# adalkiran/llama-nuts-and-bolts

Hardware: AMD Instinct MI355X
Metric: decode tokens/s Llama-3.1-8B bf16 @1/2/4/8 MI355X; % HBM roofline (higher is better)
Workload: dtype bf16; 1 GPU; Llama-3.1-8B bf16, 1xMI355X, single-prompt greedy decode, seq_len=128 -> +125 tokens (configs[1]'s prompt, --steps 125); prompt_len=128, sequences_in_flight=1, parallelism=single GPU, mode=exact-order (token-id identical to the CPU reference path), reported_repeat=median, weight_bytes_resident=16060522496

## Files before the change

### include/lnb.h

```cpp
#ifndef LNB_H
#define LNB_H
#include <stdint.h>
#ifdef __cplusplus
extern "C" {
#endif

typedef struct lnb_model lnb_model;
typedef struct lnb_ctx lnb_ctx;

typedef struct lnb_model_args {
    int32_t dim;
    int32_t n_layers;
    int32_t n_heads;
    int32_t n_kv_heads;
    int32_t vocab_size;
    int32_t multiple_of;
    double  ffn_dim_multiplier;
    float   norm_eps;
    int32_t use_scaled_rope;
    double  rope_theta;
    int32_t max_seq_len;
} lnb_model_args;

#define LNB_ABI_VERSION 6
// ... 52 lines not shown
enum { LNB_SCHED_LATENCY = 0, LNB_SCHED_THROUGHPUT = 1 };
int lnb_ctx_set_schedule(lnb_ctx* c, int sched);
int lnb_ctx_get_schedule(const lnb_ctx* c);
int lnb_ctx_set_attention(lnb_ctx* c, int long_threshold, int force_zseq);
int lnb_ctx_zseq_count(lnb_ctx* c, int* out);
int lnb_ctx_norm_fallbacks(lnb_ctx* c, int* out);
int lnb_ctx_prefill_attention_form(const lnb_ctx* c, int* out);
typedef void (*lnb_layer_cb)(int layer_1based, int n_layers, double secs, void* user);
int lnb_ctx_set_layer_callback(lnb_ctx* c, lnb_layer_cb cb, void* user);

int lnb_forward(lnb_ctx* c, const int32_t* tokens, int seq, int start_pos, float* logits_out, int32_t* argmax_last_out);

int lnb_forward_append(lnb_ctx* c, const int32_t* tokens, int seq, int start_pos, float* logits_out, int32_t* argmax_last_out);
int lnb_forward_score_append(lnb_ctx* c, const int32_t* tokens, int seq, int start_pos, const int32_t* targets,
                             float* target_logit, float* target_prob, double* log_z, int32_t* argmax_last_out);
int lnb_ctx_set_rows_attention(lnb_ctx* c, int long_threshold, int flags);
int lnb_ctx_append_attention_form(const lnb_ctx* c, int* out);

int lnb_forward_append_many(lnb_ctx* const* ctxs, int n, const int32_t* tokens, const int32_t* n_rows, const int32_t* start_pos,
                            float* logits_out, int32_t* argmax_out);
int lnb_model_append_many_info(const lnb_model* m, int* passes, int* max_columns, int* long_passes);

int lnb_decode_greedy(lnb_ctx* c, int32_t token, int start_pos, int n_steps, int32_t* out_tokens, float* ms_out);
int lnb_ctx_set_stop_ids(lnb_ctx* c, const int32_t* ids, int n);
int lnb_decode_greedy_until(lnb_ctx* c, int32_t token, int start_pos, int max_steps, int32_t* out_tokens, int* n_generated, int* finished, float* ms_out);

#define LNB_MAX_DRAFT 15
typedef struct lnb_spec_stats { int64_t passes, verify_passes, drafted, accepted; } lnb_spec_stats;
int lnb_ctx_set_draft(lnb_ctx* c, int max_draft, int ngram_min, int ngram_max, const int32_t* corpus, int n_corpus);
int lnb_decode_speculative_until(lnb_ctx* c, const int32_t* history, int n_history, int32_t token, int start_pos,
                                 int max_steps, int32_t* out_tokens, int* n_generated, int* finished,
                                 lnb_spec_stats* stats, float* ms_out);
int lnb_op_ngram_draft(int device, const int32_t* text, int n_text, const int32_t* corpus, int n_corpus,
                       int ngram_min, int ngram_max, int max_draft, int32_t* out, int* n_out);

typedef struct lnb_spec_many_info { int64_t passes, verify_passes, columns, max_columns, long_passes; } lnb_spec_many_info;
int lnb_decode_speculative_many(lnb_ctx* const* ctxs, int n, const int32_t* const* history, const int32_t* n_history,
                                const int32_t* tokens, const int32_t* start_pos, int max_steps, int col_budget,
                                int32_t* out_tokens, int32_t* n_generated, int32_t* finished,
                                lnb_spec_stats* stats, lnb_spec_many_info* info, float* ms_out);

#define LNB_MAX_TOP_K 16
int lnb_ctx_set_token_probs(lnb_ctx* c, int top_k);
int lnb_ctx_read_token_probs(lnb_ctx* c, int first, int n, int32_t* ids, float* logits, float* probs, double* log_z);
int lnb_ctx_token_prob_walks(lnb_ctx* c, int* out);
int lnb_forward_score(lnb_ctx* c, const int32_t* tokens, int seq, int start_pos, const int32_t* targets,
                      float* target_logit, float* target_prob, double* log_z, int32_t* argmax_last_out);
int lnb_op_token_probs(int device, const uint16_t* logits_bf16, int rows, int V, int top_k, const int32_t* targets,
                       int force_serial, int32_t* ids, float* logits, float* probs, float* target_prob, double* log_z, int* serial_walks);

typedef struct lnb_batch lnb_batch;
int lnb_model_enable_batch(lnb_model* m);
int64_t lnb_model_batch_bytes(lnb_model* m);
int lnb_batch_create(lnb_ctx* const* ctxs, int n, lnb_batch** out);
int lnb_batch_destroy(lnb_batch* b);
int lnb_batch_decode(lnb_batch* b, const int32_t* tokens, const int32_t* start_pos, int n_steps, int32_t* out_tokens, float* ms_out);
int lnb_batch_decode_until(lnb_batch* b, const int32_t* tokens, const int32_t* start_pos, int max_steps, int32_t* out_tokens, int32_t* n_generated, int32_t* finished, float* ms_out);
int lnb_batch_profile_kernel(lnb_batch* b, int which, int pos, int iters, float* avg_ms_out);
int lnb_batch_set_attention(lnb_batch* b, int long_threshold, int force_zseq);
int lnb_ctx_set_batched_attention(lnb_ctx* c, int long_threshold, int force_zseq);
int lnb_batch_attention_form(const lnb_batch* b, int* out);
int lnb_ctx_verify_attention_form(const lnb_ctx* c, int* out);

void* lnb_ctx_hidden_ptr(lnb_ctx* c, int which);
int lnb_forward_stage(lnb_ctx* c, const int32_t* tokens, int seq, int start_pos, float* logits_out, int32_t* argmax_last_out);
int lnb_forward_stage_begin(lnb_ctx* c, const int32_t* tokens, int seq, int start_pos, int want_argmax);
int lnb_forward_stage_end(lnb_ctx* c, int32_t* argmax_last_out);
int lnb_ctx_synchronize(lnb_ctx* c);
void* lnb_ctx_stream(lnb_ctx* c);

typedef struct lnb_pipe lnb_pipe;
int lnb_pipeline_unique_id(void* id128);
int lnb_pipeline_init(lnb_model* stage, int rank, int world, const void* id128, lnb_pipe** out);
int lnb_pipeline_init_loopback(lnb_model* stage, int rank, int world, const char* group, lnb_pipe** out);
int lnb_pipeline_init_host(lnb_model* stage, int rank, int world, lnb_pipe** out);
int lnb_pipeline_destroy(lnb_pipe* p);
int lnb_pipeline_tick(lnb_pipe* p, lnb_ctx* run, int run_rows, int run_pos, const int32_t* run_tokens,
                      lnb_ctx* send, int send_rows, lnb_ctx* recv, int recv_rows, int* token_slot_out);
int lnb_batch_set_state(lnb_batch* b, const int32_t* tokens, const int32_t* start_pos);
int lnb_batch_check_error(lnb_batch* b);
void* lnb_batch_boundary_ptr(lnb_batch* b, int which);
int lnb_pipeline_tick_batch(lnb_pipe* p, lnb_batch* run, lnb_batch* send, lnb_batch* recv, int* token_slot_out);
int lnb_pipeline_sync(lnb_pipe* p);
int lnb_pipeline_comm_count(lnb_pipe* p, int* out);
int lnb_pipeline_read_tokens(lnb_pipe* p, int first_slot, int n, int32_t* out);
int lnb_pipeline_selftest(int device, int n_bytes);

int lnb_profile_kernel(lnb_ctx* c, int which, int pos, int iters, float* avg_ms_out);
int lnb_profile_ffn_pair(lnb_ctx* c, int pos, int iters, int w2_delay_us, int w2_lds_pad, float* avg_ms_out);
int lnb_profile_kernel_stamps(lnb_ctx* c, int which, int pos, double* out, int* wall_clock_khz);

int lnb_op_linear(int device, const uint16_t* x, const uint16_t* w, uint16_t* y, int rows, int n_out, int k_in, int rw);
int lnb_op_rmsnorm_linear(int device, const uint16_t* x, const uint16_t* norm_w, float eps, const uint16_t* w,
                          uint16_t* y, int rows, int n_out, int k_in, int rw);

int lnb_op_linear_mode(int device, const uint16_t* x, const uint16_t* norm_w, float eps, const uint16_t* w, uint16_t* y,
                       int rows, int n_out, int k_in, int rw, int mode);
int lnb_op_argmax(int device, const uint16_t* logits_bf16, int n, int32_t* out);
int lnb_op_exp_table(int device, float divisor, double* out65536);

typedef struct lnb_checkpoint lnb_checkpoint;
enum { LNB_DTYPE_BF16 = 0, LNB_DTYPE_F16 = 1, LNB_DTYPE_F32 = 2 };
int lnb_checkpoint_open(const char* path, lnb_checkpoint** out);
void lnb_checkpoint_close(lnb_checkpoint* c);
int lnb_checkpoint_num_tensors(const lnb_checkpoint* c);
int lnb_checkpoint_find(const lnb_checkpoint* c, const char* name);
int lnb_checkpoint_tensor(const lnb_checkpoint* c, int index, const char** name, int* dtype, int64_t* shape4, int* rank,
                          const void** data, int64_t* nbytes);
int lnb_model_load_checkpoint(lnb_model* m, const lnb_checkpoint* c);
int lnb_model_args_from_json(const char* params_json_path, lnb_model_args* out);

typedef struct lnb_tokenizer lnb_tokenizer;
int lnb_tokenizer_load(const char* tokenizer_model_path, lnb_tokenizer** out);
void lnb_tokenizer_free(lnb_tokenizer* t);
int lnb_tokenizer_vocab_size(const lnb_tokenizer* t);
int lnb_tokenizer_special(const lnb_tokenizer* t, int32_t* bos, int32_t* eos, int32_t* eot, int32_t* eom);
int lnb_tokenizer_token_id(const lnb_tokenizer* t, const char* bytes, int len);
int lnb_tokenizer_piece(const lnb_tokenizer* t, int32_t id, const char** bytes, int* len);
int lnb_tokenizer_encode(const lnb_tokenizer* t, const char* text, int len, int32_t* out, int cap);
int lnb_tokenizer_encode_chat(const lnb_tokenizer* t, const char* const* headers, const char* const* contents, int n_parts,
                              int32_t* out, int cap);
typedef struct lnb_detok lnb_detok;
int lnb_tokenizer_stream_create(const lnb_tokenizer* t, lnb_detok** out);
void lnb_tokenizer_stream_free(lnb_detok* d);
int lnb_tokenizer_decode_stream(lnb_detok* d, int32_t token_id, char* out, int cap, int* added_to_waiting);
int lnb_tokenizer_stream_pending(const lnb_detok* d, const char** bytes, int* len);

#ifdef __cplusplus
}
#endif
#endif
```

### llama-nuts-and-bolts_amd/csrc/lnb_api.cpp

```cpp
#include <hip/hip_runtime.h>
#include <algorithm>
#include <array>
#include <cmath>
#include <cstdarg>
#include <cstdio>
#include <cstdlib>
#include <cstring>
#include <chrono>
#include <dirent.h>
#include <unistd.h>
#include <deque>
#include <map>
#include <mutex>
#include <string>
#include <vector>
#include "../../include/lnb.h"
#include "lnb_device.h"
#include "lnb_knobs.h"
#include "lnb_kvcopy.h"
#include "lnb_rowpack.h"
#include "lnb_batchplan.h"
#include "lnb_rccl.h"
static_assert(LNB_MAX_SEQ_LEN == LNB_SEQ_MAX, "lnb.h and lnb_device.h disagree on the longest context");
static_assert(ROWPACK_MAX_W == LNB_BATCH_MAX, "lnb_rowpack.h and lnb_device.h disagree on the columns of a pass");
static_assert(BATCHPLAN_COLS == LNB_STREAM_COLS, "lnb_batchplan.h and lnb_device.h disagree on the sequences of a column group");
static_assert(LNB_MAX_FORK == KVC_MAX_DST, "lnb.h and lnb_kvcopy.h disagree on the destinations of a fork");
static_assert(LNB_MAX_TOP_K == LNB_TOKPROB_MAX_K, "lnb.h and lnb_device.h disagree on the largest top-k");
static_assert(LNB_MAX_DRAFT == LNB_SPEC_MAX_DRAFT && LNB_MAX_DRAFT + 1 <= LNB_STREAM_COLS, "a verify pass is one column group of at most 16 columns");

extern "C" {
hipError_t lnbk_gemv(const GemvParams* p, int rw, int nch, int epi, int norm, hipStream_t st);
hipError_t lnbk_attn(const AttnParams* p, hipStream_t st);
hipError_t lnbk_attn_rows(const AttnParams* p, int pos0, hipStream_t st);
int lnbk_attn_short_max_T(int hd);
size_t lnbk_attn_long_lds(int seq_len);
size_t lnbk_attn_long_layout_lds(int seq_len);
size_t lnbk_attn_one_lds(int seq_len, int hd);
hipError_t lnbk_exp_table(double* tab, float divisor, hipStream_t st);
hipError_t lnbk_gemm(const GemmParams* p, int epi, hipStream_t st);
hipError_t lnbk_rmsnorm_rows(const uint16_t* x, const uint16_t* w, uint16_t* out, int S, int K, float eps, hipStream_t st);
hipError_t lnbk_embed(const uint16_t* emb, const int32_t* tokens, uint16_t* x, int S, int dim, int vocab, int* err, hipStream_t st);
hipError_t lnbk_argmax(const uint16_t* logits, int V, int32_t* next_token, StepState* state, int32_t* out_tokens, int out_cap, int advance, hipStream_t st);
hipError_t lnbk_set_state(StepState* state, int pos, int n_out, int honour_stop, hipStream_t st);
hipError_t lnbk_set_stop(StepState* state, const int32_t* ids, int n, hipStream_t st);
hipError_t lnbk_advance_state(StepState* state, int rows, hipStream_t st);
hipError_t lnbk_tile(const uint16_t* src, uint16_t* dst, int rows, int K, int row_off, int chain, int RW, int NCH, int gather, hipStream_t st);
hipError_t lnbk_synth_fill(uint16_t* dst, int rows, int K, int row_off, int chain, int RW, int NCH, uint64_t seed, uint32_t tensor_id, int kind, float sigma, hipStream_t st);
hipError_t lnbk_init(void);
hipError_t lnbk_fast_gemv(const GemvParams* p, int rw, int nch, int epi, int norm, hipStream_t st);
hipError_t lnbk_fast_gemm(const GemmParams* p, int epi, hipStream_t st);
hipError_t lnbk_fast_attn(const AttnParams* p, hipStream_t st);
hipError_t lnbk_fast_init(void);
hipError_t lnbk_m16_from_tiled(const uint16_t* src, uint16_t* dst, int rows, int K, int RW, int NCH, hipStream_t st);
hipError_t lnbk_stream(const StreamParams* p, int epi, int acc2, int num_cus, hipStream_t st);
hipError_t lnbk_batch_rmsnorm(const uint16_t* x, const uint16_t* norm_w, float eps, uint16_t* xt, int K, int nseq, hipStream_t st);
hipError_t lnbk_batch_embed(const uint16_t* emb, const BatchTab* tab, uint16_t* x, int nseq, int dim, int vocab, int* err, hipStream_t st);
hipError_t lnbk_batch_argmax(const uint16_t* logits, int V, const BatchTab* tab, int nseq, int32_t* ring, hipStream_t st);
hipError_t lnbk_batch_set_state(const BatchTab* tab, const int32_t* tokens, const int32_t* pos, int32_t* ring, int honour_stop, hipStream_t st);
hipError_t lnbk_batch_scatter_ring(const BatchTab* tab, const int32_t* ring, hipStream_t st);
hipError_t lnbk_batch_advance(const BatchTab* tab, hipStream_t st);
hipError_t lnbk_batch_prepare(void);
hipError_t lnbk_gemm_stream(const GemmParams* p, int epi, int num_cus, hipStream_t st);
hipError_t lnbk_spin(int us, hipStream_t st);
hipError_t lnbk_token_probs(const TokProbParams* p, hipStream_t st);
hipError_t lnbk_spec_argmax(const uint16_t* logits, int V, int w, int32_t* g, hipStream_t st);
hipError_t lnbk_spec_commit(const int32_t* g, int w, const BatchTab* tab, hipStream_t st);
hipError_t lnbk_ngram_draft(const DraftParams* p, hipStream_t st);
hipError_t lnbk_kv_fork(const KvForkTab* tab, int nt, int split, hipStream_t st);
hipError_t lnbk_append_many_setup(const AmPass* p, hipStream_t st);
hipError_t lnbk_append_many_finish(const uint16_t* logits, int V, const AmRow* rows, int width, int32_t* out, hipStream_t st);
hipError_t lnbk_spec_many_draft(const SmPass* p, hipStream_t st);
hipError_t lnbk_spec_many_pack(const SmPass* p, hipStream_t st);
hipError_t lnbk_spec_many_commit(const SmPass* p, hipStream_t st);
}

static int g_hwq_set_by_library = 0;
static int g_hip_live_at_load = 0;
static bool kfd_is_open() {
    DIR* d = opendir("/proc/self/fd");
    if (!d) return false;
    bool found = false;
    char path[64], target[256];
    while (struct dirent* e = readdir(d)) {
        if (e->d_name[0] == '.') continue;
        snprintf(path, sizeof path, "/proc/self/fd/%s", e->d_name);
        const ssize_t n = readlink(path, target, sizeof target - 1);
        if (n <= 0) continue;
        target[n] = 0;
        if (!strcmp(target, "/dev/kfd")) { found = true; break; }
    }
    closedir(d);
    return found;
}
__attribute__((constructor)) static void lnb_record_hip_state_at_load() {
    g_hip_live_at_load = kfd_is_open() ? 1 : 0;
}

static thread_local char g_err[1024] = "";
static int fail(const char* fmt, ...) {
    va_list ap; va_start(ap, fmt); vsnprintf(g_err, sizeof g_err, fmt, ap); va_end(ap);
    return -1;
}
extern "C" const char* lnb_last_error(void) { return g_err; }
extern "C" __attribute__((visibility("hidden"))) void lnb_set_error(const char* msg) { snprintf(g_err, sizeof g_err, "%s", msg); }
#define HIPCHK(expr) do { hipError_t e_ = (expr); if (e_ != hipSuccess) return fail("%s failed: %s (%s:%d)", #expr, hipGetErrorString(e_), __FILE__, __LINE__); } while (0)

static inline float bf_wide_h(uint16_t b) { uint32_t u = (uint32_t)b << 16; float f; memcpy(&f, &u, 4); return f; }
static inline uint16_t bf_trunc_h(float f) { uint32_t u; memcpy(&u, &f, 4); return (uint16_t)(u >> 16); }

struct TensorRef {
    int rows = 0, cols = 0;
    bool tiled = false;
    uint16_t* linear = nullptr;
    TiledDesc* td = nullptr;
    int row_off = 0, chain = 0;
    uint32_t synth_id = 0; int synth_kind = 0;
    int rank = 2;
};
struct LayerW {
    uint16_t* attn_norm = nullptr; uint16_t* ffn_norm = nullptr;
    TiledDesc wqkv{}, wo{}, w13{}, w2{};
    uint16_t *m_wqkv = nullptr, *m_wo = nullptr, *m_w13 = nullptr, *m_w2 = nullptr;
};
struct lnb_model {
    lnb_model_args a{};
    int device = 0, layer_begin = 0, layer_end = 0;
    int part_begin = 0, part_end = 0;
    int head_dim = 0, n_rep = 0, ffn_hidden = 0, q_dim = 0, kv_dim = 0;
    uint16_t* tok_embd = nullptr; uint16_t* norm = nullptr; TiledDesc output{};
    std::vector<LayerW> layers;
    std::map<std::string, TensorRef> tensors;
    float* cis = nullptr; int cis_rows = 0; float* silu = nullptr; double* exp_tab = nullptr;
    double* prob_etab = nullptr;
    std::vector<float> cis_host;
    hipStream_t stream = nullptr;
    bool finalized = false;
    int64_t weight_bytes = 0;
    bool batch_enabled = false; uint16_t* m_output = nullptr; int64_t batch_bytes = 0;
    std::mutex am_mu; struct AppendMany* am = nullptr;
    bool first() const { return part_begin == 0; }
    bool last() const { return part_end == 3 * a.n_layers; }
    bool has_part(int l, int q) const { return 3 * l + q >= part_begin && 3 * l + q < part_end; }
    bool has_attn(int l) const { return has_part(l, 0); }
    bool has_w13(int l) const { return has_part(l, 1); }
    bool has_w2(int l) const { return has_part(l, 2); }
    bool whole(int l) const { return has_attn(l) && has_w13(l) && has_w2(l); }
};
struct lnb_ctx {
    lnb_model* m = nullptr; int seq_len = 0;
    int max_rows = 0;
    hipStream_t stream = nullptr;
    std::vector<uint16_t*> ck, cv;
    StepState* st = nullptr; int32_t* dtok = nullptr; int32_t* dnext = nullptr; int* derr = nullptr;
    int32_t* dout = nullptr; int dout_cap = 0;
    uint16_t *x = nullptr, *h = nullptr, *q = nullptr, *att = nullptr, *ffn = nullptr, *logits = nullptr;
    uint16_t* xn = nullptr;
    int logits_rows = 0;
    hipGraphExec_t graph = nullptr;
    hipEvent_t ev0 = nullptr, ev1 = nullptr;
    lnb_layer_cb cb = nullptr; void* cb_user = nullptr;
    int32_t* h_io = nullptr;
    bool pending = false, pending_tokens = false, pending_argmax = false;
    int mode = LNB_MODE_EXACT;
    int sched = LNB_SCHED_LATENCY;
    int n_stop = 0;
    int batch_users = 0;
    double* e_buf = nullptr; double* z_part = nullptr; int* zseq_count = nullptr;
    int last_prefill_form = 0;
    uint64_t* score_idx = nullptr; size_t score_idx_bytes = 0; int sidx_jt = 0;
    unsigned* attn_cnt = nullptr;
    int attn_long_T = 0; int force_zseq = 0;
    int attn_short_cap = 0;
    bool attn_long = false;
    hipGraphExec_t graph_long = nullptr;
    hipGraphExec_t stage_graph[2] = {nullptr, nullptr};
    hipEvent_t ev_done = nullptr, ev_in = nullptr, ev_sent = nullptr;
    bool in_pending = false, sent_pending = false;
    int dev_pos = -1;
    bool attn_causal = false;
    int call_T = 0;
    hipEvent_t ev_h2d = nullptr; bool h2d_pending = false;
    bool recv_unmatched = false;
    int top_k = 0;
    TokProbOut* tp_out = nullptr;
    int32_t* tp_ids = nullptr; float* tp_logit = nullptr; float* tp_prob = nullptr; double* tp_logz = nullptr;
    double* tp_zpart = nullptr; uint64_t* tp_kpart = nullptr; unsigned* tp_cnt = nullptr;
    int tp_last_k = 0, tp_last_n = 0;
    void* sc_buf = nullptr; size_t sc_bytes = 0;
    int sp_max_draft = 0, sp_ngram_min = 1, sp_ngram_max = 1;
    int32_t* sp_corpus = nullptr; int sp_n_corpus = 0;
    int32_t* sp_text = nullptr; int sp_text_cap = 0;
// ... 131 lines not shown

extern "C" int lnb_model_ffn_hidden_dim(const lnb_model_args* a) {
    int h = 4 * a->dim;
    h = (int)(2 * h / 3);
    if (a->ffn_dim_multiplier > -1) h = (int)(a->ffn_dim_multiplier * (double)h);
    h = a->multiple_of * ((h + a->multiple_of - 1) / a->multiple_of);
    return h;
}

static void reg_linear(lnb_model* m, const std::string& name, uint16_t* p, int cols, uint32_t sid, int kind, int rows = 1, int rank = 1) {
    TensorRef r; r.rows = rows; r.cols = cols; r.tiled = false; r.linear = p; r.synth_id = sid; r.synth_kind = kind; r.rank = rank;
    m->tensors[name] = r;
}
static void reg_tiled(lnb_model* m, const std::string& name, TiledDesc* td, int rows, int cols, int row_off, int chain, uint32_t sid) {
    TensorRef r; r.rows = rows; r.cols = cols; r.tiled = true; r.td = td; r.row_off = row_off; r.chain = chain; r.synth_id = sid; r.rank = 2;
    m->tensors[name] = r;
}

extern "C" int lnb_model_create(const lnb_model_args* args, int device, int layer_begin, int layer_end, lnb_model** out) {
    return lnb_model_create_parts(args, device, 3 * layer_begin, 3 * layer_end, out);
}
static int model_alloc(lnb_model* m);
extern "C" int lnb_model_create_parts(const lnb_model_args* args, int device, int part_begin, int part_end, lnb_model** out) {
    if (!args || !out) return fail("null argument");
    *out = nullptr;
    const int layer_begin = part_begin / 3, layer_end = (part_end + 2) / 3;
    lnb_model_args a = *args;
    if (a.n_kv_heads < 0) a.n_kv_heads = a.n_heads;
    if (a.rope_theta <= 0) a.rope_theta = 500000.0;
    if (a.n_layers <= 0) return fail("n_layers must be positive (got %d)", a.n_layers);
    if (a.vocab_size <= 0) return fail("vocab_size must be positive (got %d; params.json without the key gives -1: take it from tok_embeddings)", a.vocab_size);
    if (a.multiple_of <= 0) return fail("multiple_of must be positive (got %d)", a.multiple_of);
    if (a.dim <= 0 || a.n_heads <= 0 || a.n_kv_heads <= 0 || a.dim % a.n_heads || a.n_heads % a.n_kv_heads) return fail("invalid head configuration");
    if (part_begin < 0 || part_end > 3 * a.n_layers || part_begin >= part_end) return fail("invalid layer range [%d,%d)", part_begin / 3, (part_end + 2) / 3);
    int hd = a.dim / a.n_heads;
    if (a.dim % 8 || hd % 8) return fail("dim and head_dim must be multiples of 8");
    int ndev = 0; HIPCHK(hipGetDeviceCount(&ndev));
    if (ndev == 0) return fail("no HIP device: liblnb_hip.so has no CPU fallback");
    if (device < 0 || device >= ndev) return fail("device %d out of range (%d devices)", device, ndev);
    HIPCHK(hipSetDevice(device));
    HIPCHK(lnbk_init());
    HIPCHK(lnbk_fast_init());
    HIPCHK(lnbk_batch_prepare());
    { hipDeviceProp_t prop; HIPCHK(hipGetDeviceProperties(&prop, device)); if (prop.multiProcessorCount > 0) g_num_cus = prop.multiProcessorCount; }
    lnb_model* m = new lnb_model();
    m->a = a; m->device = device; m->layer_begin = layer_begin; m->layer_end = layer_end; m->part_begin = part_begin; m->part_end = part_end;
    m->head_dim = hd; m->n_rep = a.n_heads / a.n_kv_heads; m->ffn_hidden = lnb_model_ffn_hidden_dim(&a);
    m->q_dim = a.n_heads * hd; m->kv_dim = a.n_kv_heads * hd;
    if (m->ffn_hidden <= 0 || m->ffn_hidden % 8) { delete m; return fail("ffn hidden dim must be a positive multiple of 8"); }
    if (model_alloc(m)) { lnb_model_destroy(m); return -1; }
    *out = m;
    return 0;
}
static int model_alloc(lnb_model* m) {
    const lnb_model_args& a = m->a;
    const int layer_begin = m->layer_begin, layer_end = m->layer_end;
    HIPCHK(hipStreamCreate(&m->stream));
    int64_t& wb = m->weight_bytes;
    const int dim = a.dim, F = m->ffn_hidden;
    if (m->first()) {
        if (alloc_linear(&m->tok_embd, (size_t)a.vocab_size * dim, wb)) return -1;
        reg_linear(m, "tok_embeddings.weight", m->tok_embd, dim, 0, 0, a.vocab_size, 2);
    }
    m->layers.resize(layer_end - layer_begin);
    const int qkv_rows = m->q_dim + 2 * m->kv_dim, rwo = auto_rw(dim, Knob::RW_WO, m->q_dim, true), rw2 = auto_rw(dim, Knob::RW_W2, F, true);
    const int rwq = auto_rw(qkv_rows, Knob::RW_QKV, dim, false, qkv_rows == 24 * g_num_cus && dim % 256 == 0 ? 24 : 0);
    const int rw13 = auto_rw(F, Knob::RW_W13, 0, false, F == 56 * g_num_cus ? 56 : 0);
    for (int l = layer_begin; l < layer_end; l++) {
        LayerW& L = m->layers[l - layer_begin];
        char nm[128]; uint32_t base = 16u * (uint32_t)(l + 1);
        if (m->has_attn(l)) {
            if (alloc_linear(&L.attn_norm, dim, wb)) return -1;
            if (alloc_tiled(L.wqkv, m->q_dim + 2 * m->kv_dim, dim, rwq, 1, wb)) return -1;
            if (alloc_tiled(L.wo, dim, m->q_dim, rwo, 1, wb)) return -1;
            snprintf(nm, sizeof nm, "layers.%d.attention_norm.weight", l); reg_linear(m, nm, L.attn_norm, dim, base + 0, 1);
            snprintf(nm, sizeof nm, "layers.%d.attention.wq.weight", l); reg_tiled(m, nm, &L.wqkv, m->q_dim, dim, 0, 0, base + 1);
            snprintf(nm, sizeof nm, "layers.%d.attention.wk.weight", l); reg_tiled(m, nm, &L.wqkv, m->kv_dim, dim, m->q_dim, 0, base + 2);
            snprintf(nm, sizeof nm, "layers.%d.attention.wv.weight", l); reg_tiled(m, nm, &L.wqkv, m->kv_dim, dim, m->q_dim + m->kv_dim, 0, base + 3);
            snprintf(nm, sizeof nm, "layers.%d.attention.wo.weight", l); reg_tiled(m, nm, &L.wo, dim, m->q_dim, 0, 0, base + 4);
        }
        if (m->has_w13(l)) {
            if (alloc_linear(&L.ffn_norm, dim, wb)) return -1;
            if (alloc_tiled(L.w13, F, dim, rw13, 2, wb)) return -1;
            snprintf(nm, sizeof nm, "layers.%d.ffn_norm.weight", l); reg_linear(m, nm, L.ffn_norm, dim, base + 5, 1);
            snprintf(nm, sizeof nm, "layers.%d.feed_forward.w1.weight", l); reg_tiled(m, nm, &L.w13, F, dim, 0, 0, base + 6);
            snprintf(nm, sizeof nm, "layers.%d.feed_forward.w3.weight", l); reg_tiled(m, nm, &L.w13, F, dim, 0, 1, base + 8);
        }
        if (m->has_w2(l)) {
            if (alloc_tiled(L.w2, dim, F, rw2, 1, wb)) return -1;
            snprintf(nm, sizeof nm, "layers.%d.feed_forward.w2.weight", l); reg_tiled(m, nm, &L.w2, dim, F, 0, 0, base + 7);
        }
    }
    if (m->last()) {
        if (alloc_linear(&m->norm, dim, wb)) return -1;
        reg_linear(m, "norm.weight", m->norm, dim, 1, 1);
        if (alloc_tiled(m->output, a.vocab_size, dim, auto_rw(a.vocab_size, Knob::RW_OUT), 1, wb)) return -1;
        reg_tiled(m, "output.weight", &m->output, a.vocab_size, dim, 0, 0, 2);
    }
    return 0;
}

static void append_many_free(lnb_model* m);
extern "C" int lnb_model_destroy(lnb_model* m) {
    if (!m) return 0;
    hipSetDevice(m->device);
    append_many_free(m);
    if (m->tok_embd) hipFree(m->tok_embd);
    if (m->norm) hipFree(m->norm);
    if (m->output.w) hipFree(m->output.w);
    for (auto& L : m->layers) {
        hipFree(L.attn_norm); hipFree(L.ffn_norm); hipFree(L.wqkv.w); hipFree(L.wo.w); hipFree(L.w13.w); hipFree(L.w2.w);
        hipFree(L.m_wqkv); hipFree(L.m_wo); hipFree(L.m_w13); hipFree(L.m_w2);
    }
    hipFree(m->m_output);
    if (m->cis) hipFree(m->cis);
    if (m->silu) hipFree(m->silu);
    if (m->exp_tab) hipFree(m->exp_tab);
    if (m->prob_etab) hipFree(m->prob_etab);
    if (m->stream) hipStreamDestroy(m->stream);
    delete m;
    return 0;
}

extern "C" int64_t lnb_model_weight_bytes(lnb_model* m) { return m ? m->weight_bytes : 0; }

extern "C" int lnb_model_set_tensor(lnb_model* m, const char* name, const uint16_t* host, const int64_t* shape, int rank) {
    if (!m || !name || !host || !shape) return fail("null argument");
    HIPCHK(hipSetDevice(m->device));
    auto it = m->tensors.find(name);
    if (it == m->tensors.end()) return fail("tensor \"%s\" does not belong to this model stage", name);
    if (m->batch_enabled) return fail("tensor \"%s\": the model's batched-decode copy has been built; bind tensors before lnb_model_enable_batch", name);
    TensorRef& r = it->second;
    if (rank != r.rank || (rank == 1 && shape[0] != r.cols) || (rank == 2 && (shape[0] != r.rows || shape[1] != r.cols)))
        return fail("tensor \"%s\": shape mismatch, expected [%d%s%d]", name, r.rank == 1 ? r.cols : r.rows, r.rank == 1 ? "" : " ", r.rank == 1 ? 0 : r.cols);
    size_t n = (size_t)r.rows * r.cols;
    if (!r.tiled) { HIPCHK(hipMemcpy(r.linear, host, n * 2, hipMemcpyHostToDevice)); return 0; }
    uint16_t* stage = nullptr;
    HIPCHK(hipMalloc((void**)&stage, n * 2));
    HIPCHK(hipMemcpy(stage, host, n * 2, hipMemcpyHostToDevice));
    hipError_t e = lnbk_tile(stage, r.td->w, r.rows, r.cols, r.row_off, r.chain, r.td->rw, r.td->nch, 0, m->stream);
    if (e == hipSuccess) e = hipStreamSynchronize(m->stream);
    hipFree(stage);
    HIPCHK(e);
    return 0;
}

extern "C" int lnb_model_num_tensors(const lnb_model* m) { return m ? (int)m->tensors.size() : 0; }
extern "C" int lnb_model_tensor_info(const lnb_model* m, int k, const char** name, int64_t* shape, int* rank) {
    if (!m || k < 0 || k >= (int)m->tensors.size()) return fail("tensor index %d out of range", k);
    auto it = m->tensors.begin();
    std::advance(it, k);
    if (name) *name = it->first.c_str();
    if (rank) *rank = it->second.rank;
    if (shape) { if (it->second.rank == 1) shape[0] = it->second.cols; else { shape[0] = it->second.rows; shape[1] = it->second.cols; } }
    return 0;
}

extern "C" int lnb_model_get_tensor(lnb_model* m, const char* name, uint16_t* host, int64_t nelem) {
    if (!m || !name || !host) return fail("null argument");
    HIPCHK(hipSetDevice(m->device));
    auto it = m->tensors.find(name);
    if (it == m->tensors.end()) return fail("tensor \"%s\" does not belong to this model stage", name);
    TensorRef& r = it->second;
    size_t n = (size_t)r.rows * r.cols;
    if ((int64_t)n != nelem) return fail("tensor \"%s\": expected %zu elements", name, n);
    if (!r.tiled) { HIPCHK(hipMemcpy(host, r.linear, n * 2, hipMemcpyDeviceToHost)); return 0; }
    uint16_t* stage = nullptr;
    HIPCHK(hipMalloc((void**)&stage, n * 2));
    hipError_t e = lnbk_tile(r.td->w, stage, r.rows, r.cols, r.row_off, r.chain, r.td->rw, r.td->nch, 1, m->stream);
    if (e == hipSuccess) e = hipStreamSynchronize(m->stream);
    if (e == hipSuccess) e = hipMemcpy(host, stage, n * 2, hipMemcpyDeviceToHost);
    hipFree(stage);
    HIPCHK(e);
    return 0;
}

extern "C" int lnb_model_fill_synthetic(lnb_model* m, uint64_t seed) {
    if (!m) return fail("null argument");
    if (m->batch_enabled) return fail("the model's batched-decode copy has been built; fill the weights before lnb_model_enable_batch");
    HIPCHK(hipSetDevice(m->device));
    for (auto& kv : m->tensors) {
        TensorRef& r = kv.second;
        if (r.tiled) HIPCHK(lnbk_synth_fill(r.td->w, r.rows, r.cols, r.row_off, r.chain, r.td->rw, r.td->nch, seed, r.synth_id, 0, 0.02f, m->stream));
        else HIPCHK(lnbk_synth_fill(r.linear, r.rows, r.cols, 0, 0, 0, 1, seed, r.synth_id, r.synth_kind, 0.02f, m->stream));
    }
    HIPCHK(hipStreamSynchronize(m->stream));
    return 0;
}

static void build_rope_table(int head_dim, int rows, double theta, bool scaled, std::vector<float>& cis) {
    const int n = head_dim / 2;
    std::vector<uint16_t> freqs(n);
    const float dimf = (float)head_dim;
    for (int i = 0; i < n; i++) {
        float val = bf_wide_h(bf_trunc_h((float)(2 * i)));
        freqs[i] = bf_trunc_h((float)(1.0 / std::pow(theta, (double)(val / dimf))));
    }
    if (scaled) {
        const float scale_factor = 8.0f, low_freq_factor = 1.0f, high_freq_factor = 4.0f, old_context_len = 8192.0f;
        const float low_freq_wavelen = old_context_len / low_freq_factor, high_freq_wavelen = old_context_len / high_freq_factor;
        for (int i = 0; i < n; i++) {
            volatile float freq = bf_wide_h(freqs[i]);
            volatile float wavelen = (float)(2 * M_PI) / freq;
            float nf;
            if (wavelen < high_freq_wavelen) nf = freq;
            else if (wavelen > low_freq_wavelen) nf = freq / scale_factor;
            else {
                volatile float smooth = (old_context_len / wavelen - low_freq_factor) / (high_freq_factor - low_freq_factor);
                volatile float t1 = (1 - smooth) * freq; t1 = t1 / scale_factor;
                volatile float t2 = smooth * freq;
                nf = t1 + t2;
            }
            freqs[i] = bf_trunc_h(nf);
        }
    }
    cis.resize((size_t)rows * n * 2);
    for (int p = 0; p < rows; p++) {
        const float t = bf_wide_h(bf_trunc_h((float)p));
        for (int i = 0; i < n; i++) {
            volatile float prod = t * bf_wide_h(freqs[i]);
            const double ang = (double)bf_wide_h(bf_trunc_h(prod));
            cis[((size_t)p * n + i) * 2 + 0] = (float)std::cos(ang);
            cis[((size_t)p * n + i) * 2 + 1] = (float)std::sin(ang);
        }
    }
}

static void prob_exp_table(std::vector<double>& et) {
    et.resize(1 << 16);
    for (int i = 0; i < (1 << 16); i++) et[i] = std::exp((double)bf_wide_h((uint16_t)i));
}
extern "C" int lnb_model_finalize(lnb_model* m, int rope_rows) {
    if (!m) return fail("null argument");
    HIPCHK(hipSetDevice(m->device));
    m->cis_rows = rope_rows > 0 ? rope_rows : m->a.max_seq_len * 2;
    build_rope_table(m->head_dim, m->cis_rows, m->a.rope_theta, m->a.use_scaled_rope != 0, m->cis_host);
    if (m->cis) hipFree(m->cis);
    HIPCHK(hipMalloc((void**)&m->cis, m->cis_host.size() * 4));
    HIPCHK(hipMemcpy(m->cis, m->cis_host.data(), m->cis_host.size() * 4, hipMemcpyHostToDevice));
    std::vector<float> silu(1 << 16);
    for (int i = 0; i < (1 << 16); i++) { double x = (double)bf_wide_h((uint16_t)i); silu[i] = (float)(x / (1.0 + std::exp(-x))); }
    if (!m->silu) HIPCHK(hipMalloc((void**)&m->silu, silu.size() * 4));
    HIPCHK(hipMemcpy(m->silu, silu.data(), silu.size() * 4, hipMemcpyHostToDevice));
    std::vector<double> et;
    prob_exp_table(et);
    if (!m->prob_etab) HIPCHK(hipMalloc((void**)&m->prob_etab, et.size() * 8));
    HIPCHK(hipMemcpy(m->prob_etab, et.data(), et.size() * 8, hipMemcpyHostToDevice));
    if (!m->exp_tab) HIPCHK(hipMalloc((void**)&m->exp_tab, (size_t)(1 << 16) * 8));
    HIPCHK(lnbk_exp_table(m->exp_tab, bf_wide_h(bf_trunc_h((float)std::sqrt((double)m->head_dim))), m->stream));
    HIPCHK(hipStreamSynchronize(m->stream));
    m->finalized = true;
    return 0;
}

extern "C" int lnb_model_rope_table(lnb_model* m, float* out, int64_t nfloats, int* rows_out) {
    if (!m || !m->finalized) return fail("model not finalized");
    if (rows_out) *rows_out = m->cis_rows;
    if (out) {
        if ((size_t)nfloats != m->cis_host.size()) return fail("rope table has %zu floats", m->cis_host.size());
        memcpy(out, m->cis_host.data(), m->cis_host.size() * 4);
    }
    return 0;
}

static int ctx_alloc(lnb_ctx* c);
static int ctx_create_common(lnb_model* m, int seq_len, int max_rows, lnb_ctx** out) {
    if (m->head_dim != 128 && m->head_dim != 64 && m->head_dim != 32) return fail("head_dim %d not one of 32/64/128", m->head_dim);
    lnb_ctx* c = new lnb_ctx();
    c->m = m; c->seq_len = seq_len; c->max_rows = max_rows > 0 && max_rows < seq_len ? max_rows : seq_len;
    if (ctx_alloc(c)) { lnb_ctx_destroy(c); return -1; }
    *out = c;
    return 0;
}
extern "C" int lnb_ctx_create(lnb_model* m, int seq_len, lnb_ctx** out) {
    if (!m || !out) return fail("null argument");
    *out = nullptr;
    if (!m->finalized) return fail("model not finalized");
    HIPCHK(hipSetDevice(m->device));
    const int sl = seq_len > 0 ? seq_len : m->a.max_seq_len;
    if (m->head_dim != 128 && m->head_dim != 64 && m->head_dim != 32) return fail("head_dim %d not one of 32/64/128", m->head_dim);
    if (lnbk_attn_long_lds(sl) > 160 * 1024)
        return fail("seq_len %d too long for the LDS staging of the attention kernels (about 23000 positions)", sl);
    return ctx_create_common(m, sl, 0, out);
}
extern "C" int lnb_ctx_create_long(lnb_model* m, int seq_len, int max_rows, lnb_ctx** out) {
    if (!m || !out) return fail("null argument");
    *out = nullptr;
    if (!m->finalized) return fail("model not finalized");
    HIPCHK(hipSetDevice(m->device));
    const int sl = seq_len > 0 ? seq_len : m->a.max_seq_len;
    if (sl > LNB_MAX_SEQ_LEN) return fail("seq_len %d too long: a long context holds at most %d positions", sl, LNB_MAX_SEQ_LEN);
    if (sl > m->cis_rows)
        return fail("seq_len %d is beyond the model's %d-row RoPE table: pass rope_rows >= %d to lnb_model_finalize", sl, m->cis_rows, sl);
    return ctx_create_common(m, sl, max_rows, out);
}
extern "C" int lnb_ctx_max_rows(const lnb_ctx* c, int* out) {
    if (!c || !out) return fail("null argument");
    *out = c->max_rows;
    return 0;
}
static int ctx_alloc(lnb_ctx* c) {
    lnb_model* m = c->m;
    HIPCHK(hipStreamCreateWithFlags(&c->stream, hipStreamNonBlocking));
// ... 324 lines not shown
    uint16_t* ck = c->ck[l - m->layer_begin]; uint16_t* cv = c->cv[l - m->layer_begin];
    uint16_t* const hbuf = m->whole(l) ? c->h : c->x;
    if (use_mfma(S) && which != K_ATTN) {
        switch (which) {
        case K_QKV: {
            HIPCHK(lnbk_rmsnorm_rows(c->x, L.attn_norm, c->xn, S, a.dim, a.norm_eps, st));
            GemmParams g = gemm_of(L.wqkv, c->xn, a.dim, L.wqkv.n_rows, S, c->st);
            g.cis = m->cis; g.q_out = c->q; g.cache_k = ck; g.cache_v = cv; g.seq_len = c->seq_len; g.q_dim = m->q_dim; g.kv_dim = m->kv_dim; g.head_dim = m->head_dim;
            HIPCHK(gemm_dispatch(c->mode, &g, EPI_QKV_ROPE, st)); return 0; }
        case K_WO: { GemmParams g = gemm_of(L.wo, c->att, m->q_dim, a.dim, S, c->st); g.out = hbuf; g.res = c->x; HIPCHK(gemm_dispatch(c->mode, &g, EPI_RESID, st)); return 0; }
        case K_W13: {
            HIPCHK(lnbk_rmsnorm_rows(hbuf, L.ffn_norm, c->xn, S, a.dim, a.norm_eps, st));
            GemmParams g = gemm_of(L.w13, c->xn, a.dim, m->ffn_hidden, S, c->st); g.out = c->ffn; g.silu = m->silu;
            HIPCHK(gemm_dispatch(c->mode, &g, EPI_SILU_MUL, st)); return 0; }
        case K_W2: { GemmParams g = gemm_of(L.w2, c->ffn, m->ffn_hidden, a.dim, S, c->st); g.out = c->x; g.res = hbuf; HIPCHK(gemm_dispatch(c->mode, &g, EPI_RESID, st)); return 0; }
        }
    }
    switch (which) {
    case K_QKV: {
        GemvParams g{}; g.w = L.wqkv.w; g.x = c->x; g.norm_w = L.attn_norm; g.norm_fb = c->zseq_count + 1; g.eps = a.norm_eps; g.K = a.dim; g.n_rows = L.wqkv.n_rows; g.S = S; g.st = c->st;
        g.cis = m->cis; g.q_out = c->q; g.cache_k = ck; g.cache_v = cv; g.seq_len = c->seq_len; g.q_dim = m->q_dim; g.kv_dim = m->kv_dim; g.head_dim = m->head_dim;
        g.sched = c->sched;
        set_grid(g, L.wqkv); HIPCHK(gemv_dispatch(c, &g, L.wqkv.rw, 1, EPI_QKV_ROPE, 1, st)); return 0; }
    case K_ATTN: {
        AttnParams ap{}; ap.q = c->q; ap.cache_k = ck; ap.cache_v = cv; ap.out = c->att; ap.st = c->st; ap.dbg = g_dbg;
        ap.S = S; ap.H = a.n_heads; ap.KVH = a.n_kv_heads; ap.hd = m->head_dim; ap.seq_len = c->seq_len;
        ap.lds_T = c->seq_len < c->attn_short_cap ? c->seq_len : c->attn_short_cap;
        ap.host_T = c->call_T;
        ap.divisor = bf_wide_h(bf_trunc_h((float)std::sqrt((double)m->head_dim)));
        ap.mfma = use_mfma(S) ? 1 : 0; ap.exp_tab = m->exp_tab;
        ap.causal = (c->attn_causal && S > 1) ? 1 : 0;
        ap.longctx = 0; ap.force_zseq = c->force_zseq & 1; ap.e_buf = c->e_buf; ap.z_part = c->z_part; ap.zseq_count = c->zseq_count; ap.cnt = c->attn_cnt;
        if (ap.mfma && c->sidx_jt > 0 && c->call_T > 0 && c->sidx_jt * 16 >= c->call_T) { ap.score_idx = c->score_idx; ap.sidx_jt = c->sidx_jt; }
        if (S == 1 && c->attn_long) {
            const bool one = (knob(Knob::ATTN_ONE) || (c->force_zseq & 12)) && !(c->force_zseq & 2) && c->sched == LNB_SCHED_LATENCY && m->head_dim % 16 == 0 &&
                             a.n_heads * (m->head_dim / 16) <= g_num_cus && lnbk_attn_one_lds(c->seq_len, m->head_dim) <= (size_t)160 * 1024;
            ap.longctx = one ? ((c->force_zseq & 4) ? 3 : 2) : 1;
        }
        if (c->attn_rows && ap.causal) {
            ap.e_buf = c->sp_e_buf; ap.z_part = c->sp_z_part; ap.force_zseq = c->rows_flags & 1;
            HIPCHK(lnbk_attn_rows(&ap, c->call_T - S, st)); return 0;
        }
        if (c->mode == LNB_MODE_FAST && ap.mfma) {
            hipError_t e = lnbk_fast_attn(&ap, st);
            if (e != hipErrorNotSupported) { HIPCHK(e); return 0; }
        }
        HIPCHK(lnbk_attn(&ap, st)); return 0; }
    case K_WO: {
        GemvParams o{}; o.w = L.wo.w; o.x = c->att; o.K = m->q_dim; o.n_rows = a.dim; o.S = S; o.st = c->st; o.out = hbuf; o.res = c->x; o.sched = c->sched;
        set_grid(o, L.wo); HIPCHK(gemv_dispatch(c, &o, L.wo.rw, 1, EPI_RESID, 0, st)); return 0; }
    case K_W13: {
        GemvParams f{}; f.w = L.w13.w; f.x = hbuf; f.norm_w = L.ffn_norm; f.norm_fb = c->zseq_count + 1; f.eps = a.norm_eps; f.K = a.dim; f.n_rows = m->ffn_hidden; f.S = S; f.st = c->st;
        f.out = c->ffn; f.silu = m->silu; f.sched = c->sched;
        set_grid(f, L.w13); HIPCHK(gemv_dispatch(c, &f, L.w13.rw, 2, EPI_SILU_MUL, 1, st)); return 0; }
    case K_W2: {
        GemvParams d{}; d.w = L.w2.w; d.x = c->ffn; d.K = m->ffn_hidden; d.n_rows = a.dim; d.S = S; d.st = c->st; d.out = c->x; d.res = hbuf; d.lds_pad = lds_pad; d.sched = c->sched; d.prio = knob(Knob::W2_PRIO);
        set_grid(d, L.w2); HIPCHK(gemv_dispatch(c, &d, L.w2.rw, 1, EPI_RESID, 0, st)); return 0; }
    }
    return fail("bad kernel id");
}
static int enqueue_layers(lnb_ctx* c, int S, bool with_cb) {
    lnb_model* m = c->m;
    for (int l = m->layer_begin; l < m->layer_end; l++) {
        auto t0 = std::chrono::steady_clock::now();
        for (int k = K_QKV; k <= K_W2; k++) {
            if (!(k <= K_WO ? m->has_attn(l) : k == K_W13 ? m->has_w13(l) : m->has_w2(l))) continue;
            if (enqueue_layer_kernel(c, l, S, k)) return -1;
        }
        if (with_cb && c->cb) {
            HIPCHK(hipStreamSynchronize(c->stream));
            double secs = std::chrono::duration<double>(std::chrono::steady_clock::now() - t0).count();
            c->cb(l + 1, m->a.n_layers, secs, c->cb_user);
        }
    }
    return 0;
}
static int enqueue_head(lnb_ctx* c, int first, int rows) {
    lnb_model* m = c->m;
    if (use_mfma(rows)) {
        HIPCHK(lnbk_rmsnorm_rows(c->x + (size_t)first * m->a.dim, m->norm, c->xn, rows, m->a.dim, m->a.norm_eps, c->stream));
        GemmParams gm = gemm_of(m->output, c->xn, m->a.dim, m->a.vocab_size, rows, c->st); gm.out = c->logits;
        HIPCHK(gemm_dispatch(c->mode, &gm, EPI_STORE, c->stream));
        return 0;
    }
    GemvParams g{}; g.w = m->output.w; g.x = c->x + (size_t)first * m->a.dim; g.norm_w = m->norm; g.norm_fb = c->zseq_count + 1; g.eps = m->a.norm_eps; g.K = m->a.dim;
    g.n_rows = m->a.vocab_size; g.S = rows; g.st = c->st; g.out = c->logits;
    set_grid(g, m->output);
    HIPCHK(gemv_dispatch(c, &g, m->output.rw, 1, EPI_STORE, 1, c->stream));
    return 0;
}

static bool want_long_attention(const lnb_ctx* c, int seq, int start_pos) {
    return seq == 1 && (start_pos + 1 > c->attn_long_T || start_pos + 1 > c->attn_short_cap);
}
static int check_call(lnb_ctx* c, int seq, int start_pos, bool causal = false) {
    if (seq == 0) return fail("empty token array");
    if (seq < 0 || start_pos < 0) return fail("negative sequence length or start position");
    const int T = start_pos + seq;
    if (T > c->m->cis_rows) return fail("incompatible locStart, locEnd values and tensor (position %d beyond the %d-row RoPE table)", T, c->m->cis_rows);
    if (T > c->seq_len) return fail("incompatible locStart, locEnd values and tensor (position %d beyond the KV cache of %d)", T, c->seq_len);
    if (seq > c->max_rows) return fail("a call of %d rows on a context whose activation buffers hold %d rows (lnb_ctx_create_long's max_rows)", seq, c->max_rows);
    if (seq > 1 && !causal && T % seq != 0) return fail("two tensor shapes cannot be broadcasted: [%d %d %d] and [%d %d]", c->m->a.n_heads, seq, T, seq, seq);
    const bool mfma_attn = use_mfma(seq) && (c->m->head_dim == 64 || c->m->head_dim == 128);
    c->call_T = T;
    c->sidx_jt = 0;
    bool stage_has_attn = false;
    for (int l = c->m->layer_begin; l < c->m->layer_end && !stage_has_attn; l++) stage_has_attn = c->m->has_attn(l);
// ... 1950 lines not shown
    HIPCHK(hipSetDevice(p->m->device));
    HIPCHK(hipDeviceSynchronize());
    for (int i = 0; i < n; i++) out[i] = p->h_tok[(first_slot + i) % p->tok_cap];
    return 0;
}

static int op_linear_impl(int device, const uint16_t* x, const uint16_t* norm_w, float eps, const uint16_t* w, uint16_t* y,
                          int rows, int n_out, int k_in, int rw, int mode = LNB_MODE_EXACT) {
    if (!x || !w || !y) return fail("null argument");
    if (rows <= 0 || n_out <= 0 || k_in <= 0) return fail("empty operand");
    if (k_in % 8) return fail("in_features must be a multiple of 8");
    int ndev = 0; HIPCHK(hipGetDeviceCount(&ndev));
    if (ndev == 0) return fail("no HIP device: liblnb_hip.so has no CPU fallback");
    HIPCHK(hipSetDevice(device));
    HIPCHK(lnbk_init());
    HIPCHK(lnbk_fast_init());
    if (mode != LNB_MODE_EXACT && mode != LNB_MODE_FAST) return fail("unknown mode %d", mode);
    if (rw == 0) rw = auto_rw(n_out, Knob::RW_OP, k_in, norm_w == nullptr);
    if (rw != 16 && rw != 32 && rw != 64 && !(rw == 4 && !norm_w && k_in % 128 == 0 && k_in <= 16384) && !(rw == 24 && k_in % 256 == 0))
        return fail("rw must be 16, 32 or 64 (or 4: row-broadcast layout, no fused norm, in_features a multiple of 128; or 24: quad layout, in_features a multiple of 256)");
    if ((size_t)k_in * 4 > 120 * 1024) return fail("in_features %d does not fit the LDS staging", k_in);
    TiledDesc t{}; int64_t bytes = 0;
    if (alloc_tiled(t, n_out, k_in, rw, 1, bytes)) return -1;
    uint16_t *dx = nullptr, *dw = nullptr, *dy = nullptr, *dn = nullptr; StepState* st = nullptr;
    HIPCHK(hipMalloc((void**)&dx, (size_t)rows * k_in * 2)); HIPCHK(hipMalloc((void**)&dw, (size_t)n_out * k_in * 2));
    HIPCHK(hipMalloc((void**)&dy, (size_t)rows * n_out * 2)); HIPCHK(hipMalloc((void**)&st, sizeof(StepState)));
    HIPCHK(hipMemset(st, 0, sizeof(StepState)));
    HIPCHK(hipMemcpy(dx, x, (size_t)rows * k_in * 2, hipMemcpyHostToDevice));
    HIPCHK(hipMemcpy(dw, w, (size_t)n_out * k_in * 2, hipMemcpyHostToDevice));
    if (norm_w) { HIPCHK(hipMalloc((void**)&dn, (size_t)k_in * 2)); HIPCHK(hipMemcpy(dn, norm_w, (size_t)k_in * 2, hipMemcpyHostToDevice)); }
    HIPCHK(lnbk_tile(dw, t.w, n_out, k_in, 0, 0, rw, 1, 0, nullptr));
    if (use_mfma(rows) && knob(Knob::OP_STREAM) && k_in % 128 == 0) {
        HIPCHK(lnbk_batch_prepare());
        const size_t mb = m16_elems(n_out, k_in, 1) * 2;
        HIPCHK(hipMalloc((void**)&t.w16, mb)); HIPCHK(hipMemset(t.w16, 0, mb));
        HIPCHK(lnbk_m16_from_tiled(t.w, t.w16, n_out, k_in, rw, 1, nullptr));
    }
    if (use_mfma(rows)) {
        uint16_t* dxn = nullptr;
        if (norm_w) { HIPCHK(hipMalloc((void**)&dxn, (size_t)rows * k_in * 2)); HIPCHK(lnbk_rmsnorm_rows(dx, dn, dxn, rows, k_in, eps, nullptr)); }
        GemmParams gm = gemm_of(t, norm_w ? dxn : dx, k_in, n_out, rows, st); gm.out = dy;
        HIPCHK(gemm_dispatch(mode, &gm, EPI_STORE, nullptr));
        HIPCHK(hipDeviceSynchronize());
        if (dxn) hipFree(dxn);
    } else {
    GemvParams g{}; g.w = t.w; g.x = dx; g.norm_w = dn; g.eps = eps; g.K = k_in; g.n_rows = n_out; g.S = rows; g.st = st; g.out = dy;
    set_grid(g, t);
    if (mode == LNB_MODE_FAST) HIPCHK(lnbk_fast_gemv(&g, rw, 1, EPI_STORE, norm_w ? 1 : 0, nullptr));
    else HIPCHK(lnbk_gemv(&g, rw, 1, EPI_STORE, norm_w ? 1 : 0, nullptr));
    }
    HIPCHK(hipDeviceSynchronize());
    HIPCHK(hipMemcpy(y, dy, (size_t)rows * n_out * 2, hipMemcpyDeviceToHost));
    hipFree(dx); hipFree(dw); hipFree(dy); hipFree(st); hipFree(t.w); if (dn) hipFree(dn); if (t.w16) hipFree(t.w16);
    return 0;
}
extern "C" int lnb_op_argmax(int device, const uint16_t* logits_bf16, int n, int32_t* out) {
    if (!logits_bf16 || !out) return fail("null argument");
    if (n <= 0) return fail("empty operand");
    int ndev = 0; HIPCHK(hipGetDeviceCount(&ndev));
    if (ndev == 0) return fail("no HIP device: liblnb_hip.so has no CPU fallback");
    HIPCHK(hipSetDevice(device));
    uint16_t* d = nullptr; int32_t* dn = nullptr; StepState* st = nullptr;
    HIPCHK(hipMalloc((void**)&d, (size_t)n * 2 + 16)); HIPCHK(hipMalloc((void**)&dn, 16)); HIPCHK(hipMalloc((void**)&st, sizeof(StepState)));
    HIPCHK(hipMemset(st, 0, sizeof(StepState)));
    HIPCHK(hipMemcpy(d, logits_bf16, (size_t)n * 2, hipMemcpyHostToDevice));
    hipError_t e = lnbk_argmax(d, n, dn, st, nullptr, 0, 0, nullptr);
    if (e == hipSuccess) e = hipDeviceSynchronize();
    if (e == hipSuccess) e = hipMemcpy(out, dn, 4, hipMemcpyDeviceToHost);
    hipFree(d); hipFree(dn); hipFree(st);
    HIPCHK(e);
    return 0;
}
extern "C" int lnb_op_token_probs(int device, const uint16_t* logits_bf16, int rows, int V, int top_k, const int32_t* targets,
                                  int force_serial, int32_t* ids, float* logits, float* probs, float* target_prob, double* log_z, int* serial_walks) {
    if (!logits_bf16 || !log_z || (top_k > 0 && (!ids || !logits || !probs)) || (targets && !target_prob)) return fail("null argument");
    if (rows <= 0 || V <= 0) return fail("empty operand");
    if (top_k < 0 || top_k > LNB_MAX_TOP_K) return fail("top_k must be 0..%d (got %d)", LNB_MAX_TOP_K, top_k);
    if (targets) for (int i = 0; i < rows; i++) if (targets[i] >= V) return fail("target id %d at index %d is outside the row of %d", targets[i], i, V);
    int ndev = 0; HIPCHK(hipGetDeviceCount(&ndev));
    if (ndev == 0) return fail("no HIP device: liblnb_hip.so has no CPU fallback");
    HIPCHK(hipSetDevice(device));
    const size_t R = rows, K = top_k, G = lnb_tokprob_slices(rows);
    std::vector<double> et; prob_exp_table(et);
    const size_t o_et = align256(sizeof(TokProbOut)), o_x = o_et + align256(65536 * 8), o_z = o_x + align256(R * V * 2 + 16), o_k = o_z + align256(R * LNB_TOKPROB_MAX_G * 8),
                 o_cnt = o_k + align256(R * G * K * 8), o_ids = o_cnt + align256(R * 4), o_lg = o_ids + align256(R * K * 4), o_pr = o_lg + align256(R * K * 4),
                 o_lz = o_pr + align256(R * K * 4), o_tg = o_lz + align256(R * 8), o_tl = o_tg + align256(R * 4), o_tp = o_tl + align256(R * 4),
                 o_w = o_tp + align256(R * 4), need = o_w + 256;
    char* b = nullptr;
    HIPCHK(hipMalloc((void**)&b, need));
    TokProbOut o{}; o.ids = (int32_t*)(b + o_ids); o.logit = (float*)(b + o_lg); o.prob = (float*)(b + o_pr); o.log_z = (double*)(b + o_lz); o.walks = (int*)(b + o_w); o.cap = rows;
    TokProbParams p{};
    p.logits = (const uint16_t*)(b + o_x); p.V = V; p.rows = rows; p.k = top_k; p.G = (int)G; p.etab = (const double*)(b + o_et);
    p.zpart = (double*)(b + o_z); p.kpart = (uint64_t*)(b + o_k); p.cnt = (unsigned*)(b + o_cnt); p.out = (const TokProbOut*)b; p.per_row_out = 0;
    if (targets) { p.targets = (const int32_t*)(b + o_tg); p.tlogit = (float*)(b + o_tl); p.tprob = (float*)(b + o_tp); }
    p.force_serial = force_serial ? 1 : 0;
    int walks = 0;
    hipError_t e = hipMemcpy(b, &o, sizeof o, hipMemcpyHostToDevice);
    if (e == hipSuccess) e = hipMemcpy(b + o_et, et.data(), 65536 * 8, hipMemcpyHostToDevice);
    if (e == hipSuccess) e = hipMemcpy(b + o_x, logits_bf16, R * V * 2, hipMemcpyHostToDevice);
    if (e == hipSuccess && targets) e = hipMemcpy(b + o_tg, targets, R * 4, hipMemcpyHostToDevice);
    if (e == hipSuccess) e = hipMemset(b + o_cnt, 0, R * 4);
    if (e == hipSuccess) e = hipMemset(b + o_w, 0, 4);
    if (e == hipSuccess) e = lnbk_token_probs(&p, nullptr);
    if (e == hipSuccess) e = hipDeviceSynchronize();
    if (e == hipSuccess && K) e = hipMemcpy(ids, b + o_ids, R * K * 4, hipMemcpyDeviceToHost);
    if (e == hipSuccess && K) e = hipMemcpy(logits, b + o_lg, R * K * 4, hipMemcpyDeviceToHost);
// ... 37 lines not shown
```

### llama-nuts-and-bolts_amd/csrc/lnb_device.h

```cpp
#pragma once
#include <stdint.h>
#include <stddef.h>

#if defined(__HIPCC__)
#define LNB_HD __host__ __device__ __forceinline__
#else
#define LNB_HD inline
#endif

struct TiledDesc {
    uint16_t* w;
    int n_rows;
    int k;
    int rw;
    int nch;
    int n_blocks;
    uint16_t* w16;
};
LNB_HD size_t tiled_index(int n, int k, int c, int K, int RW, int NCH) {
    if (RW == 4) return ((((size_t)(n >> 2) * (size_t)(K >> 7) + (size_t)(k >> 7)) * 64 + (size_t)((n & 3) * 16 + (k & 15))) << 3) + (size_t)((k & 127) >> 4);
    size_t b = (size_t)(n / RW), r = (size_t)(n % RW), kc = (size_t)(k >> 3), e = (size_t)(k & 7);
    return ((((b * (size_t)(K >> 3) + kc) * (size_t)NCH + (size_t)c) * (size_t)RW + r) << 3) + e;
}
LNB_HD size_t tiled_elems(int n_rows, int K, int RW, int NCH) {
// ... 3 lines not shown

LNB_HD uint64_t lnb_splitmix64(uint64_t z) {
    z += 0x9E3779B97F4A7C15ULL;
    z = (z ^ (z >> 30)) * 0xBF58476D1CE4E5B9ULL;
    z = (z ^ (z >> 27)) * 0x94D049BB133111EBULL;
    return z ^ (z >> 31);
}
LNB_HD int32_t lnb_synth_isum(uint64_t base, uint64_t idx) {
    uint64_t a = lnb_splitmix64(base ^ idx);
    uint64_t b = lnb_splitmix64(a);
    int32_t s = 0;
    for (int i = 0; i < 4; i++) { s += (int32_t)((a >> (16 * i)) & 0xFFFF); s += (int32_t)((b >> (16 * i)) & 0xFFFF); }
    return s - 262140;
}

constexpr int LNB_MAX_STOP_IDS = 8;
struct StepState {
    int32_t pos;
    int32_t n_out;
    int32_t finished;
    int32_t n_stop;
    int32_t stop[LNB_MAX_STOP_IDS];
    int32_t honour_stop;
};

enum { EPI_STORE = 0, EPI_QKV_ROPE = 1, EPI_RESID = 2, EPI_SILU_MUL = 3 };

struct GemvParams {
    const uint16_t* w;
    const uint16_t* x;
    const uint16_t* norm_w;
    float eps;
    int K;
    int n_rows;
    int S;
    int n_blocks;
    int n_wg;
    const StepState* st;
    uint16_t* out;
    const uint16_t* res;
    const float* silu;
    const float* cis;
    uint16_t* q_out;
    uint16_t* cache_k;
    uint16_t* cache_v;
    int seq_len;
    int q_dim, kv_dim, head_dim;
    long long* dbg;
    int dbg_full;
    int* norm_fb;
    int lds_pad;
    int prio;
    int sched;
};

struct GemmParams {
    const uint16_t* w;
    int rw, nch;
    const uint16_t* x;
    int K, n_rows, S;
    const StepState* st;
    uint16_t* out; const uint16_t* res; const float* silu;
    const float* cis; uint16_t* q_out; uint16_t* cache_k; uint16_t* cache_v; int seq_len, q_dim, kv_dim, head_dim;
    const uint16_t* w16;
    const struct BatchTab* btab; const struct BatchKV* bkv;
    uint16_t* out_xt;
    int rows_fastest;
};

struct AttnParams {
    const uint16_t* q;
    const uint16_t* cache_k;
    const uint16_t* cache_v;
    uint16_t* out;
    const StepState* st;
    int S, H, KVH, hd, seq_len;
    int lds_T;
    int host_T;
    float divisor;
    long long* dbg;
    int mfma;
    const double* exp_tab;
    int longctx;
    int force_zseq;
    double* e_buf;
    double* z_part;
    int pw_floats;
    int* zseq_count;
    unsigned* cnt;
    const struct BatchTab* btab; const struct BatchKV* bkv; uint16_t* out_xt;
    uint64_t* score_idx;
    int sidx_jt;
    int touch;
    int causal;
    int head_major;
};
constexpr int LNB_ATTN_ROWS_MAX = 16;
struct AttnRowsParams {
    AttnParams a;
    int W;
    int row0;
    int pos0;
    int pos_off;
};

constexpr int LNB_BATCH_MAX = 128;
// ... 114 lines not shown
```

### llama-nuts-and-bolts_amd/csrc/lnb_kernels.hip

```cpp
#include <hip/hip_runtime.h>
#include <cstdlib>
#include <type_traits>
#include "lnb_device.h"
#include "lnb_seqsum.h"

#define DEVINL __device__ __forceinline__

DEVINL float bf_lo(uint32_t u) { return __uint_as_float(u << 16); }
DEVINL float bf_hi(uint32_t u) { return __uint_as_float(u & 0xffff0000u); }
DEVINL float bf_wide(uint16_t b) { return __uint_as_float(((uint32_t)b) << 16); }
DEVINL uint16_t bf_trunc(float f) { return (uint16_t)(__float_as_uint(f) >> 16); }

DEVINL uint4 ld_nt_u4(const void* p) {
    typedef unsigned int u4v __attribute__((ext_vector_type(4)));
    u4v v = __builtin_nontemporal_load((const u4v*)p);
    return make_uint4(v.x, v.y, v.z, v.w);
}

DEVINL float mac8(float acc, const float4& xa, const float4& xb, const uint4& w) {
    acc = fmaf(xa.x, bf_lo(w.x), acc); acc = fmaf(xa.y, bf_hi(w.x), acc);
    acc = fmaf(xa.z, bf_lo(w.y), acc); acc = fmaf(xa.w, bf_hi(w.y), acc);
    acc = fmaf(xb.x, bf_lo(w.z), acc); acc = fmaf(xb.y, bf_hi(w.z), acc);
    acc = fmaf(xb.z, bf_lo(w.w), acc); acc = fmaf(xb.w, bf_hi(w.w), acc);
    return acc;
}

DEVINL float add4(float acc, const float4& p) { acc += p.x; acc += p.y; acc += p.z; acc += p.w; return acc; }
DEVINL void touch16(const float4& a, const float4& b, const float4& c, const float4& d) {
    asm volatile("" ::"v"(a.x), "v"(a.y), "v"(a.z), "v"(a.w), "v"(b.x), "v"(b.y), "v"(b.z), "v"(b.w),
                 "v"(c.x), "v"(c.y), "v"(c.z), "v"(c.w), "v"(d.x), "v"(d.y), "v"(d.z), "v"(d.w));
}
typedef float f32x2 __attribute__((ext_vector_type(2)));
DEVINL float4 mul4(const float4& x, float w0, float w1, float w2, float w3) {
    f32x2 a = {x.x, x.y}, b = {x.z, x.w}, u = {w0, w1}, v = {w2, w3};
    a = a * u; b = b * v;
    return make_float4(a.x, a.y, b.x, b.y);
}


template <bool NORM> struct XCh { static constexpr int value = NORM ? 6 : 12; };
template <bool NORM, int NS, int X_CH>
DEVINL void x_issue(const GemvParams& p, const uint16_t* xrow, int sidx, int lane, uint4 (&xv)[X_CH], uint4 (&nv)[X_CH]) {
#pragma unroll
    for (int i = 0; i < X_CH; i++) {
        const int k = ((i * NS + sidx) * 64 + lane) * 8;
        const int kc = k < p.K ? k : p.K - 8;
        uint4 a = *(const uint4*)(xrow + kc);
        uint4 b = make_uint4(0, 0, 0, 0);
        if (NORM) b = *(const uint4*)(p.norm_w + kc);
        const bool in = k < p.K;
        xv[i] = make_uint4(in ? a.x : 0u, in ? a.y : 0u, in ? a.z : 0u, in ? a.w : 0u);
        nv[i] = b;
    }
}
template <bool NORM, int NS, int X_CH>
DEVINL void x_store(const GemvParams& p, float* xs, int kpad, int sidx, int lane, const uint4 (&xv)[X_CH]) {
#pragma unroll
// ... 332 lines not shown
            c.z = bf_wide(bf_trunc(bf_wide(bf_trunc(bf_lo(v.w) * r)) * bf_lo(wv.w)));
            c.w = bf_wide(bf_trunc(bf_wide(bf_trunc(bf_hi(v.w) * r)) * bf_hi(wv.w)));
            *(float4*)(xs + k) = a; *(float4*)(xs + k + 4) = c;
        }
    }
}

template <int NCH, int EPI, int PX = 1>
DEVINL void gemv_epilogue(const GemvParams& p, const float (&acc)[NCH], int m, int n, bool valid) {
    if (EPI == EPI_STORE) {
        if (valid) p.out[(size_t)m * p.n_rows + n] = bf_trunc(acc[0]);
    } else if (EPI == EPI_RESID) {
        if (valid) {
            size_t o = (size_t)m * p.n_rows + n;
            p.out[o] = bf_trunc(bf_wide(p.res[o]) + bf_wide(bf_trunc(acc[0])));
        }
    } else if (EPI == EPI_SILU_MUL) {
        if (valid) {
            uint16_t g = bf_trunc(acc[0]), u = bf_trunc(acc[NCH - 1]);
            uint16_t gs = bf_trunc(p.silu[g]);
            p.out[(size_t)m * p.n_rows + n] = bf_trunc(bf_wide(gs) * bf_wide(u));
        }
    } else if (EPI == EPI_QKV_ROPE) {
        const int pos = p.st->pos + m;
        const uint16_t mine = bf_trunc(acc[0]);
        const uint16_t other = (uint16_t)__shfl_xor((int)mine, PX);
        if (valid) {
            if (n < p.q_dim + p.kv_dim) {
                const int d = n % p.head_dim, i = d >> 1;
                const float2 cs = *(const float2*)(p.cis + ((size_t)pos * (p.head_dim >> 1) + i) * 2);
                const double cr = (double)cs.x, ci = (double)cs.y;
                uint16_t r16;
                if ((n & 1) == 0) { double a = (double)bf_wide(mine), bb = (double)bf_wide(other); r16 = bf_trunc((float)(a * cr - bb * ci)); }
                else              { double a = (double)bf_wide(other), bb = (double)bf_wide(mine); r16 = bf_trunc((float)(a * ci + bb * cr)); }
                if (n < p.q_dim) p.q_out[(size_t)m * p.q_dim + n] = r16;
                else {
                    const int kc = n - p.q_dim, kh = kc / p.head_dim;
                    p.cache_k[(((size_t)kh * (p.head_dim >> 3) + (d >> 3)) * p.seq_len + pos) * 8 + (d & 7)] = r16;
                }
            } else {
                p.cache_v[(size_t)pos * p.kv_dim + (n - p.q_dim - p.kv_dim)] = mine;
            }
        }
    }
}

#define TIMED_BARRIER() do { if (p.dbg_full) { long long tb_ = clock64(); __builtin_amdgcn_s_barrier(); t_wait += clock64() - tb_; } else __builtin_amdgcn_s_barrier(); } while (0)
#define LNB_STAMP(i) do { if (p.dbg && lane == 0) p.dbg[(size_t)4096 * 8 * 4 + ((size_t)blockIdx.x * 8 + wave) * 8 + (i)] = clock64() - t_begin; } while (0)
#define LNB_WALL_EXIT() do { if (p.dbg && lane == 0) p.dbg[(size_t)4096 * 8 * 4 + ((size_t)blockIdx.x * 8 + wave) * 8 + 7] = (long long)wall_clock64() - t_wall0; } while (0)
#define DBG_EXIT() do { if (p.dbg && lane == 0) { long long* d_ = p.dbg + ((size_t)blockIdx.x * 8 + wave) * 4; d_[0] = clock64() - t_begin; d_[1] = t_wait; d_[2] = t_x; d_[3] = t_aux; } LNB_WALL_EXIT(); } while (0)

typedef unsigned int u32x4 __attribute__((ext_vector_type(4)));
DEVINL void ld_nt_asm(u32x4& dst, unsigned voff, const char* sbase) { asm volatile("global_load_dwordx4 %0, %1, %2 nt ; RING_LOAD" : "=&v"(dst) : "v"(voff), "s"(sbase) : "memory"); }
template <int N, int NP> DEVINL void wait_ring(u32x4 (&b)[NP]) {
    static_assert(NP == 1 || NP == 2 || NP == 4 || NP == 8, "loads per stage per helper");
    if constexpr (NP == 1) asm volatile("s_waitcnt vmcnt(%1) ; RING_RETIRE %0" : "+v"(b[0]) : "n"(N) : "memory");
    if constexpr (NP == 2) asm volatile("s_waitcnt vmcnt(%2) ; RING_RETIRE %0 %1" : "+v"(b[0]), "+v"(b[1]) : "n"(N) : "memory");
    if constexpr (NP == 4) asm volatile("s_waitcnt vmcnt(%4) ; RING_RETIRE %0 %1 %2 %3" : "+v"(b[0]), "+v"(b[1]), "+v"(b[2]), "+v"(b[3]) : "n"(N) : "memory");
    if constexpr (NP == 8) asm volatile("s_waitcnt vmcnt(%8) ; RING_RETIRE %0 %1 %2 %3 %4 %5 %6 %7" : "+v"(b[0]), "+v"(b[1]), "+v"(b[2]), "+v"(b[3]), "+v"(b[4]), "+v"(b[5]), "+v"(b[6]), "+v"(b[7]) : "n"(N) : "memory");
}

template <int RW, int NCH, int SA, int NH, int R, int EPI, bool NORM, int XC = XCh<NORM>::value>
__global__ __launch_bounds__((1 + NH) * 64) void gemv_chain_kernel(GemvParams p) {
    extern __shared__ __attribute__((aligned(16))) char smem[];
    long long t_begin = p.dbg ? clock64() : 0, t_wait = 0, t_x = 0, t_aux = 0;
    const long long t_wall0 = p.dbg ? (long long)wall_clock64() : 0;
    constexpr int KC = SA / (NCH * RW * 16);
    constexpr int GS = KC / 2;
    constexpr int SB = 2 * SA;
    constexpr int UNITS = SA / 16;
    constexpr int NP = UNITS / (64 * NH);
    static_assert(KC >= 2 && (KC & 1) == 0, "bad stage geometry");
    static_assert(UNITS % (64 * NH) == 0 && R * NP <= 60, "vmcnt is a 6-bit counter");
    static_assert(NH >= 2, "x staging is sized for >= 3 stager waves");
    char* ringB = smem;
    float* xs = (float*)(smem + 2 * SB);

    const int lane = threadIdx.x & 63;
    const int wave = __builtin_amdgcn_readfirstlane((int)(threadIdx.x >> 6));
    const int K = p.K, S = p.S;
    const int m = (S == 1) ? 0 : (int)(blockIdx.x % (unsigned)S);
    const int wg = (S == 1) ? (int)blockIdx.x : (int)(blockIdx.x / (unsigned)S);
    const size_t stream_bytes = (size_t)K * NCH * RW * 2;
    const int nstages = (int)((stream_bytes + SA - 1) / SA);
    const int nb_mine = (p.n_blocks - wg + p.n_wg - 1) / p.n_wg;
    const int T = nb_mine * nstages;
    constexpr int NS = 1 + NH;
    const int kpad = nstages * KC * 8 + 320;
    const uint16_t* xrow = p.x + (size_t)m * K;

    constexpr int CW = (NH > 3) ? 3 : 0;
    if (wave != CW) {
        const int hw = wave < CW ? wave : wave - 1;
        u32x4 buf[R][NP];
        {
            uint4 xv[XC], nv[XC];
            x_issue<NORM, NS>(p, xrow, 1 + hw, lane, xv, nv);
            __builtin_amdgcn_s_waitcnt(0x0F70);
        const size_t last16 = stream_bytes - 16;
        static_assert(NCH == 1 || (NCH == 2 && NP % 2 == 0), "two chains: an even number of loads per lane (pairs)");
        unsigned loff[NP];
#pragma unroll
        for (int i = 0; i < NP; i++) {
            const int pq = ((i >> 1) * NH + hw) * 64 + lane;
            loff[i] = NCH == 2 ? (unsigned)((((pq / RW) * 2 + (i & 1)) * RW + (pq % RW)) * 16) : (unsigned)(((i * NH + hw) * 64 + lane) * 16);
        }
        int ib = wg, is = 0, issued = 0;
        auto issue_next = [&](u32x4 (&dst)[NP]) {
            const size_t soff = (size_t)is * SA;
            const char* sb = (const char*)p.w + (size_t)ib * stream_bytes + soff;
            const unsigned lim = (soff + SA <= stream_bytes) ? 0xFFFFFFFFu : (unsigned)(last16 - soff);
#pragma unroll
            for (int i = 0; i < NP; i++) ld_nt_asm(dst[i], loff[i] < lim ? loff[i] : lim, sb);
            if (issued + 1 < T) { issued++; if (++is == nstages) { is = 0; ib += p.n_wg; } }
        };
            constexpr bool late = NORM;
            constexpr int EARLY_ = NCH == 2 ? LNB_EARLY_W13 : LNB_EARLY_HEAD;
            constexpr int EARLY = late ? (EARLY_ < R ? EARLY_ : R) : R;
#pragma unroll
            for (int j = 0; j < EARLY; j++) issue_next(buf[j]);
            x_store<NORM, NS>(p, xs, kpad, 1 + hw, lane, xv);
            __builtin_amdgcn_fence(__ATOMIC_RELEASE, "workgroup");
            TIMED_BARRIER();
            if (NORM) {
                __builtin_amdgcn_fence(__ATOMIC_ACQUIRE, "workgroup");
                rms_fold<rms_nf(NH)>(p, xs, ringB, hw - (NH - rms_nf(NH)), lane, t_aux);
                {
#pragma unroll
                    for (int j = EARLY; j < R; j++) issue_next(buf[j]);
                }
                TIMED_BARRIER();
                __builtin_amdgcn_fence(__ATOMIC_ACQUIRE, "workgroup");
                if constexpr (NORM) x_normalize<NS>(p, xs, kpad, xs[kpad], 1 + hw, lane, xv, nv);
                __builtin_amdgcn_fence(__ATOMIC_RELEASE, "workgroup");
                TIMED_BARRIER();
            }
            __builtin_amdgcn_fence(__ATOMIC_ACQUIRE, "workgroup");
        int st = 0;
        for (int it0 = 0; it0 <= T; it0 += R) {
#pragma unroll
            for (int j = 0; j < R; j++) {
                const int t = it0 + j;
                if (t <= T) {
                    if (t < T) {
                        const long long tb_ = p.dbg_full ? clock64() : 0;
                        wait_ring<(R - 1) * NP, NP>(buf[j]);
                        if (p.dbg_full) t_x += clock64() - tb_;
                        char* dst = ringB + (t & 1) * SB;
                        const float* xst = xs + (size_t)st * (KC * 8);
                        if constexpr (NCH == 2) {
#pragma unroll
                            for (int pi = 0; pi < NP / 2; pi++) {
                                const int pq = (pi * NH + hw) * 64 + lane, kc = pq / RW, r = pq % RW;
                                const float4 xa = *(const float4*)(xst + kc * 8), xb = *(const float4*)(xst + kc * 8 + 4);
                                const u32x4 vg = buf[j][2 * pi], vu = buf[j][(2 * pi + 1) % NP];
                                const float4 ga = mul4(xa, bf_lo(vg.x), bf_hi(vg.x), bf_lo(vg.y), bf_hi(vg.y)), gb = mul4(xb, bf_lo(vg.z), bf_hi(vg.z), bf_lo(vg.w), bf_hi(vg.w));
                                const float4 ua = mul4(xa, bf_lo(vu.x), bf_hi(vu.x), bf_lo(vu.y), bf_hi(vu.y)), ub = mul4(xb, bf_lo(vu.z), bf_hi(vu.z), bf_lo(vu.w), bf_hi(vu.w));
                                char* d = dst + r * 16;
                                *(float4*)(d + ((4 * kc + 0) * RW) * 16) = make_float4(ga.x, ua.x, ga.y, ua.y);
                                *(float4*)(d + ((4 * kc + 1) * RW) * 16) = make_float4(ga.z, ua.z, ga.w, ua.w);
                                *(float4*)(d + ((4 * kc + 2) * RW) * 16) = make_float4(gb.x, ub.x, gb.y, ub.y);
                                *(float4*)(d + ((4 * kc + 3) * RW) * 16) = make_float4(gb.z, ub.z, gb.w, ub.w);
                            }
                        } else {
                        float4 xa[NP], xb[NP];
#pragma unroll
                        for (int i = 0; i < NP; i++) {
                            const int q = (i * NH + hw) * 64 + lane;
                            const int kc = q / (NCH * RW);
                            xa[i] = *(const float4*)(xst + kc * 8); xb[i] = *(const float4*)(xst + kc * 8 + 4);
                        }
#pragma unroll
                        for (int i = 0; i < NP; i++) {
                            const int q = (i * NH + hw) * 64 + lane;
                            const int kc = q / (NCH * RW), u = q % (NCH * RW);
                            const u32x4 v = buf[j][i];
                            *(float4*)(dst + ((2 * kc) * (NCH * RW) + u) * 16) = mul4(xa[i], bf_lo(v.x), bf_hi(v.x), bf_lo(v.y), bf_hi(v.y));
                            *(float4*)(dst + ((2 * kc + 1) * (NCH * RW) + u) * 16) = mul4(xb[i], bf_lo(v.z), bf_hi(v.z), bf_lo(v.w), bf_hi(v.w));
                        }
                        }
                        if (++st == nstages) st = 0;
                        __builtin_amdgcn_sched_barrier(0);
                        issue_next(buf[j]);
                    }
                    __builtin_amdgcn_fence(__ATOMIC_RELEASE, "workgroup");
                    TIMED_BARRIER();
                }
            }
        }
        }
        asm volatile("s_waitcnt vmcnt(0) ; RING_RETIRE_ALL" ::: "memory");
        DBG_EXIT();
        return;
    }
    {
        uint4 xv[XC], nv[XC];
        x_issue<NORM, NS>(p, xrow, 0, lane, xv, nv);
        x_store<NORM, NS>(p, xs, kpad, 0, lane, xv);
        __builtin_amdgcn_fence(__ATOMIC_RELEASE, "workgroup");
        TIMED_BARRIER();
        __builtin_amdgcn_fence(__ATOMIC_ACQUIRE, "workgroup");
        if (NORM) {
            const float r = rms_scale_wide<rms_nf(NH)>(p, xs, ringB, lane, t_aux);
            if (lane == 0) xs[kpad] = r;
            __builtin_amdgcn_fence(__ATOMIC_RELEASE, "workgroup");
            TIMED_BARRIER();
            if constexpr (NORM) x_normalize<NS>(p, xs, kpad, r, 0, lane, xv, nv);
            __builtin_amdgcn_fence(__ATOMIC_RELEASE, "workgroup");
            TIMED_BARRIER();
            __builtin_amdgcn_fence(__ATOMIC_ACQUIRE, "workgroup");
        }
    }
    if (p.dbg) t_x = clock64() - t_begin;
    LNB_STAMP(6);
    float acc[NCH];
#pragma unroll
    for (int c = 0; c < NCH; c++) acc[c] = 0.0f;
    const int row = (RW & (RW - 1)) == 0 ? (lane & (RW - 1)) : (lane % RW);
    int st = 0, blk = wg;
    for (int it = 0; it <= T; it++) {
        const int t = it - 1;
        if (t >= 0) {
            const char* src = ringB + (t & 1) * SB + row * 16;
            float4 pb[2][NCH][4];
#pragma unroll
            for (int c = 0; c < NCH; c++)
#pragma unroll
                for (int j = 0; j < 4; j++) pb[0][c][j] = *(const float4*)(src + ((j * NCH + c) * RW) * 16);
#pragma unroll
            for (int g = 0; g < GS; g++) {
                const int cur = g & 1, nxt = cur ^ 1;
                if (g + 1 < GS) {
#pragma unroll
                    for (int c = 0; c < NCH; c++)
#pragma unroll
                        for (int j = 0; j < 4; j++) pb[nxt][c][j] = *(const float4*)(src + (((4 * (g + 1) + j) * NCH + c) * RW) * 16);
                }
                __builtin_amdgcn_sched_barrier(0);
#pragma unroll
                for (int c = 0; c < NCH; c++) touch16(pb[cur][c][0], pb[cur][c][1], pb[cur][c][2], pb[cur][c][3]);
                __builtin_amdgcn_sched_barrier(0);
                if constexpr (NCH == 2) {
                    f32x2 a2 = {acc[0], acc[1]};
#pragma unroll
                    for (int j = 0; j < 4; j++)
#pragma unroll
                        for (int h = 0; h < 2; h++) {
                            const float4 q4 = pb[cur][h][j];
                            a2 = a2 + f32x2{q4.x, q4.y};
                            a2 = a2 + f32x2{q4.z, q4.w};
                        }
                    acc[0] = a2.x; acc[1] = a2.y;
                } else {
#pragma unroll
                for (int j = 0; j < 4; j++)
#pragma unroll
                    for (int c = 0; c < NCH; c++) acc[c] = add4(acc[c], pb[cur][c][j]);
                }
                __builtin_amdgcn_sched_barrier(0);
            }
            if (++st == nstages) {
                gemv_epilogue<NCH, EPI>(p, acc, m, blk * RW + lane, (lane < RW) && (blk * RW + lane < p.n_rows));
#pragma unroll
                for (int c = 0; c < NCH; c++) acc[c] = 0.0f;
                st = 0; blk += p.n_wg;
            }
        }
        TIMED_BARRIER();
        __builtin_amdgcn_fence(__ATOMIC_ACQUIRE, "workgroup");
    }
    DBG_EXIT();
}

#define LNB_QP(j) " quad_perm:[" #j "," #j "," #j "," #j "] row_mask:0xf bank_mask:0xf\n\t"
#define LNB_QADD4(j) "v_add_f32_dpp %0, %1, %0" LNB_QP(j) "v_add_f32_dpp %0, %2, %0" LNB_QP(j) "v_add_f32_dpp %0, %3, %0" LNB_QP(j) "v_add_f32_dpp %0, %4, %0" LNB_QP(j)
DEVINL void chain16q(float& acc, const float4& q) {
    asm volatile("s_nop 1\n\t" LNB_QADD4(0) LNB_QADD4(1) LNB_QADD4(2) LNB_QADD4(3) : "+v"(acc) : "v"(q.x), "v"(q.y), "v"(q.z), "v"(q.w));
}
constexpr int GQ_SLOTS = 3;
__host__ __device__ constexpr int gq_ncw(int RW) { return (RW + 15) / 16; }
template <int RW, int KS, int NH, int R, int EPI, bool NORM, int XC = XCh<NORM>::value>
__global__ __launch_bounds__((gq_ncw(RW) + NH) * 64) void gemv_quad_kernel(GemvParams p) {
    extern __shared__ __attribute__((aligned(16))) char smem[];
    long long t_begin = p.dbg ? clock64() : 0, t_wait = 0, t_x = 0, t_aux = 0;
    const long long t_wall0 = p.dbg ? (long long)wall_clock64() : 0;
    constexpr int NCW = gq_ncw(RW), NW = NCW + NH;
    constexpr int KC = KS / 8;
    constexpr int GS = KS / 16;
    constexpr int SA = RW * KS * 2;
    constexpr int SB = 2 * SA;
    constexpr int UNITS = RW * KC;
    constexpr int NP = UNITS / (64 * NH);
    static_assert(RW % 8 == 0 && KS % 16 == 0, "rows in eights (conflict-free product writes), whole 16-step groups");
    static_assert(UNITS % (64 * NH) == 0 && R * NP <= 60, "vmcnt is a 6-bit counter");
    static_assert(NH >= 2 && GS >= 4 && GS % 4 == 0, "stage geometry");
    char* ringB = smem;
    float* xs = (float*)(smem + GQ_SLOTS * SB);

    const int lane = threadIdx.x & 63;
    const int wave = __builtin_amdgcn_readfirstlane((int)(threadIdx.x >> 6));
    const int K = p.K, S = p.S;
    const int m = (S == 1) ? 0 : (int)(blockIdx.x % (unsigned)S);
    const int wg = (S == 1) ? (int)blockIdx.x : (int)(blockIdx.x / (unsigned)S);
    const size_t stream_bytes = (size_t)K * RW * 2;
    const int nstages = (int)((stream_bytes + SA - 1) / SA);
    const int nb_mine = (p.n_blocks - wg + p.n_wg - 1) / p.n_wg;
    const int T = nb_mine * nstages;
    constexpr int NS = NW;
    const int kpad = nstages * KS + 320;
    const uint16_t* xrow = p.x + (size_t)m * K;

    if (wave >= NCW) {
        const int hw = wave - NCW;
        u32x4 buf[R][NP];
        uint4 xv[XC], nv[XC];
        x_issue<NORM, NS>(p, xrow, wave, lane, xv, nv);
        __builtin_amdgcn_s_waitcnt(0x0F70);
        const size_t last16 = stream_bytes - 16;
        unsigned loff[NP];
#pragma unroll
        for (int i = 0; i < NP; i++) loff[i] = (unsigned)(((i * NH + hw) * 64 + lane) * 16);
        int ib = wg, is = 0, issued = 0;
        auto issue_next = [&](u32x4 (&dst)[NP]) {
            const size_t soff = (size_t)is * SA;
            const char* sb = (const char*)p.w + (size_t)ib * stream_bytes + soff;
// ... 2926 lines not shown
    const float qnan = __uint_as_float(0x7FC00000u);
    if (lane < k) {
        const size_t at = (size_t)slot * k + lane;
        o.ids[at] = id;
        o.logit[at] = id >= 0 ? bf_wide(b) : qnan;
        o.prob[at] = id >= 0 ? pr : qnan;
    }
    if (lane == 0 && o.log_z) o.log_z[slot] = log(z);
    if (lane == 32 && p.targets) { p.tlogit[row] = id >= 0 ? bf_wide(b) : qnan; p.tprob[row] = id >= 0 ? pr : qnan; }
}

__global__ void set_state_kernel(StepState* st, int pos, int n_out, int honour_stop) { st->pos = pos; st->n_out = n_out; st->finished = 0; st->honour_stop = honour_stop; }
struct StopIds { int32_t n; int32_t id[LNB_MAX_STOP_IDS]; };
__global__ void set_stop_kernel(StepState* st, StopIds s) { st->n_stop = s.n; for (int k = 0; k < LNB_MAX_STOP_IDS; k++) st->stop[k] = k < s.n ? s.id[k] : -1; st->finished = 0; }
__global__ void advance_state_kernel(StepState* st, int rows) { st->pos = st->pos + rows; }

__global__ void tile_scatter_kernel(const uint16_t* src, uint16_t* dst, int rows, int K, int row_off, int chain, int RW, int NCH) {
    size_t idx = (size_t)blockIdx.x * blockDim.x + threadIdx.x;
    size_t total = (size_t)rows * (K >> 3);
    if (idx >= total) return;
    int r = (int)(idx / (K >> 3)), kc = (int)(idx % (K >> 3));
    uint4 v = *(const uint4*)(src + (size_t)r * K + (size_t)kc * 8);
    if (RW == 4) {
        const uint16_t* e = (const uint16_t*)&v;
        for (int i = 0; i < 8; i++) dst[tiled_index(row_off + r, kc * 8 + i, chain, K, RW, NCH)] = e[i];
        return;
    }
    *(uint4*)(dst + tiled_index(row_off + r, kc * 8, chain, K, RW, NCH)) = v;
}
__global__ void tile_gather_kernel(const uint16_t* src, uint16_t* dst, int rows, int K, int row_off, int chain, int RW, int NCH) {
    size_t idx = (size_t)blockIdx.x * blockDim.x + threadIdx.x;
    size_t total = (size_t)rows * (K >> 3);
    if (idx >= total) return;
    int r = (int)(idx / (K >> 3)), kc = (int)(idx % (K >> 3));
    if (RW == 4) {
        for (int i = 0; i < 8; i++) dst[(size_t)r * K + (size_t)kc * 8 + i] = src[tiled_index(row_off + r, kc * 8 + i, chain, K, RW, NCH)];
        return;
    }
    uint4 v = *(const uint4*)(src + tiled_index(row_off + r, kc * 8, chain, K, RW, NCH));
    *(uint4*)(dst + (size_t)r * K + (size_t)kc * 8) = v;
}
__global__ void synth_fill_kernel(uint16_t* dst, int rows, int K, int row_off, int chain, int RW, int NCH,
                                  uint64_t base, int kind, float sigma) {
    size_t idx = (size_t)blockIdx.x * blockDim.x + threadIdx.x;
    size_t total = (size_t)rows * K;
    if (idx >= total) return;
    int r = (int)(idx / K), k = (int)(idx % K);
    float g = (float)lnb_synth_isum(base, idx) * (1.0f / 53510.0f);
    float v = kind == 1 ? fmaf(0.1f, g, 1.0f) : sigma * g;
    size_t o = RW ? tiled_index(row_off + r, k, chain, K, RW, NCH) : idx;
    dst[o] = bf_trunc(v);
}

#include "lnb_batch_kernels.h"
#include "lnb_knobs.h"

template <class... K> static hipError_t raise_lds_to(int bytes, K... kernels) {
    hipError_t e = hipSuccess;
    ((e = e != hipSuccess ? e : hipFuncSetAttribute((const void*)kernels, hipFuncAttributeMaxDynamicSharedMemorySize, bytes)), ...);
    return e;
}
template <class... K> static hipError_t raise_lds(K... kernels) { return raise_lds_to(160 * 1024, kernels...); }
template <int MIN_HD = 32, class F> static hipError_t with_hd(const AttnParams* p, F&& f) {
    hipError_t e = hipErrorInvalidValue;
    if (!p || p->hd == 128) e = f(std::integral_constant<int, 128>{});
    if (p ? p->hd == 64 : e == hipSuccess) e = f(std::integral_constant<int, 64>{});
    if constexpr (MIN_HD <= 32) if (p ? p->hd == 32 : e == hipSuccess) e = f(std::integral_constant<int, 32>{});
    return e;
}

static size_t xs_bytes(int K, int steps_per_stage) { return ((size_t)((K + steps_per_stage - 1) / steps_per_stage) * steps_per_stage + 320) * 4 + 16; }

template <int RW, int NCH, int SA, int NH, int R, int EPI, bool NORM, int XC>
static hipError_t launch_chain_x(const GemvParams* p, hipStream_t st) {
    auto kfn = gemv_chain_kernel<RW, NCH, SA, NH, R, EPI, NORM, XC>;
    if (!p) return raise_lds(kfn);
    size_t lds = 4 * (size_t)SA + xs_bytes(p->K, SA / (NCH * RW * 2));
    if (lds > 160 * 1024) return hipErrorInvalidValue;
    if (xs_bytes(p->K, SA / (NCH * RW * 2)) / 4 > (size_t)XC * (1 + NH) * 512) return hipErrorInvalidValue;
    if (NORM && (rms_scratch_bytes(rms_nf(NH)) > 4 * (size_t)SA || seq_leaf_size(p->K, rms_nf(NH) * 64) > 256)) return hipErrorInvalidValue;
    hipLaunchKernelGGL(kfn, dim3((unsigned)(p->S * p->n_wg)), dim3((1 + NH) * 64), lds, st, *p);
    return hipGetLastError();
}
template <int RW, int NCH, int SA, int NH, int R, int EPI, bool NORM>
static hipError_t launch_chain_t(const GemvParams* p, hipStream_t st) {
    if constexpr (NORM) {
        if (!p) {
            hipError_t e = launch_chain_x<RW, NCH, SA, NH, R, EPI, NORM, 2>(p, st);
            if (e == hipSuccess) e = launch_chain_x<RW, NCH, SA, NH, R, EPI, NORM, 3>(p, st);
            return e != hipSuccess ? e : launch_chain_x<RW, NCH, SA, NH, R, EPI, NORM, XCh<NORM>::value>(p, st);
        }
        const size_t need = xs_bytes(p->K, SA / (NCH * RW * 2)) / 4, per = (size_t)(1 + NH) * 512;
        if (need <= 2 * per) return launch_chain_x<RW, NCH, SA, NH, R, EPI, NORM, 2>(p, st);
        if (need <= 3 * per) return launch_chain_x<RW, NCH, SA, NH, R, EPI, NORM, 3>(p, st);
    }
    return launch_chain_x<RW, NCH, SA, NH, R, EPI, NORM, XCh<NORM>::value>(p, st);
}

template <int RW, int KS, int NH, int R, int EPI, bool NORM, int XC>
static hipError_t launch_quad_x(const GemvParams* p, hipStream_t st) {
    auto kfn = gemv_quad_kernel<RW, KS, NH, R, EPI, NORM, XC>;
    if (!p) return raise_lds(kfn);
    constexpr int NW = gq_ncw(RW) + NH;
    constexpr size_t SB = (size_t)RW * KS * 4;
    if (p->K % KS) return hipErrorInvalidValue;
    const size_t lds = GQ_SLOTS * SB + xs_bytes(p->K, KS);
    if (lds > 160 * 1024) return hipErrorInvalidValue;
    if (xs_bytes(p->K, KS) / 4 > (size_t)XC * NW * 512) return hipErrorInvalidValue;
    if (NORM && (rms_scratch_bytes(rms_nf(NH)) > GQ_SLOTS * SB || seq_leaf_size(p->K, rms_nf(NH) * 64) > 256)) return hipErrorInvalidValue;
    hipLaunchKernelGGL(kfn, dim3((unsigned)(p->S * p->n_wg)), dim3(NW * 64), lds, st, *p);
    return hipGetLastError();
}
template <int RW, int KS, int NH, int R, int EPI, bool NORM>
static hipError_t launch_quad_t(const GemvParams* p, hipStream_t st) {
    if constexpr (NORM) {
        if (!p) {
            hipError_t e = launch_quad_x<RW, KS, NH, R, EPI, NORM, 2>(p, st);
            return e != hipSuccess ? e : launch_quad_x<RW, KS, NH, R, EPI, NORM, XCh<NORM>::value>(p, st);
        }
        if (xs_bytes(p->K, KS) / 4 <= (size_t)2 * (gq_ncw(RW) + NH) * 512) return launch_quad_x<RW, KS, NH, R, EPI, NORM, 2>(p, st);
    }
    return launch_quad_x<RW, KS, NH, R, EPI, NORM, XCh<NORM>::value>(p, st);
}

template <int EPI, bool NORM, int NCH>
static hipError_t launch_gemv_rw(const GemvParams* p, int rw, hipStream_t st) {
    auto either = [&](bool first, auto a, auto b) { const hipError_t e = (p && !first) ? hipSuccess : a(p, st); return (p ? first : e != hipSuccess) ? e : b(p, st); };
    if constexpr (NCH == 1) if (rw == 24) return either(p && p->sched, launch_quad_t<24, 128, 6, 10, EPI, NORM>, launch_quad_t<24, 256, 6, LNB_QUAD_R, EPI, NORM>);
    if (!NORM && NCH == 1 && (rw == 16 || rw == 32) && (!p || xs_bytes(p->K, 8192 / (rw * 2)) / 4 > (size_t)XCh<false>::value * 3 * 512)) {
        const hipError_t e = rw == 16 ? launch_chain_t<16, 1, 8192, 4, 7, EPI, false>(p, st) : launch_chain_t<32, 1, 8192, 4, 7, EPI, false>(p, st);
        if (p || e != hipSuccess) return e;
    }
    if constexpr (NCH == 1 && !NORM && (EPI == EPI_RESID || EPI == EPI_STORE)) {
        const int quad16 = p ? knob(Knob::W2_QUAD) : 0;
        if (rw == 16 && (!p || (quad16 && p->K % 128 == 0))) {
            const hipError_t e = either(quad16 == 2, launch_quad_t<16, 256, 4, 7, EPI, false>, launch_quad_t<16, 128, 4, 14, EPI, false>);
            if (p || e != hipSuccess) return e;
        }
    }
    if (rw == 16) return launch_chain_t<16, NCH, 8192, 2, 7, EPI, NORM>(p, st);
    if (rw == 32) return (NORM && NCH == 1) ? launch_chain_t<32, 1, 12288, 6, 5, EPI, NORM>(p, st) : launch_chain_t<32, NCH, 8192, 2, 7, EPI, NORM>(p, st);
    if (rw == 64) return launch_chain_t<64, NCH, 12288, 6, 8, EPI, NORM>(p, st);
    if constexpr (NCH == 2) if (rw == 56) return either(p && p->sched && knob(Knob::TP_W13), launch_chain_t<56, 2, 14336, 7, 6, EPI, NORM>, launch_chain_t<56, 2, 14336, 7, 8, EPI, NORM>);
    if constexpr (NCH == 2) if (rw == 28) return launch_chain_t<28, 2, 14336, 7, 8, EPI, NORM>(p, st);
    return hipErrorInvalidValue;
}

template <int EPI> static hipError_t launch_rowcast(const GemvParams* p, hipStream_t st) {
    auto kfn = rowcast_kernel<EPI>;
    auto kl = rowcast_lds_kernel<EPI>;
    if (!p) return raise_lds(kl, kfn);
    if ((p->K & 127) || p->K > 16384) return hipErrorInvalidValue;
    if (knob(Knob::ROWCAST_LDS) && !p->sched && p->K % (128 * RL_SC) == 0 && p->K >= 2 * 128 * RL_SC && rl_lds_bytes(p->K) + (size_t)(p->lds_pad > 0 ? p->lds_pad : 0) <= 160 * 1024) {
        hipLaunchKernelGGL(kl, dim3((unsigned)(p->S * p->n_wg)), dim3(512), rl_lds_bytes(p->K) + (size_t)(p->lds_pad > 0 ? p->lds_pad : 0), st, *p);
        return hipGetLastError();
    }
    hipLaunchKernelGGL(kfn, dim3((unsigned)(p->S * p->n_wg)), dim3(256), (size_t)p->K * 4 + (size_t)(p->lds_pad > 0 ? p->lds_pad : 0), st, *p);
    return hipGetLastError();
}

extern "C" hipError_t lnbk_gemv(const GemvParams* p, int rw, int nch, int epi, int norm, hipStream_t st) {
    if (rw == 4) {
        if (nch != 1 || norm) return hipErrorInvalidValue;
        if (epi == EPI_STORE) return launch_rowcast<EPI_STORE>(p, st);
        if (epi == EPI_RESID) return launch_rowcast<EPI_RESID>(p, st);
        return hipErrorInvalidValue;
    }
    if (nch == 2) {
        if (epi == EPI_SILU_MUL && norm) return launch_gemv_rw<EPI_SILU_MUL, true, 2>(p, rw, st);
        return hipErrorInvalidValue;
    }
    switch (epi) {
        case EPI_STORE: return norm ? launch_gemv_rw<EPI_STORE, true, 1>(p, rw, st) : launch_gemv_rw<EPI_STORE, false, 1>(p, rw, st);
        case EPI_QKV_ROPE: return norm ? launch_gemv_rw<EPI_QKV_ROPE, true, 1>(p, rw, st) : hipErrorInvalidValue;
        case EPI_RESID: return norm ? hipErrorInvalidValue : launch_gemv_rw<EPI_RESID, false, 1>(p, rw, st);
        default: return hipErrorInvalidValue;
    }
}

template <int EPI, int NCH> static hipError_t launch_gemm(const GemmParams* p, hipStream_t st) {
    const struct { void (*k)(GemmParams); size_t lds; } t128{gemm_mfma_kernel<EPI, NCH, 4, 128>, gemm_lds_bytes(NCH, 4)},
        t64{gemm_mfma_kernel<EPI, NCH, 4, 64>, gemm_lds_bytes(NCH, 4, 64)}, t1{gemm_mfma_kernel<EPI, NCH, 1, 128>, gemm_lds_bytes(NCH, 1)};
    hipError_t e = hipSuccess;
    if (!p) { for (const auto& t : {t128, t64, t1}) if (e == hipSuccess) e = raise_lds_to((int)t.lds, t.k); return e; }
    const unsigned mb = (unsigned)((p->S + 127) / 128), nb4 = (unsigned)((p->n_rows + GM_NB - 1) / GM_NB);
    const int force = knob(Knob::GEMM_TILE);
    const int tile = force ? force : (nb4 * mb <= 160 ? 1 : (NCH == 2 && nb4 * mb > 1024) ? 128 : nb4 * mb <= GM_MB64_UPTO ? 64 : 128);
    if (tile == 1)
        hipLaunchKernelGGL(t1.k, dim3((unsigned)((p->n_rows + 15) / 16), mb), dim3(256), t1.lds, st, *p);
    else if (tile == 64)
        hipLaunchKernelGGL(t64.k, dim3(nb4, (unsigned)((p->S + 63) / 64)), dim3(256), t64.lds, st, *p);
    else
        hipLaunchKernelGGL(t128.k, dim3(nb4, mb), dim3(256), t128.lds, st, *p);
    return hipGetLastError();
}

extern "C" hipError_t lnbk_gemm(const GemmParams* p, int epi, hipStream_t st) {
    switch (epi) {
// ... 102 lines not shown
    });
}
static hipError_t launch_attn_short(const AttnParams* p, hipStream_t st) {
    const auto gqa = attn_gqa_kernel<128, 4>;
    const auto dense = attn_exact_kernel<128, true>;
    const size_t lds = p ? attn_lds_bytes(p->lds_T, p->hd) : 0;
    if (!p) { const hipError_t e = raise_lds(gqa, dense); if (e != hipSuccess) return e; }
    else {
        if (lds > 160 * 1024 || p->lds_T <= 0 || p->lds_T > p->seq_len || p->host_T > p->lds_T) return hipErrorInvalidValue;
        if (p->btab && p->hd == 128 && p->H == 4 * p->KVH) {
            const int mode = knob(Knob::ATTN_GQA);
            const size_t gl = gqa_lds_bytes(p->lds_T, 128, 4);
            if (mode != 0 && p->exp_tab && gl <= 160 * 1024 && (mode == 1 || (long)p->KVH * p->S >= 256)) {
                AttnParams q = *p;
                if (knob(Knob::ATTN_GQA_FORCE_ZSEQ)) q.force_zseq = 1;
                if (knob(Knob::ATTN_GQA_DBG)) q.dbg = g_gqa_dbg;
                hipLaunchKernelGGL(gqa, dim3(p->KVH, p->S), dim3(512), gl, st, q);
                return hipGetLastError();
            }
        }
        if (p->btab && p->hd == 128 && (long)p->H * p->S > 256 && knob(Knob::ATTN_BATCH_DENSE)) {
            AttnParams q = *p;
            q.head_major = knob(Knob::ATTN_BATCH_HEADMAJOR) != 0;
            hipLaunchKernelGGL(dense, dim3(p->H, p->S), dim3(ATT_NT), lds, st, q);
            return hipGetLastError();
        }
    }
    return with_hd(p, [&](auto HD) {
        const auto plain = attn_exact_kernel<HD>, append = attn_exact_kernel<HD, false, true>;
        if (!p) return raise_lds(plain, append);
        const auto k = p->causal && !p->btab && p->S > 1 ? append : plain;
        hipLaunchKernelGGL(k, dim3(p->H, p->S), dim3(ATT_NT), lds, st, *p);
        return hipGetLastError();
    });
}
extern "C" hipError_t lnbk_attn(const AttnParams* p, hipStream_t st) {
    if (p->btab && p->longctx) return launch_attn_long<true>(p, st);
    if (p->longctx >= 2 && p->S == 1) return launch_attn_one(p, st);
    if (p->longctx && p->S == 1) return launch_attn_long<false>(p, st);
    if (p->mfma && p->S >= 16 && (p->hd == 128 || p->hd == 64)) return launch_attn_prefill(p, st);
    return launch_attn_short(p, st);
}
extern "C" hipError_t lnbk_init(void) {
    static bool done = false;
    if (done) return hipSuccess;
    hipError_t e = raise_lds(rmsnorm_rows_kernel);
    for (int ep = EPI_STORE; ep <= EPI_SILU_MUL && e == hipSuccess; ep++) e = lnbk_gemm(nullptr, ep, nullptr);
    auto gemv = [&](int rw, int nch, int epi, int norm) { if (e == hipSuccess) e = lnbk_gemv(nullptr, rw, nch, epi, norm, nullptr); };
    gemv(4, 1, EPI_STORE, 0); gemv(4, 1, EPI_RESID, 0); gemv(56, 2, EPI_SILU_MUL, 1); gemv(28, 2, EPI_SILU_MUL, 1);
    for (int rw : {16, 24, 32, 64}) {
        gemv(rw, 1, EPI_STORE, 1); gemv(rw, 1, EPI_STORE, 0); gemv(rw, 1, EPI_QKV_ROPE, 1); gemv(rw, 1, EPI_RESID, 0);
        if (rw != 24) gemv(rw, 2, EPI_SILU_MUL, 1);
    }
    for (auto prepare : {launch_attn_long<true>, launch_attn_long<false>, launch_attn_one, launch_attn_short}) if (e == hipSuccess) e = prepare(nullptr, nullptr);
    if (e == hipSuccess) e = launch_attn_rows(nullptr, -1, nullptr);
    if (e != hipSuccess) return e;
    if (knob(Knob::ATTN_GQA_DBG) && !g_gqa_dbg) { if (hipMalloc(&g_gqa_dbg, 8 * 16 * 8) != hipSuccess) return hipErrorOutOfMemory; (void)hipMemset(g_gqa_dbg, 0, 8 * 16 * 8); }
    done = true;
    return hipSuccess;
}

extern "C" hipError_t lnbk_embed(const uint16_t* emb, const int32_t* tokens, uint16_t* x, int S, int dim, int vocab, int* err, hipStream_t st) {
    hipLaunchKernelGGL(embed_kernel, dim3(S), dim3(256), 0, st, emb, tokens, x, dim, vocab, err);
    return hipGetLastError();
}
extern "C" hipError_t lnbk_argmax(const uint16_t* logits, int V, int32_t* next_token, StepState* state, int32_t* out_tokens,
                                  int out_cap, int advance, hipStream_t st) {
    hipLaunchKernelGGL(argmax_kernel, dim3(1), dim3(1024), 0, st, logits, V, next_token, state, out_tokens, out_cap, advance);
    return hipGetLastError();
}
extern "C" hipError_t lnbk_set_state(StepState* state, int pos, int n_out, int honour_stop, hipStream_t st) {
    hipLaunchKernelGGL(set_state_kernel, dim3(1), dim3(1), 0, st, state, pos, n_out, honour_stop);
    return hipGetLastError();
}
extern "C" hipError_t lnbk_set_stop(StepState* state, const int32_t* ids, int n, hipStream_t st) {
    StopIds s{}; s.n = n; for (int k = 0; k < n && k < LNB_MAX_STOP_IDS; k++) s.id[k] = ids[k];
    hipLaunchKernelGGL(set_stop_kernel, dim3(1), dim3(1), 0, st, state, s);
    return hipGetLastError();
}
extern "C" hipError_t lnbk_advance_state(StepState* state, int rows, hipStream_t st) {
    hipLaunchKernelGGL(advance_state_kernel, dim3(1), dim3(1), 0, st, state, rows);
    return hipGetLastError();
}
extern "C" hipError_t lnbk_tile(const uint16_t* src, uint16_t* dst, int rows, int K, int row_off, int chain, int RW, int NCH, int gather, hipStream_t st) {
    size_t total = (size_t)rows * (K >> 3);
    unsigned blocks = (unsigned)((total + 255) / 256);
    if (gather) hipLaunchKernelGGL(tile_gather_kernel, dim3(blocks), dim3(256), 0, st, src, dst, rows, K, row_off, chain, RW, NCH);
    else hipLaunchKernelGGL(tile_scatter_kernel, dim3(blocks), dim3(256), 0, st, src, dst, rows, K, row_off, chain, RW, NCH);
    return hipGetLastError();
}
extern "C" hipError_t lnbk_synth_fill(uint16_t* dst, int rows, int K, int row_off, int chain, int RW, int NCH,
                                      uint64_t seed, uint32_t tensor_id, int kind, float sigma, hipStream_t st) {
    uint64_t base = lnb_splitmix64(seed + 0x9E3779B97F4A7C15ULL * (uint64_t)(tensor_id + 1u));
    size_t total = (size_t)rows * K;
    unsigned blocks = (unsigned)((total + 255) / 256);
    hipLaunchKernelGGL(synth_fill_kernel, dim3(blocks), dim3(256), 0, st, dst, rows, K, row_off, chain, RW, NCH, base, kind, sigma);
    return hipGetLastError();
}

extern "C" hipError_t lnbk_m16_from_tiled(const uint16_t* src, uint16_t* dst, int rows, int K, int RW, int NCH, hipStream_t st) {
    const size_t total = (size_t)rows * NCH * K;
    hipLaunchKernelGGL(m16_from_tiled_kernel, dim3((unsigned)((total + 255) / 256)), dim3(256), 0, st, src, dst, rows, K, RW, NCH);
    return hipGetLastError();
}
static auto pair_kernel(int epi) -> void (*)(StreamParams) {
    return epi == EPI_STORE ? mfma_pair_kernel<EPI_STORE> : epi == EPI_RESID ? mfma_pair_kernel<EPI_RESID> : epi == EPI_QKV_ROPE ? mfma_pair_kernel<EPI_QKV_ROPE> : nullptr;
// ... 198 lines not shown
```

### llama-nuts-and-bolts_amd/csrc/lnb_knobs.h

```cpp
#pragma once
#include <atomic>
#include <cstdlib>
#define LNB_KNOBS(X) \
     \
    X(RW_QKV, 0, LIVE, "rows per block of the resident wq|wk|wv layout (16 / 24 / 32 / 64; 0: by shape)") \
    X(RW_WO, 0, LIVE, "rows per block of the resident wo layout (4: row-broadcast; 0: by shape)") \
    X(RW_W13, 0, LIVE, "rows per block of the resident gate|up layout (28: the half-height band order, measurement; 0: by shape)") \
    X(RW_W2, 0, LIVE, "rows per block of the resident w2 layout (16 with W2_QUAD: measurement; 0: by shape)") \
    X(RW_OUT, 0, LIVE, "rows per block of the resident LM-head layout (0: by shape)") \
    X(RW_OP, 0, LIVE, "rows per block of a stand-alone lnb_op_linear operand (0: by shape)") \
     \
    X(PREFILL_MFMA, 1, ONCE, "0: calls of 16+ rows stay on the one-row kernels (what the parity tests compare the matrix-core forms with)") \
    X(PREFILL_STREAM, 1, ONCE, "0: prefill products on the LDS-tiled gemm_mfma_kernel, never the streaming feed") \
    X(PREFILL_NATIVE, 1, ONCE, "0: the streaming feed only from the matrix-core copy, not from the resident layouts") \
    X(GEMM_TILE, 0, ONCE, "force the gemm_mfma_kernel tile: 1 (16-row) / 64 / 128; 0: by tile count") \
    X(GS_NTW, 0, LIVE, "force gemm_stream_kernel's batch tiles per wave: 1 / 2 / 4") \
    X(GS_NTW_CHAIN, 0, ONCE, "the same, for the chain layouts only") \
    X(GS_TT, -1, LIVE, "two weight tiles per wave in gemm_stream_kernel: 0 never, 1 whenever the form exists, -1 by workgroup count") \
    X(GS_ORDER, -1, ONCE, "gemm_stream_kernel dispatch order: 1 row groups fastest, 0 tile groups fastest, -1 by row-group count") \
    X(GEMM_BLGP, 0, LIVE, "1 / 2: chain-layout prefill products through gemm_blgp_kernel (bit-exact, measured slower)") \
    X(NORM_ROWS_WIDE, 1, ONCE, "0: prefill RMSNorm on the one-wave rmsnorm_rows_kernel") \
    X(ATTN_MFMA2, 0, LIVE, "N > 0: prefill attention of N+ rows on the two-tile attn_mfma2_kernel (measured slower); 0: never") \
    X(ATTN_SIDX_MB, 4096, LIVE, "largest score-index scratch (MiB) the scores-kept prefill attention may allocate") \
    X(ATTN_SIDX_KEEP_MB, 256, LIVE, "a score-index scratch above this (MiB) is given back at the next one-token call") \
    X(OP_STREAM, 0, LIVE, "1: lnb_op_linear of 16+ rows through gemm_stream_kernel (tests)") \
     \
    X(ATTN_LONG_T, 512, LIVE, "context length from which a new context decodes with the long-context attention kernels") \
    X(ATTN_ONE, 0, ONCE, "1: long-context decode attention in one launch (attn_one_kernel; measured slower); a context beyond lnb_ctx_create's capacity keeps the two launches") \
    X(ATTN_LAZY, 1, LIVE, "0: the long-context PV pass without the lazy certificate (attn_long_pv_kernel); a context beyond lnb_ctx_create's capacity keeps the lazy one") \
    X(ATTN_TOUCH, 1, LIVE, "0: the long-context scores pass does not touch V ahead of the PV pass (A/B)") \
    X(ATTN_ROWS_RPW, 4, ONCE, "query rows per PV workgroup of the multi-row long-context attention (attn_rows_pv_kernel): 1, 2 or 4 -- any other value makes the calls that would run it fail with a message naming this knob") \
     \
    X(BATCH_GROUPS, 1, ONCE, "0: 17..32 sequences decode as rows, not as two column groups") \
    X(STREAM_PAIR, 1, LIVE, "0: thin batched products on the one-wave mfma_stream_kernel, not mfma_pair_kernel") \
    X(ATTN_GQA, -1, LIVE, "batched decode attention per (KV head, sequence): 0 never, 1 always, -1 from 256 workgroups on") \
    X(ATTN_GQA_FORCE_ZSEQ, 0, LIVE, "1: every head of attn_gqa_kernel walks the serial denominator (tests)") \
    X(ATTN_BATCH_DENSE, 1, LIVE, "0: batched decode attention never takes the dense-dispatch attn_exact_kernel form") \
    X(ATTN_BATCH_HEADMAJOR, 0, LIVE, "1: that form dispatches head-major (A/B)") \
    X(APPEND_MANY_COLS, 128, LIVE, "columns per pass of lnb_forward_append_many (1..128; any other value makes the call fail with a message naming this knob): tests reach every width form and the pass boundary with few rows, the bench sweeps it") \
     \
    X(FORK_COPY, 0, LIVE, "1: lnb_ctx_fork on the copy engine (hipMemcpy2DAsync per layer and destination, no kernel launch): the comparison kv_fork_kernel has to beat (2.5x slower at 4096 positions into 127 contexts, 7.6 - 52x at 128 positions, 1.4x at its best: no crossover), and a cross-check on its bits") \
    X(FORK_NT, 0, LIVE, "1: kv_fork_kernel with non-temporal loads and stores (measurement: from 3 % faster to 20 % slower than the plain form)") \
    X(FORK_SPLIT, 0, LIVE, "N > 1: kv_fork_kernel deals the destinations over N workgroup groups, each reading the source (measurement: slower from 1024 positions on)") \
     \
    X(FAST_GEMM_MIN_ROWS, 192, ONCE, "rows from which the tolerance mode uses its bf16 GEMM instead of the exact one") \
    X(FAST_GEMM_2WG, -1, ONCE, "bf16 GEMM batch tile: 1 = 128 rows and two workgroups per CU, 0 = 256 rows, -1 by row count") \
    X(FAST_RG, 0, ONCE, "force the rows per unit of the split-K GEMV: 8 / 16 / 32 / 64") \
    X(FAST_GRID_CAP, 2048, ONCE, "largest grid.x of the split-K GEMV") \
     \
    X(PIPELINE_GRAPH, 1, LIVE, "0: pipeline stages launch eagerly instead of replaying captured graphs") \
    X(PIPELINE_LOG_CAP, 1 << 16, LIVE, "entries of a pipeline stage's event log ring (the wrap-around test shrinks it)") \
     \
    X(NO_GRAPH, 0, LIVE, "1: greedy and batched decode launch every step eagerly") \
    X(GEMV_TIMING, 0, LIVE, "1: lnb_profile_kernel dumps the per-wave stamps of the profiled launch") \
    X(PROFILE_SAME_LAYER, 0, LIVE, "1: lnb_profile_kernel stays on one layer (weights served from the Infinity Cache)") \
    X(MEASURE_SKIP_TOKEN_KERNELS, 0, LIVE, "1: the decode step without its embedding and argmax launches (timing only: tokens are garbage)") \
    X(ROWCAST_LDS, 1, ONCE, "0: the row-broadcast GEMV always on the self-feeding rowcast_kernel") \
    X(TP_W13, 1, ONCE, "0: the throughput schedule keeps the eight-stage gate|up kernel (A/B)") \
    X(W2_QUAD, 0, LIVE, "1 / 2: a 16-row w2 layout on gemv_quad_kernel with 128- / 256-step stages (measurement only)") \
    X(W2_PRIO, 0, LIVE, "wave priority handed to the w2 launch of a block (measurement)") \
    X(W2_LDS_PAD, 28 * 1024, LIVE, "LDS padding of the w2 launch in the profiled w1|w3 + w2 pair (measurement)") \
    X(ATTN_GQA_DBG, 0, LIVE, "1: attn_gqa_kernel stamps the phases of one workgroup (lnbk_attn_gqa_dbg_dump prints them)")
enum KnobLife { ONCE, LIVE };
// ... 16 lines not shown
```

### llama-nuts-and-bolts_amd/lnb.py

```python
import ctypes as C
import os
import subprocess

import numpy as np

_HERE = os.path.dirname(os.path.abspath(__file__))
_SO = os.environ.get("LNB_SO") or os.path.join(_HERE, "liblnb_hip.so")
_CSRC = os.path.join(_HERE, "csrc")


MODE_EXACT, MODE_FAST = 0, 1


class LnbError(RuntimeError):
    pass


def build(force=False):
    srcs = [os.path.join(_CSRC, f) for f in os.listdir(_CSRC) if f.endswith((".hip", ".cpp", ".h", ".hpp")) or f == "Makefile"]
    srcs.append(os.path.join(_HERE, "..", "include", "lnb.h"))
    if os.environ.get("LNB_SO"):
        return _SO
    if force or not os.path.exists(_SO) or any(os.path.getmtime(s) > os.path.getmtime(_SO) for s in srcs):
        subprocess.check_call(["make", "-C", _CSRC, "-s"])
    return _SO


class ModelArgs(C.Structure):
    _fields_ = [("dim", C.c_int32), ("n_layers", C.c_int32), ("n_heads", C.c_int32), ("n_kv_heads", C.c_int32),
                ("vocab_size", C.c_int32), ("multiple_of", C.c_int32), ("ffn_dim_multiplier", C.c_double),
                ("norm_eps", C.c_float), ("use_scaled_rope", C.c_int32), ("rope_theta", C.c_double),
                ("max_seq_len", C.c_int32)]


LLAMA_8B = dict(dim=4096, n_layers=32, n_heads=32, n_kv_heads=8, vocab_size=128256, multiple_of=1024,
                ffn_dim_multiplier=1.3, norm_eps=1e-5, use_scaled_rope=1, rope_theta=500000.0, max_seq_len=2048)

_lib = None
EXPORTS = [
    "lnb_last_error", "lnb_device_count", "lnb_device_info", "lnb_device_can_access_peer", "lnb_device_pci_bus_id", "lnb_model_create", "lnb_model_create_parts", "lnb_model_destroy", "lnb_model_ffn_hidden_dim",
    "lnb_model_set_tensor", "lnb_model_get_tensor", "lnb_model_fill_synthetic", "lnb_model_finalize",
    "lnb_model_rope_table", "lnb_model_weight_bytes", "lnb_ctx_create", "lnb_ctx_destroy", "lnb_ctx_reset",
    "lnb_ctx_read_kv", "lnb_ctx_set_layer_callback", "lnb_forward", "lnb_decode_greedy", "lnb_ctx_hidden_ptr",
    "lnb_forward_stage", "lnb_forward_stage_begin", "lnb_forward_stage_end", "lnb_ctx_synchronize", "lnb_ctx_stream", "lnb_op_linear", "lnb_op_rmsnorm_linear", "lnb_op_argmax", "lnb_op_exp_table", "lnb_op_linear_mode", "lnb_ctx_set_mode", "lnb_ctx_get_mode", "lnb_ctx_set_schedule", "lnb_ctx_get_schedule", "lnb_ctx_set_attention", "lnb_ctx_zseq_count", "lnb_ctx_norm_fallbacks", "lnb_ctx_prefill_attention_form",
    "lnb_profile_kernel", "lnb_profile_kernel_stamps", "lnb_model_num_tensors", "lnb_model_tensor_info",
    "lnb_checkpoint_open", "lnb_checkpoint_close", "lnb_checkpoint_num_tensors", "lnb_checkpoint_find", "lnb_checkpoint_tensor",
    "lnb_model_load_checkpoint", "lnb_model_args_from_json",
    "lnb_tokenizer_load", "lnb_tokenizer_free", "lnb_tokenizer_vocab_size", "lnb_tokenizer_special", "lnb_tokenizer_token_id",
    "lnb_tokenizer_piece", "lnb_tokenizer_encode", "lnb_tokenizer_encode_chat",
    "lnb_tokenizer_stream_create", "lnb_tokenizer_stream_free", "lnb_tokenizer_decode_stream", "lnb_tokenizer_stream_pending",
    "lnb_pipeline_unique_id", "lnb_pipeline_init", "lnb_pipeline_init_loopback", "lnb_pipeline_destroy", "lnb_pipeline_tick", "lnb_pipeline_sync", "lnb_pipeline_read_tokens", "lnb_pipeline_selftest", "lnb_pipeline_comm_count",
    "lnb_model_enable_batch", "lnb_model_batch_bytes", "lnb_batch_create", "lnb_batch_destroy", "lnb_batch_decode", "lnb_batch_decode_until", "lnb_ctx_set_stop_ids", "lnb_decode_greedy_until", "lnb_batch_profile_kernel", "lnb_batch_set_state", "lnb_batch_check_error", "lnb_pipeline_tick_batch",
    "lnb_pipeline_init_host", "lnb_batch_boundary_ptr",
    "lnb_abi_version", "lnb_runtime_info", "lnb_profile_ffn_pair",
    "lnb_ctx_set_token_probs", "lnb_ctx_read_token_probs", "lnb_ctx_token_prob_walks", "lnb_forward_score", "lnb_op_token_probs",
    "lnb_forward_append", "lnb_forward_score_append",
    "lnb_ctx_set_draft", "lnb_decode_speculative_until", "lnb_op_ngram_draft",
    "lnb_batch_set_attention", "lnb_ctx_set_batched_attention", "lnb_batch_attention_form", "lnb_ctx_verify_attention_form",
    "lnb_ctx_create_long", "lnb_ctx_max_rows",
    "lnb_ctx_set_rows_attention", "lnb_ctx_append_attention_form",
    "lnb_ctx_fork", "lnb_ctx_prefix_bytes", "lnb_ctx_save_prefix", "lnb_ctx_load_prefix",
    "lnb_forward_append_many", "lnb_model_append_many_info",
    "lnb_decode_speculative_many",
]
MAX_TOP_K = 16
MAX_DRAFT = 15
MAX_SEQ_LEN = 131072
MAX_FORK = 128
ABI_VERSION = 6


class SpecStats(C.Structure):
    _fields_ = [("passes", C.c_int64), ("verify_passes", C.c_int64), ("drafted", C.c_int64), ("accepted", C.c_int64)]

    def as_dict(self):
        return {n: int(getattr(self, n)) for n, _ in self._fields_}


class SpecManyInfo(C.Structure):
    _fields_ = [("passes", C.c_int64), ("verify_passes", C.c_int64), ("columns", C.c_int64), ("max_columns", C.c_int64), ("long_passes", C.c_int64)]

    def as_dict(self):
        return {n: int(getattr(self, n)) for n, _ in self._fields_}


class RuntimeInfo(C.Structure):
    _fields_ = [("abi_version", C.c_int32), ("device", C.c_int32), ("n_cus", C.c_int32),
                ("shader_clock_khz", C.c_int32), ("memory_clock_khz", C.c_int32), ("wall_clock_khz", C.c_int32),
                ("hw_queues_env", C.c_int32), ("hw_queues_set_by_library", C.c_int32), ("hip_initialised_before_load", C.c_int32),
                ("hw_queues_expected", C.c_int32), ("hw_queues_measured", C.c_int32), ("probe_ms", C.c_float),
                ("device_name", C.c_char * 64), ("arch", C.c_char * 32)]



def lib():
    global _lib
    if _lib is not None:
        return _lib
    if not os.path.exists(_SO):
        raise LnbError("liblnb_hip.so is not built (run __graft_entry__.build()); there is no fallback path")
    L = C.CDLL(_SO)
    vp, i32p, f32p = C.c_void_p, C.POINTER(C.c_int32), C.POINTER(C.c_float)
    if not hasattr(L, "lnb_abi_version") or L.lnb_abi_version() != ABI_VERSION:
        raise LnbError("liblnb_hip.so reports ABI version %s, this binding is written against %d: rebuild the library (make -C csrc)"
                       % (L.lnb_abi_version() if hasattr(L, "lnb_abi_version") else "none", ABI_VERSION))
    L.lnb_runtime_info.argtypes = [C.c_int, C.c_int, C.POINTER(RuntimeInfo)]
    L.lnb_profile_ffn_pair.argtypes = [vp, C.c_int, C.c_int, C.c_int, C.c_int, f32p]
# ... 6 lines not shown
    L.lnb_model_create_parts.argtypes = [C.POINTER(ModelArgs), C.c_int, C.c_int, C.c_int, C.POINTER(vp)]
    L.lnb_model_destroy.argtypes = [vp]
    L.lnb_model_ffn_hidden_dim.argtypes = [C.POINTER(ModelArgs)]
    L.lnb_model_set_tensor.argtypes = [vp, C.c_char_p, vp, C.POINTER(C.c_int64), C.c_int]
    L.lnb_model_get_tensor.argtypes = [vp, C.c_char_p, vp, C.c_int64]
    L.lnb_model_fill_synthetic.argtypes = [vp, C.c_uint64]
    L.lnb_model_finalize.argtypes = [vp, C.c_int]
    L.lnb_model_rope_table.argtypes = [vp, vp, C.c_int64, C.POINTER(C.c_int)]
    L.lnb_model_weight_bytes.argtypes = [vp]
    L.lnb_model_weight_bytes.restype = C.c_int64
    L.lnb_ctx_create.argtypes = [vp, C.c_int, C.POINTER(vp)]
    L.lnb_ctx_create_long.argtypes = [vp, C.c_int, C.c_int, C.POINTER(vp)]
    L.lnb_ctx_max_rows.argtypes = [vp, C.POINTER(C.c_int)]
    L.lnb_ctx_destroy.argtypes = [vp]
    L.lnb_ctx_reset.argtypes = [vp]
    L.lnb_ctx_read_kv.argtypes = [vp, C.c_int, C.c_int, vp]
    L.lnb_ctx_set_layer_callback.argtypes = [vp, vp, vp]
    L.lnb_forward.argtypes = [vp, vp, C.c_int, C.c_int, vp, i32p]
    L.lnb_decode_greedy.argtypes = [vp, C.c_int32, C.c_int, C.c_int, vp, f32p]
    L.lnb_ctx_hidden_ptr.argtypes = [vp, C.c_int]
    L.lnb_ctx_hidden_ptr.restype = vp
    L.lnb_forward_stage.argtypes = [vp, vp, C.c_int, C.c_int, vp, i32p]
    L.lnb_forward_stage_begin.argtypes = [vp, vp, C.c_int, C.c_int, C.c_int]
    L.lnb_forward_stage_end.argtypes = [vp, i32p]
    L.lnb_ctx_synchronize.argtypes = [vp]
    L.lnb_ctx_stream.argtypes = [vp]
    L.lnb_ctx_stream.restype = vp
    L.lnb_profile_kernel.argtypes = [vp, C.c_int, C.c_int, C.c_int, f32p]
    L.lnb_profile_kernel_stamps.argtypes = [vp, C.c_int, C.c_int, vp, C.POINTER(C.c_int)]
    L.lnb_op_linear.argtypes = [C.c_int, vp, vp, vp, C.c_int, C.c_int, C.c_int, C.c_int]
    L.lnb_op_rmsnorm_linear.argtypes = [C.c_int, vp, vp, C.c_float, vp, vp, C.c_int, C.c_int, C.c_int, C.c_int]
    L.lnb_ctx_set_mode.argtypes = [vp, C.c_int]
    L.lnb_ctx_get_mode.argtypes = [vp]
    L.lnb_ctx_set_schedule.argtypes = [vp, C.c_int]
    L.lnb_ctx_get_schedule.argtypes = [vp]
    L.lnb_ctx_set_attention.argtypes = [vp, C.c_int, C.c_int]
    L.lnb_ctx_zseq_count.argtypes = [vp, C.POINTER(C.c_int)]
    L.lnb_ctx_norm_fallbacks.argtypes = [vp, C.POINTER(C.c_int)]
    L.lnb_ctx_prefill_attention_form.argtypes = [vp, C.POINTER(C.c_int)]
    L.lnb_pipeline_unique_id.argtypes = [vp]
    L.lnb_pipeline_init.argtypes = [vp, C.c_int, C.c_int, vp, C.POINTER(vp)]
    L.lnb_pipeline_init_loopback.argtypes = [vp, C.c_int, C.c_int, C.c_char_p, C.POINTER(vp)]
    L.lnb_pipeline_init_host.argtypes = [vp, C.c_int, C.c_int, C.POINTER(vp)]
    L.lnb_batch_boundary_ptr.argtypes = [vp, C.c_int]
    L.lnb_batch_boundary_ptr.restype = C.c_void_p
    L.lnb_pipeline_selftest.argtypes = [C.c_int, C.c_int]
    L.lnb_pipeline_destroy.argtypes = [vp]
    L.lnb_pipeline_tick.argtypes = [vp, vp, C.c_int, C.c_int, vp, vp, C.c_int, vp, C.c_int, C.POINTER(C.c_int)]
    L.lnb_pipeline_sync.argtypes = [vp]
    L.lnb_pipeline_comm_count.argtypes = [vp, C.POINTER(C.c_int)]
    L.lnb_model_enable_batch.argtypes = [vp]
    L.lnb_model_batch_bytes.argtypes = [vp]
    L.lnb_model_batch_bytes.restype = C.c_int64
    L.lnb_batch_create.argtypes = [C.POINTER(vp), C.c_int, C.POINTER(vp)]
    L.lnb_batch_destroy.argtypes = [vp]
    L.lnb_batch_decode.argtypes = [vp, i32p, i32p, C.c_int, vp, f32p]
    L.lnb_batch_decode_until.argtypes = [vp, i32p, i32p, C.c_int, vp, vp, vp, f32p]
    L.lnb_ctx_set_stop_ids.argtypes = [vp, vp, C.c_int]
    L.lnb_decode_greedy_until.argtypes = [vp, C.c_int32, C.c_int, C.c_int, vp, C.POINTER(C.c_int), C.POINTER(C.c_int), f32p]
    L.lnb_batch_profile_kernel.argtypes = [vp, C.c_int, C.c_int, C.c_int, f32p]
    L.lnb_batch_set_state.argtypes = [vp, i32p, i32p]
    L.lnb_batch_check_error.argtypes = [vp]
    L.lnb_batch_set_attention.argtypes = [vp, C.c_int, C.c_int]
    L.lnb_ctx_set_batched_attention.argtypes = [vp, C.c_int, C.c_int]
    L.lnb_batch_attention_form.argtypes = [vp, C.POINTER(C.c_int)]
    L.lnb_ctx_verify_attention_form.argtypes = [vp, C.POINTER(C.c_int)]
    L.lnb_ctx_set_rows_attention.argtypes = [vp, C.c_int, C.c_int]
    L.lnb_ctx_append_attention_form.argtypes = [vp, C.POINTER(C.c_int)]
    L.lnb_ctx_fork.argtypes = [vp, C.c_int, C.POINTER(vp), C.c_int]
    L.lnb_ctx_prefix_bytes.argtypes = [vp, C.c_int]
    L.lnb_ctx_prefix_bytes.restype = C.c_int64
    L.lnb_ctx_save_prefix.argtypes = [vp, C.c_int, vp, C.c_int64]
    L.lnb_ctx_load_prefix.argtypes = [vp, vp, C.c_int64, C.POINTER(C.c_int)]
    L.lnb_forward_append_many.argtypes = [C.POINTER(vp), C.c_int, vp, vp, vp, vp, vp]
    L.lnb_model_append_many_info.argtypes = [vp, C.POINTER(C.c_int), C.POINTER(C.c_int), C.POINTER(C.c_int)]
    L.lnb_decode_speculative_many.argtypes = [C.POINTER(vp), C.c_int, C.POINTER(vp), vp, vp, vp, C.c_int, C.c_int, vp, vp, vp,
                                              C.POINTER(SpecStats), C.POINTER(SpecManyInfo), f32p]
    L.lnb_pipeline_tick_batch.argtypes = [vp, vp, vp, vp, C.POINTER(C.c_int)]
    L.lnb_pipeline_read_tokens.argtypes = [vp, C.c_int, C.c_int, vp]
    L.lnb_op_linear_mode.argtypes = [C.c_int, vp, vp, C.c_float, vp, vp, C.c_int, C.c_int, C.c_int, C.c_int, C.c_int]
    L.lnb_op_argmax.argtypes = [C.c_int, vp, C.c_int, i32p]
    L.lnb_op_exp_table.argtypes = [C.c_int, C.c_float, vp]
    L.lnb_ctx_set_token_probs.argtypes = [vp, C.c_int]
    L.lnb_ctx_read_token_probs.argtypes = [vp, C.c_int, C.c_int, vp, vp, vp, vp]
    L.lnb_ctx_token_prob_walks.argtypes = [vp, C.POINTER(C.c_int)]
    L.lnb_forward_score.argtypes = [vp, vp, C.c_int, C.c_int, vp, vp, vp, vp, i32p]
    L.lnb_forward_append.argtypes = [vp, vp, C.c_int, C.c_int, vp, i32p]
    L.lnb_forward_score_append.argtypes = [vp, vp, C.c_int, C.c_int, vp, vp, vp, vp, i32p]
    L.lnb_op_token_probs.argtypes = [C.c_int, vp, C.c_int, C.c_int, C.c_int, vp, C.c_int, vp, vp, vp, vp, vp, C.POINTER(C.c_int)]
    L.lnb_ctx_set_draft.argtypes = [vp, C.c_int, C.c_int, C.c_int, vp, C.c_int]
    L.lnb_decode_speculative_until.argtypes = [vp, vp, C.c_int, C.c_int32, C.c_int, C.c_int, vp, C.POINTER(C.c_int), C.POINTER(C.c_int),
                                               C.POINTER(SpecStats), f32p]
    L.lnb_op_ngram_draft.argtypes = [C.c_int, vp, C.c_int, vp, C.c_int, C.c_int, C.c_int, C.c_int, vp, C.POINTER(C.c_int)]
    L.lnb_model_num_tensors.argtypes = [vp]
    L.lnb_model_tensor_info.argtypes = [vp, C.c_int, C.POINTER(C.c_char_p), C.POINTER(C.c_int64), C.POINTER(C.c_int)]
    L.lnb_checkpoint_open.argtypes = [C.c_char_p, C.POINTER(vp)]
    L.lnb_checkpoint_close.argtypes = [vp]
    L.lnb_checkpoint_close.restype = None
    L.lnb_checkpoint_num_tensors.argtypes = [vp]
    L.lnb_checkpoint_find.argtypes = [vp, C.c_char_p]
    L.lnb_checkpoint_tensor.argtypes = [vp, C.c_int, C.POINTER(C.c_char_p), C.POINTER(C.c_int), C.POINTER(C.c_int64), C.POINTER(C.c_int),
                                        C.POINTER(vp), C.POINTER(C.c_int64)]
    L.lnb_model_load_checkpoint.argtypes = [vp, vp]
    L.lnb_model_args_from_json.argtypes = [C.c_char_p, C.POINTER(ModelArgs)]
    L.lnb_tokenizer_load.argtypes = [C.c_char_p, C.POINTER(vp)]
    L.lnb_tokenizer_free.argtypes = [vp]
# ... 191 lines not shown
        _chk(self.L.lnb_model_create_parts(C.byref(self.args), device, self.part_begin, self.part_end, C.byref(self.h)))
        self.ffn_hidden = self.L.lnb_model_ffn_hidden_dim(C.byref(self.args))
        self.head_dim = self.args.dim // self.args.n_heads

    def set_tensor(self, name, arr_u16, shape=None):
        a = np.ascontiguousarray(arr_u16, dtype=np.uint16)
        shp = tuple(shape) if shape is not None else a.shape
        s = (C.c_int64 * len(shp))(*shp)
        _chk(self.L.lnb_model_set_tensor(self.h, name.encode(), _p(a), s, len(shp)))

    def get_tensor(self, name, nelem):
        out = np.empty(nelem, dtype=np.uint16)
        _chk(self.L.lnb_model_get_tensor(self.h, name.encode(), _p(out), nelem))
        return out

    def fill_synthetic(self, seed=1234):
        _chk(self.L.lnb_model_fill_synthetic(self.h, seed))
        return self

    def load_checkpoint(self, ckpt):
        _chk(self.L.lnb_model_load_checkpoint(self.h, ckpt.h))
        return self

    def tensor_infos(self):
        out = []
        for k in range(self.L.lnb_model_num_tensors(self.h)):
            name, shape, rank = C.c_char_p(), (C.c_int64 * 2)(), C.c_int()
            _chk(self.L.lnb_model_tensor_info(self.h, k, C.byref(name), shape, C.byref(rank)))
            out.append((name.value.decode(), tuple(shape[:rank.value])))
        return out

    def finalize(self, rope_rows=0):
        _chk(self.L.lnb_model_finalize(self.h, rope_rows))
        return self

    @property
    def PrecomputedFreqsCis(self):
        rows = C.c_int(0)
        _chk(self.L.lnb_model_rope_table(self.h, None, 0, C.byref(rows)))
        out = np.empty((rows.value, self.head_dim // 2, 2), dtype=np.float32)
        _chk(self.L.lnb_model_rope_table(self.h, _p(out), out.size, C.byref(rows)))
        return out

    def weight_bytes(self):
        return int(self.L.lnb_model_weight_bytes(self.h))

    def enable_batch(self):
        _chk(self.L.lnb_model_enable_batch(self.h))
        return self

    def batch_bytes(self):
        return int(self.L.lnb_model_batch_bytes(self.h))

    def append_many_info(self):
        p, w, g = C.c_int(0), C.c_int(0), C.c_int(0)
        _chk(self.L.lnb_model_append_many_info(self.h, C.byref(p), C.byref(w), C.byref(g)))
        return {"passes": p.value, "max_columns": w.value, "long_passes": g.value}

    def close(self):
        if self.h:
            self.L.lnb_model_destroy(self.h)
            self.h = C.c_void_p()


class InferenceContext:

    def __init__(self, transformer, seq_len, max_rows=None, long_context=False):
        self.t, self.L = transformer, transformer.L
        self.SequenceLength = seq_len
        self.h = C.c_void_p()
        if long_context or max_rows is not None:
            _chk(self.L.lnb_ctx_create_long(transformer.h, seq_len, int(max_rows or 0), C.byref(self.h)))
        else:
            _chk(self.L.lnb_ctx_create(transformer.h, seq_len, C.byref(self.h)))

    def max_rows(self):
        n = C.c_int(0)
        _chk(self.L.lnb_ctx_max_rows(self.h, C.byref(n)))
        return n.value

    def set_mode(self, mode):
        _chk(self.L.lnb_ctx_set_mode(self.h, {"exact": 0, "fast": 1}.get(mode, mode)))
        return self

    def set_schedule(self, sched):
        _chk(self.L.lnb_ctx_set_schedule(self.h, {"latency": 0, "throughput": 1}.get(sched, sched)))
        return self

    def set_attention(self, long_threshold=-1, force_zseq=0):
        _chk(self.L.lnb_ctx_set_attention(self.h, long_threshold, force_zseq))
        return self

    def zseq_count(self):
        n = C.c_int(0)
        _chk(self.L.lnb_ctx_zseq_count(self.h, C.byref(n)))
        return n.value

    def norm_fallbacks(self):
        n = C.c_int(0)
        _chk(self.L.lnb_ctx_norm_fallbacks(self.h, C.byref(n)))
        return n.value

    def prefill_attention_form(self):
        n = C.c_int(0)
        _chk(self.L.lnb_ctx_prefill_attention_form(self.h, C.byref(n)))
        return n.value
# ... 388 lines not shown
    _chk(lib().lnb_op_argmax(device, _p(a), a.size, C.byref(out)))
    return out.value


def op_token_probs(logits_u16, top_k, targets=None, force_serial=False, device=0):
    a = np.ascontiguousarray(logits_u16, dtype=np.uint16)
    if a.ndim == 1:
        a = a[None, :]
    rows, V = a.shape
    k = int(top_k)
    ids = np.empty((rows, max(k, 1)), dtype=np.int32)
    lg = np.empty((rows, max(k, 1)), dtype=np.float32)
    pr = np.empty((rows, max(k, 1)), dtype=np.float32)
    lz = np.empty(rows, dtype=np.float64)
    tg = None if targets is None else np.ascontiguousarray(targets, dtype=np.int32)
    tp = np.empty(rows, dtype=np.float32)
    walks = C.c_int(0)
    _chk(lib().lnb_op_token_probs(device, _p(a), rows, V, k, None if tg is None else _p(tg), 1 if force_serial else 0,
                                  _p(ids), _p(lg), _p(pr), _p(tp) if tg is not None else None, _p(lz), C.byref(walks)))
    out = dict(ids=ids[:, :k], logits=lg[:, :k], probs=pr[:, :k], log_z=lz, serial_walks=walks.value)
    if tg is not None:
        out["target_prob"] = tp
    return out


def op_ngram_draft(text, corpus=(), ngram_min=1, ngram_max=4, max_draft=MAX_DRAFT, device=0):
    t = np.ascontiguousarray(text, dtype=np.int32)
    c = np.ascontiguousarray(corpus, dtype=np.int32)
    out = np.empty(max(int(max_draft), 1), dtype=np.int32)
    n = C.c_int(0)
    _chk(lib().lnb_op_ngram_draft(device, _p(t) if t.size else None, int(t.size), _p(c) if c.size else None, int(c.size),
                                  int(ngram_min), int(ngram_max), int(max_draft), _p(out), C.byref(n)))
    return out[:n.value].copy()


def op_exp_table(divisor=1.0, device=0):
    out = np.empty(65536, dtype=np.float64)
    _chk(lib().lnb_op_exp_table(device, C.c_float(divisor), _p(out)))
    return out


_M64 = (1 << 64) - 1


def _splitmix64(z):
    z = (z + 0x9E3779B97F4A7C15) & _M64
    z = ((z ^ (z >> 30)) * 0xBF58476D1CE4E5B9) & _M64
    z = ((z ^ (z >> 27)) * 0x94D049BB133111EB) & _M64
    return z ^ (z >> 31)


def synth_tokens(seed, n, vocab):
    return np.array([_splitmix64(seed ^ ((i * 0x9E3779B97F4A7C15) & _M64)) % vocab for i in range(n)], dtype=np.int32)
```

Measured before the change: 238.4 tokens/s.

## Stream gate|up weights from a lossless 13-bit packed copy in one-token decode

At finalize time the build makes a second copy of each layer's w13 (gate|up) matrix packed at 13 bits per weight: 8 low bits, a 4-bit exponent code relative to a per-matrix base, and 1 sign bit. It first checks that the matrix's exponent range fits a 16-value window and holds no subnormals or inf/NaN. A new gemv kernel variant reads this packed copy and rebuilds the exact bf16 values in registers, so single-token exact-mode latency steps move about 19% fewer bytes for the FFN up projection, which is the largest weight stream. The cost is extra HBM for the packed copy, more ALU work to unpack, refresh logic whenever tensors are rebound, and a fallback to raw weights when the window check fails.

```diff
diff --git a/include/lnb.h b/include/lnb.h
--- a/include/lnb.h
+++ b/include/lnb.h
@@ -128,6 +128,8 @@
 typedef struct lnb_batch lnb_batch;
 int lnb_model_enable_batch(lnb_model* m);
 int64_t lnb_model_batch_bytes(lnb_model* m);
+int64_t lnb_model_wpack_bytes(lnb_model* m);
+int lnb_model_wpack_info(lnb_model* m, int32_t* counts6);
 int lnb_batch_create(lnb_ctx* const* ctxs, int n, lnb_batch** out);
 int lnb_batch_destroy(lnb_batch* b);
 int lnb_batch_decode(lnb_batch* b, const int32_t* tokens, const int32_t* start_pos, int n_steps, int32_t* out_tokens, float* ms_out);
@@ -169,6 +171,8 @@
 int lnb_op_linear(int device, const uint16_t* x, const uint16_t* w, uint16_t* y, int rows, int n_out, int k_in, int rw);
 int lnb_op_rmsnorm_linear(int device, const uint16_t* x, const uint16_t* norm_w, float eps, const uint16_t* w,
                           uint16_t* y, int rows, int n_out, int k_in, int rw);
+int lnb_op_rmsnorm_gate_up(int device, const uint16_t* x, const uint16_t* norm_w, float eps, const uint16_t* w1, const uint16_t* w3, uint16_t* y,
+                           int n_out, int k_in, int packed, int* status);
 
 int lnb_op_linear_mode(int device, const uint16_t* x, const uint16_t* norm_w, float eps, const uint16_t* w, uint16_t* y,
                        int rows, int n_out, int k_in, int rw, int mode);
diff --git a/llama-nuts-and-bolts_amd/csrc/lnb_api.cpp b/llama-nuts-and-bolts_amd/csrc/lnb_api.cpp
--- a/llama-nuts-and-bolts_amd/csrc/lnb_api.cpp
+++ b/llama-nuts-and-bolts_amd/csrc/lnb_api.cpp
@@ -19,6 +19,7 @@
 #include "lnb_knobs.h"
 #include "lnb_kvcopy.h"
 #include "lnb_rowpack.h"
+#include "lnb_wpack.h"
 #include "lnb_batchplan.h"
 #include "lnb_rccl.h"
 static_assert(LNB_MAX_SEQ_LEN == LNB_SEQ_MAX, "lnb.h and lnb_device.h disagree on the longest context");
@@ -47,6 +48,11 @@
 hipError_t lnbk_tile(const uint16_t* src, uint16_t* dst, int rows, int K, int row_off, int chain, int RW, int NCH, int gather, hipStream_t st);
 hipError_t lnbk_synth_fill(uint16_t* dst, int rows, int K, int row_off, int chain, int RW, int NCH, uint64_t seed, uint32_t tensor_id, int kind, float sigma, hipStream_t st);
 hipError_t lnbk_init(void);
+int lnbk_w13p_supported(int rw, int K);
+hipError_t lnbk_gemv_w13p(const GemvParams* p, hipStream_t st);
+size_t lnbk_wpack_w13_bytes(int n_blocks, int K);
+hipError_t lnbk_wpack_stats(const uint16_t* w, size_t elems, unsigned* d_stats, hipStream_t st);
+hipError_t lnbk_wpack_w13(const uint16_t* w, void* out, int K, int n_blocks, unsigned base, hipStream_t st);
 hipError_t lnbk_fast_gemv(const GemvParams* p, int rw, int nch, int epi, int norm, hipStream_t st);
 hipError_t lnbk_fast_gemm(const GemmParams* p, int epi, hipStream_t st);
 hipError_t lnbk_fast_attn(const AttnParams* p, hipStream_t st);
@@ -121,6 +127,8 @@
     uint16_t* attn_norm = nullptr; uint16_t* ffn_norm = nullptr;
     TiledDesc wqkv{}, wo{}, w13{}, w2{};
     uint16_t *m_wqkv = nullptr, *m_wo = nullptr, *m_w13 = nullptr, *m_w2 = nullptr;
+    void* p_w13 = nullptr; unsigned p_base = 0; bool p_ok = false;
+    int p_status = -1;
 };
 struct lnb_model {
     lnb_model_args a{};
@@ -137,6 +145,7 @@
     bool finalized = false;
     int64_t weight_bytes = 0;
     bool batch_enabled = false; uint16_t* m_output = nullptr; int64_t batch_bytes = 0;
+    int64_t wpack_bytes = 0;
     std::mutex am_mu; struct AppendMany* am = nullptr;
     bool first() const { return part_begin == 0; }
     bool last() const { return part_end == 3 * a.n_layers; }
@@ -374,6 +383,7 @@
     *out = m;
     return 0;
 }
+static int wpack_refresh(lnb_model* m, const TiledDesc* t);
 static int model_alloc(lnb_model* m) {
     const lnb_model_args& a = m->a;
     const int layer_begin = m->layer_begin, layer_end = m->layer_end;
@@ -432,7 +442,7 @@
     if (m->output.w) hipFree(m->output.w);
     for (auto& L : m->layers) {
         hipFree(L.attn_norm); hipFree(L.ffn_norm); hipFree(L.wqkv.w); hipFree(L.wo.w); hipFree(L.w13.w); hipFree(L.w2.w);
-        hipFree(L.m_wqkv); hipFree(L.m_wo); hipFree(L.m_w13); hipFree(L.m_w2);
+        hipFree(L.m_wqkv); hipFree(L.m_wo); hipFree(L.m_w13); hipFree(L.m_w2); hipFree(L.p_w13);
     }
     hipFree(m->m_output);
     if (m->cis) hipFree(m->cis);
@@ -445,6 +455,76 @@
 }
 
 extern "C" int64_t lnb_model_weight_bytes(lnb_model* m) { return m ? m->weight_bytes : 0; }
+
+static int wpack_matrix_window(lnb_model* m, const TiledDesc& t, unsigned* d_stats, unsigned* base) {
+    HIPCHK(lnbk_wpack_stats(t.w, tiled_elems(t.n_rows, t.k, t.rw, t.nch), d_stats, m->stream));
+    WpackStats s;
+    HIPCHK(hipMemcpyAsync(&s, d_stats, sizeof s, hipMemcpyDeviceToHost, m->stream));
+    HIPCHK(hipStreamSynchronize(m->stream));
+    return wpack_window(&s, base);
+}
+static int wpack_build(lnb_model* m) {
+    unsigned* d_stats = nullptr;
+    for (int l = m->layer_begin; l < m->layer_end; l++) {
+        LayerW& L = m->layers[l - m->layer_begin];
+        if (!m->has_w13(l) || L.p_ok || L.w13.nch != 2 || !lnbk_w13p_supported(L.w13.rw, L.w13.k)) continue;
+        if (!d_stats) HIPCHK(hipMalloc((void**)&d_stats, sizeof(WpackStats)));
+        unsigned base = 0;
+        const int why = wpack_matrix_window(m, L.w13, d_stats, &base);
+        if (why < 0) { hipFree(d_stats); return -1; }
+        L.p_status = why;
+        if (why != WPACK_OK) continue;
+        const size_t n = lnbk_wpack_w13_bytes(L.w13.n_blocks, L.w13.k);
+        if (!L.p_w13) {
+            if (hipMalloc(&L.p_w13, n) != hipSuccess) { (void)hipGetLastError(); L.p_w13 = nullptr; L.p_status = WPACK_NOMEM; continue; }
+            m->wpack_bytes += (int64_t)n;
+        }
+        hipError_t e = lnbk_wpack_w13(L.w13.w, L.p_w13, L.w13.k, L.w13.n_blocks, base, m->stream);
+        if (e == hipSuccess) e = hipStreamSynchronize(m->stream);
+        if (e != hipSuccess) { hipFree(d_stats); return fail("packing the gate|up matrix of layer %d failed: %s", l, hipGetErrorString(e)); }
+        L.p_base = base; L.p_ok = true;
+    }
+    hipFree(d_stats);
+    return 0;
+}
+static int wpack_refresh(lnb_model* m, const TiledDesc* t) {
+    unsigned* d_stats = nullptr; int rc = 0;
+    for (int l = m->layer_begin; l < m->layer_end && !rc; l++) {
+        LayerW& L = m->layers[l - m->layer_begin];
+        if (!L.p_ok || (t && t != &L.w13)) continue;
+        if (!d_stats && hipMalloc((void**)&d_stats, sizeof(WpackStats)) != hipSuccess) { (void)hipGetLastError(); L.p_ok = false; rc = fail("out of memory"); break; }
+        L.p_ok = false;
+        HIPCHK(lnbk_wpack_stats(L.w13.w, tiled_elems(L.w13.n_rows, L.w13.k, L.w13.rw, L.w13.nch), d_stats, m->stream));
+        WpackStats s;
+        HIPCHK(hipMemcpyAsync(&s, d_stats, sizeof s, hipMemcpyDeviceToHost, m->stream));
+        HIPCHK(hipStreamSynchronize(m->stream));
+        unsigned base = 0;
+        const int why = wpack_window(&s, &base);
+        const bool fits = why == WPACK_OK && (s.max_e2 == 0 || (s.min_e2 > L.p_base && s.max_e2 <= L.p_base + 15));
+        if (!fits) {
+            L.p_status = why != WPACK_OK ? why : WPACK_WINDOW;
+            rc = fail("layer %d: the gate|up weights bound after lnb_model_finalize do not fit the window of the matrix's 13-bit copy; the layer decodes from the raw "
+                      "weights from now on (a decode step captured before keeps the old copy: bind every tensor before lnb_model_finalize)", l);
+            break;
+        }
+        HIPCHK(lnbk_wpack_w13(L.w13.w, L.p_w13, L.w13.k, L.w13.n_blocks, L.p_base, m->stream));
+        HIPCHK(hipStreamSynchronize(m->stream));
+        L.p_ok = true; L.p_status = WPACK_OK;
+    }
+    hipFree(d_stats);
+    return rc;
+}
+extern "C" int64_t lnb_model_wpack_bytes(lnb_model* m) { return m ? m->wpack_bytes : 0; }
+extern "C" int lnb_model_wpack_info(lnb_model* m, int32_t* counts6) {
+    if (!m || !counts6) return fail("null argument");
+    for (int i = 0; i < 6; i++) counts6[i] = 0;
+    for (int l = m->layer_begin; l < m->layer_end; l++) {
+        const LayerW& L = m->layers[l - m->layer_begin];
+        if (!m->has_w13(l)) continue;
+        counts6[L.p_ok ? 0 : (L.p_status > 0 && L.p_status <= WPACK_NOMEM) ? L.p_status : 5]++;
+    }
+    return 0;
+}
 
 extern "C" int lnb_model_set_tensor(lnb_model* m, const char* name, const uint16_t* host, const int64_t* shape, int rank) {
     if (!m || !name || !host || !shape) return fail("null argument");
@@ -464,6 +544,7 @@
     if (e == hipSuccess) e = hipStreamSynchronize(m->stream);
     hipFree(stage);
     HIPCHK(e);
+    if (wpack_refresh(m, r.td)) return -1;
     return 0;
 }
 
@@ -507,6 +588,7 @@
         else HIPCHK(lnbk_synth_fill(r.linear, r.rows, r.cols, 0, 0, 0, 1, seed, r.synth_id, r.synth_kind, 0.02f, m->stream));
     }
     HIPCHK(hipStreamSynchronize(m->stream));
+    if (wpack_refresh(m, nullptr)) return -1;
     return 0;
 }
 
@@ -571,6 +653,7 @@
     if (!m->exp_tab) HIPCHK(hipMalloc((void**)&m->exp_tab, (size_t)(1 << 16) * 8));
     HIPCHK(lnbk_exp_table(m->exp_tab, bf_wide_h(bf_trunc_h((float)std::sqrt((double)m->head_dim))), m->stream));
     HIPCHK(hipStreamSynchronize(m->stream));
+    if (knob(Knob::W13_PACKED) && wpack_build(m)) return -1;
     m->finalized = true;
     return 0;
 }
@@ -1001,7 +1084,9 @@
     case K_W13: {
         GemvParams f{}; f.w = L.w13.w; f.x = hbuf; f.norm_w = L.ffn_norm; f.norm_fb = c->zseq_count + 1; f.eps = a.norm_eps; f.K = a.dim; f.n_rows = m->ffn_hidden; f.S = S; f.st = c->st;
         f.out = c->ffn; f.silu = m->silu; f.sched = c->sched;
-        set_grid(f, L.w13); HIPCHK(gemv_dispatch(c, &f, L.w13.rw, 2, EPI_SILU_MUL, 1, st)); return 0; }
+        set_grid(f, L.w13);
+        if (S == 1 && L.p_ok && c->mode == LNB_MODE_EXACT && c->sched == LNB_SCHED_LATENCY) { f.wp = L.p_w13; f.wp_base4 = L.p_base * 0x01010101u; HIPCHK(lnbk_gemv_w13p(&f, st)); return 0; }
+        HIPCHK(gemv_dispatch(c, &f, L.w13.rw, 2, EPI_SILU_MUL, 1, st)); return 0; }
     case K_W2: {
         GemvParams d{}; d.w = L.w2.w; d.x = c->ffn; d.K = m->ffn_hidden; d.n_rows = a.dim; d.S = S; d.st = c->st; d.out = c->x; d.res = hbuf; d.lds_pad = lds_pad; d.sched = c->sched; d.prio = knob(Knob::W2_PRIO);
         set_grid(d, L.w2); HIPCHK(gemv_dispatch(c, &d, L.w2.rw, 1, EPI_RESID, 0, st)); return 0; }
@@ -3058,6 +3143,48 @@
     HIPCHK(hipDeviceSynchronize());
     HIPCHK(hipMemcpy(y, dy, (size_t)rows * n_out * 2, hipMemcpyDeviceToHost));
     hipFree(dx); hipFree(dw); hipFree(dy); hipFree(st); hipFree(t.w); if (dn) hipFree(dn); if (t.w16) hipFree(t.w16);
+    return 0;
+}
+extern "C" int lnb_op_rmsnorm_gate_up(int device, const uint16_t* x, const uint16_t* norm_w, float eps, const uint16_t* w1, const uint16_t* w3, uint16_t* y,
+                                      int n_out, int k_in, int packed, int* status) {
+    if (!x || !norm_w || !w1 || !w3 || !y) return fail("null argument");
+    if (n_out <= 0 || k_in <= 0) return fail("empty operand");
+    if (k_in % 8) return fail("in_features must be a multiple of 8");
+    int ndev = 0; HIPCHK(hipGetDeviceCount(&ndev));
+    if (ndev == 0) return fail("no HIP device: liblnb_hip.so has no CPU fallback");
+    HIPCHK(hipSetDevice(device));
+    HIPCHK(lnbk_init());
+    if (!lnbk_w13p_supported(56, k_in)) return fail("in_features %d does not fit the LDS staging of the 56-row gate|up kernel", k_in);
+    TiledDesc t{}; int64_t bytes = 0;
+    if (alloc_tiled(t, n_out, k_in, 56, 2, bytes)) return -1;
+    const size_t wn = (size_t)n_out * k_in * 2;
+    uint16_t *dx = nullptr, *dw = nullptr, *dy = nullptr, *dn = nullptr; StepState* st = nullptr; float* dsilu = nullptr; unsigned* dstats = nullptr; void* wp = nullptr;
+    HIPCHK(hipMalloc((void**)&dx, (size_t)k_in * 2)); HIPCHK(hipMalloc((void**)&dw, wn)); HIPCHK(hipMalloc((void**)&dn, (size_t)k_in * 2));
+    HIPCHK(hipMalloc((void**)&dy, (size_t)n_out * 2)); HIPCHK(hipMalloc((void**)&st, sizeof(StepState))); HIPCHK(hipMalloc((void**)&dsilu, (size_t)65536 * 4));
+    HIPCHK(hipMalloc((void**)&dstats, sizeof(WpackStats)));
+    HIPCHK(hipMemset(st, 0, sizeof(StepState)));
+    std::vector<float> silu(1 << 16);
+    for (int i = 0; i < (1 << 16); i++) { double v = (double)bf_wide_h((uint16_t)i); silu[i] = (float)(v / (1.0 + std::exp(-v))); }
+    HIPCHK(hipMemcpy(dsilu, silu.data(), silu.size() * 4, hipMemcpyHostToDevice));
+    HIPCHK(hipMemcpy(dx, x, (size_t)k_in * 2, hipMemcpyHostToDevice)); HIPCHK(hipMemcpy(dn, norm_w, (size_t)k_in * 2, hipMemcpyHostToDevice));
+    HIPCHK(hipMemcpy(dw, w1, wn, hipMemcpyHostToDevice)); HIPCHK(lnbk_tile(dw, t.w, n_out, k_in, 0, 0, 56, 2, 0, nullptr)); HIPCHK(hipDeviceSynchronize());
+    HIPCHK(hipMemcpy(dw, w3, wn, hipMemcpyHostToDevice)); HIPCHK(lnbk_tile(dw, t.w, n_out, k_in, 0, 1, 56, 2, 0, nullptr)); HIPCHK(hipDeviceSynchronize());
+    HIPCHK(lnbk_wpack_stats(t.w, tiled_elems(n_out, k_in, 56, 2), dstats, nullptr));
+    WpackStats ws; HIPCHK(hipMemcpy(&ws, dstats, sizeof ws, hipMemcpyDeviceToHost));
+    unsigned base = 0;
+    const int why = wpack_window(&ws, &base);
+    if (status) *status = why;
+    GemvParams g{}; g.w = t.w; g.x = dx; g.norm_w = dn; g.eps = eps; g.K = k_in; g.n_rows = n_out; g.S = 1; g.st = st; g.out = dy; g.silu = dsilu;
+    set_grid(g, t);
+    if (packed && why == WPACK_OK) {
+        HIPCHK(hipMalloc(&wp, lnbk_wpack_w13_bytes(t.n_blocks, k_in)));
+        HIPCHK(lnbk_wpack_w13(t.w, wp, k_in, t.n_blocks, base, nullptr));
+        g.wp = wp; g.wp_base4 = base * 0x01010101u;
+        HIPCHK(lnbk_gemv_w13p(&g, nullptr));
+    } else HIPCHK(lnbk_gemv(&g, 56, 2, EPI_SILU_MUL, 1, nullptr));
+    HIPCHK(hipDeviceSynchronize());
+    HIPCHK(hipMemcpy(y, dy, (size_t)n_out * 2, hipMemcpyDeviceToHost));
+    hipFree(dx); hipFree(dw); hipFree(dy); hipFree(dn); hipFree(st); hipFree(dsilu); hipFree(dstats); hipFree(t.w); if (wp) hipFree(wp);
     return 0;
 }
 extern "C" int lnb_op_argmax(int device, const uint16_t* logits_bf16, int n, int32_t* out) {
diff --git a/llama-nuts-and-bolts_amd/csrc/lnb_device.h b/llama-nuts-and-bolts_amd/csrc/lnb_device.h
--- a/llama-nuts-and-bolts_amd/csrc/lnb_device.h
+++ b/llama-nuts-and-bolts_amd/csrc/lnb_device.h
@@ -79,6 +79,8 @@
     int lds_pad;
     int prio;
     int sched;
+    const void* wp;
+    unsigned wp_base4;
 };
 
 struct GemmParams {
diff --git a/llama-nuts-and-bolts_amd/csrc/lnb_kernels.hip b/llama-nuts-and-bolts_amd/csrc/lnb_kernels.hip
--- a/llama-nuts-and-bolts_amd/csrc/lnb_kernels.hip
+++ b/llama-nuts-and-bolts_amd/csrc/lnb_kernels.hip
@@ -3,6 +3,7 @@
 #include <type_traits>
 #include "lnb_device.h"
 #include "lnb_seqsum.h"
+#include "lnb_wpack.h"
 
 #define DEVINL __device__ __forceinline__
 
@@ -441,6 +442,10 @@
 
 typedef unsigned int u32x4 __attribute__((ext_vector_type(4)));
 DEVINL void ld_nt_asm(u32x4& dst, unsigned voff, const char* sbase) { asm volatile("global_load_dwordx4 %0, %1, %2 nt ; RING_LOAD" : "=&v"(dst) : "v"(voff), "s"(sbase) : "memory"); }
+DEVINL void ld_nt_asm4(unsigned& dst, unsigned voff, const char* sbase) { asm volatile("global_load_dword %0, %1, %2 nt ; RING_LOAD" : "=&v"(dst) : "v"(voff), "s"(sbase) : "memory"); }
+template <int N> DEVINL void wait_ring_pk(u32x4 (&b)[4], unsigned& s) {
+    asm volatile("s_waitcnt vmcnt(%4) ; RING_RETIRE %0 %1 %2 %3" : "+v"(b[0]), "+v"(b[1]), "+v"(b[2]), "+v"(s) : "n"(N) : "memory");
+}
 template <int N, int NP> DEVINL void wait_ring(u32x4 (&b)[NP]) {
     static_assert(NP == 1 || NP == 2 || NP == 4 || NP == 8, "loads per stage per helper");
     if constexpr (NP == 1) asm volatile("s_waitcnt vmcnt(%1) ; RING_RETIRE %0" : "+v"(b[0]) : "n"(N) : "memory");
@@ -449,8 +454,8 @@
     if constexpr (NP == 8) asm volatile("s_waitcnt vmcnt(%8) ; RING_RETIRE %0 %1 %2 %3 %4 %5 %6 %7" : "+v"(b[0]), "+v"(b[1]), "+v"(b[2]), "+v"(b[3]), "+v"(b[4]), "+v"(b[5]), "+v"(b[6]), "+v"(b[7]) : "n"(N) : "memory");
 }
 
-template <int RW, int NCH, int SA, int NH, int R, int EPI, bool NORM, int XC = XCh<NORM>::value>
-__global__ __launch_bounds__((1 + NH) * 64) void gemv_chain_kernel(GemvParams p) {
+template <int RW, int NCH, int SA, int NH, int R, int EPI, bool NORM, int XC, bool PK>
+DEVINL void gemv_chain_body(const GemvParams& p) {
     extern __shared__ __attribute__((aligned(16))) char smem[];
     long long t_begin = p.dbg ? clock64() : 0, t_wait = 0, t_x = 0, t_aux = 0;
     const long long t_wall0 = p.dbg ? (long long)wall_clock64() : 0;
@@ -462,6 +467,7 @@
     static_assert(KC >= 2 && (KC & 1) == 0, "bad stage geometry");
     static_assert(UNITS % (64 * NH) == 0 && R * NP <= 60, "vmcnt is a 6-bit counter");
     static_assert(NH >= 2, "x staging is sized for >= 3 stager waves");
+    static_assert(!PK || (NCH == 2 && NP == 4 && 2 * NH * 64 == KC * RW), "packed source: one 32-weight group (two (chunk, row) pairs x two chains) per helper lane and stage");
     char* ringB = smem;
     float* xs = (float*)(smem + 2 * SB);
 
@@ -482,6 +488,7 @@
     if (wave != CW) {
         const int hw = wave < CW ? wave : wave - 1;
         u32x4 buf[R][NP];
+        unsigned sgn[PK ? R : 1];
         {
             uint4 xv[XC], nv[XC];
             x_issue<NORM, NS>(p, xrow, 1 + hw, lane, xv, nv);
@@ -495,7 +502,15 @@
             loff[i] = NCH == 2 ? (unsigned)((((pq / RW) * 2 + (i & 1)) * RW + (pq % RW)) * 16) : (unsigned)(((i * NH + hw) * 64 + lane) * 16);
         }
         int ib = wg, is = 0, issued = 0;
-        auto issue_next = [&](u32x4 (&dst)[NP]) {
+        const unsigned pk_l16 = (unsigned)((hw * 64 + lane) * 16), pk_l4 = (unsigned)(NH * 64 * 48 + (hw * 64 + lane) * 4);
+        auto issue_next = [&](u32x4 (&dst)[NP], unsigned& sg) {
+            if constexpr (PK) {
+                const char* sb = (const char*)p.wp + ((size_t)ib * nstages + is) * wpack_stage_bytes(NH * 64);
+                ld_nt_asm(dst[0], pk_l16, sb); ld_nt_asm(dst[1], pk_l16 + NH * 64 * 16, sb); ld_nt_asm(dst[2], pk_l16 + NH * 64 * 32, sb);
+                ld_nt_asm4(sg, pk_l4, sb);
+                if (issued + 1 < T) { issued++; if (++is == nstages) { is = 0; ib += p.n_wg; } }
+                return;
+            }
             const size_t soff = (size_t)is * SA;
             const char* sb = (const char*)p.w + (size_t)ib * stream_bytes + soff;
             const unsigned lim = (soff + SA <= stream_bytes) ? 0xFFFFFFFFu : (unsigned)(last16 - soff);
@@ -507,7 +522,7 @@
             constexpr int EARLY_ = NCH == 2 ? LNB_EARLY_W13 : LNB_EARLY_HEAD;
             constexpr int EARLY = late ? (EARLY_ < R ? EARLY_ : R) : R;
 #pragma unroll
-            for (int j = 0; j < EARLY; j++) issue_next(buf[j]);
+            for (int j = 0; j < EARLY; j++) issue_next(buf[j], sgn[PK ? j : 0]);
             x_store<NORM, NS>(p, xs, kpad, 1 + hw, lane, xv);
             __builtin_amdgcn_fence(__ATOMIC_RELEASE, "workgroup");
             TIMED_BARRIER();
@@ -516,7 +531,7 @@
                 rms_fold<rms_nf(NH)>(p, xs, ringB, hw - (NH - rms_nf(NH)), lane, t_aux);
                 {
 #pragma unroll
-                    for (int j = EARLY; j < R; j++) issue_next(buf[j]);
+                    for (int j = EARLY; j < R; j++) issue_next(buf[j], sgn[PK ? j : 0]);
                 }
                 TIMED_BARRIER();
                 __builtin_amdgcn_fence(__ATOMIC_ACQUIRE, "workgroup");
@@ -533,11 +548,32 @@
                 if (t <= T) {
                     if (t < T) {
                         const long long tb_ = p.dbg_full ? clock64() : 0;
-                        wait_ring<(R - 1) * NP, NP>(buf[j]);
+                        if constexpr (PK) wait_ring_pk<(R - 1) * 4>(buf[j], sgn[j]);
+                        else wait_ring<(R - 1) * NP, NP>(buf[j]);
                         if (p.dbg_full) t_x += clock64() - tb_;
                         char* dst = ringB + (t & 1) * SB;
                         const float* xst = xs + (size_t)st * (KC * 8);
-                        if constexpr (NCH == 2) {
+                        if constexpr (PK) {
+                            const unsigned base4 = p.wp_base4, sg = sgn[j];
+#pragma unroll
+                            for (int pi = 0; pi < 2; pi++) {
+                                const int pq = (pi * NH + hw) * 64 + lane, kc = pq / RW, r = pq % RW;
+                                const float4 xa = *(const float4*)(xst + kc * 8), xb = *(const float4*)(xst + kc * 8 + 4);
+                                const u32x4 lo = buf[j][pi];
+                                const unsigned cg = pi ? buf[j][2].z : buf[j][2].x, cu = pi ? buf[j][2].w : buf[j][2].y;
+                                const unsigned hg0 = wpack_hi4(wpack_spread(cg, 0), sg, 4 * pi + 0, base4), hg1 = wpack_hi4(wpack_spread(cg, 1), sg, 4 * pi + 1, base4);
+                                const unsigned hu0 = wpack_hi4(wpack_spread(cu, 0), sg, 4 * pi + 2, base4), hu1 = wpack_hi4(wpack_spread(cu, 1), sg, 4 * pi + 3, base4);
+#define LNB_WIDE4(h, l) __uint_as_float(wpack_wide<0>(h, l)), __uint_as_float(wpack_wide<1>(h, l)), __uint_as_float(wpack_wide<2>(h, l)), __uint_as_float(wpack_wide<3>(h, l))
+                                const float4 ga = mul4(xa, LNB_WIDE4(hg0, lo.x)), gb = mul4(xb, LNB_WIDE4(hg1, lo.y));
+                                const float4 ua = mul4(xa, LNB_WIDE4(hu0, lo.z)), ub = mul4(xb, LNB_WIDE4(hu1, lo.w));
+#undef LNB_WIDE4
+                                char* d = dst + r * 16;
+                                *(float4*)(d + ((4 * kc + 0) * RW) * 16) = make_float4(ga.x, ua.x, ga.y, ua.y);
+                                *(float4*)(d + ((4 * kc + 1) * RW) * 16) = make_float4(ga.z, ua.z, ga.w, ua.w);
+                                *(float4*)(d + ((4 * kc + 2) * RW) * 16) = make_float4(gb.x, ub.x, gb.y, ub.y);
+                                *(float4*)(d + ((4 * kc + 3) * RW) * 16) = make_float4(gb.z, ub.z, gb.w, ub.w);
+                            }
+                        } else if constexpr (NCH == 2) {
 #pragma unroll
                             for (int pi = 0; pi < NP / 2; pi++) {
                                 const int pq = (pi * NH + hw) * 64 + lane, kc = pq / RW, r = pq % RW;
@@ -570,7 +606,7 @@
                         }
                         if (++st == nstages) st = 0;
                         __builtin_amdgcn_sched_barrier(0);
-                        issue_next(buf[j]);
+                        issue_next(buf[j], sgn[PK ? j : 0]);
                     }
                     __builtin_amdgcn_fence(__ATOMIC_RELEASE, "workgroup");
                     TIMED_BARRIER();
@@ -660,6 +696,10 @@
     }
     DBG_EXIT();
 }
+template <int RW, int NCH, int SA, int NH, int R, int EPI, bool NORM, int XC = XCh<NORM>::value>
+__global__ __launch_bounds__((1 + NH) * 64) void gemv_chain_kernel(GemvParams p) { gemv_chain_body<RW, NCH, SA, NH, R, EPI, NORM, XC, false>(p); }
+template <int RW, int NCH, int SA, int NH, int R, int EPI, bool NORM, int XC = XCh<NORM>::value>
+__global__ __launch_bounds__((1 + NH) * 64) void gemv_chain_pk_kernel(GemvParams p) { gemv_chain_body<RW, NCH, SA, NH, R, EPI, NORM, XC, true>(p); }
 
 #define LNB_QP(j) " quad_perm:[" #j "," #j "," #j "," #j "] row_mask:0xf bank_mask:0xf\n\t"
 #define LNB_QADD4(j) "v_add_f32_dpp %0, %1, %0" LNB_QP(j) "v_add_f32_dpp %0, %2, %0" LNB_QP(j) "v_add_f32_dpp %0, %3, %0" LNB_QP(j) "v_add_f32_dpp %0, %4, %0" LNB_QP(j)
@@ -3692,6 +3732,41 @@
     dst[o] = bf_trunc(v);
 }
 
+__global__ void wpack_stats_kernel(const uint16_t* w, size_t n_units, unsigned* stats) {
+    __shared__ unsigned sh[4];
+    if (threadIdx.x == 0) { sh[0] = 0xFFu; sh[1] = sh[2] = sh[3] = 0; }
+    __syncthreads();
+    WpackStats s; wpack_stats_init(&s);
+    for (size_t u = (size_t)blockIdx.x * blockDim.x + threadIdx.x; u < n_units; u += (size_t)gridDim.x * blockDim.x) {
+        const uint4 v = *(const uint4*)(w + u * 8);
+        const uint16_t* e = (const uint16_t*)&v;
+#pragma unroll
+        for (int i = 0; i < 8; i++) wpack_stats_add(&s, e[i]);
+    }
+    atomicMin(&sh[0], s.min_e2); atomicMax(&sh[1], s.max_e2); if (s.subnormal) atomicOr(&sh[2], 1u); if (s.infnan) atomicOr(&sh[3], 1u);
+    __syncthreads();
+    if (threadIdx.x == 0) { atomicMin(&stats[0], sh[0]); atomicMax(&stats[1], sh[1]); if (sh[2]) atomicOr(&stats[2], 1u); if (sh[3]) atomicOr(&stats[3], 1u); }
+}
+__global__ void wpack_pack_kernel(const uint16_t* w, char* out, int K, int rw, int lanes, int n_blocks, unsigned base) {
+    const int nst = wpack_stages(K, lanes, rw), kcs = 2 * lanes / rw;
+    const size_t idx = (size_t)blockIdx.x * blockDim.x + threadIdx.x;
+    if (idx >= (size_t)n_blocks * nst * lanes) return;
+    const int L = (int)(idx % lanes), st = (int)((idx / lanes) % nst), b = (int)(idx / ((size_t)lanes * nst));
+    uint4 g[4];
+#pragma unroll
+    for (int u = 0; u < 4; u++) {
+        const int pq = (u >> 1) * lanes + L, kcg = st * kcs + pq / rw, r = pq % rw;
+        g[u] = kcg < (K >> 3) ? *(const uint4*)(w + ((((size_t)b * (K >> 3) + kcg) * 2 + (u & 1)) * rw + r) * 8) : make_uint4(0, 0, 0, 0);
+    }
+    uint32_t low8[8], code4[4], sg;
+    wpack_pack_group((const uint16_t*)g, base, low8, code4, &sg);
+    char* o = out + ((size_t)b * nst + st) * wpack_stage_bytes(lanes);
+    *(uint4*)(o + (size_t)L * 16) = make_uint4(low8[0], low8[1], low8[2], low8[3]);
+    *(uint4*)(o + (size_t)lanes * 16 + (size_t)L * 16) = make_uint4(low8[4], low8[5], low8[6], low8[7]);
+    *(uint4*)(o + (size_t)lanes * 32 + (size_t)L * 16) = make_uint4(code4[0], code4[1], code4[2], code4[3]);
+    *(uint32_t*)(o + (size_t)lanes * 48 + (size_t)L * 4) = sg;
+}
+
 #include "lnb_batch_kernels.h"
 #include "lnb_knobs.h"
 
@@ -3711,9 +3786,10 @@
 
 static size_t xs_bytes(int K, int steps_per_stage) { return ((size_t)((K + steps_per_stage - 1) / steps_per_stage) * steps_per_stage + 320) * 4 + 16; }
 
-template <int RW, int NCH, int SA, int NH, int R, int EPI, bool NORM, int XC>
+template <int RW, int NCH, int SA, int NH, int R, int EPI, bool NORM, int XC, bool PK = false>
 static hipError_t launch_chain_x(const GemvParams* p, hipStream_t st) {
-    auto kfn = gemv_chain_kernel<RW, NCH, SA, NH, R, EPI, NORM, XC>;
+    void (*kfn)(GemvParams);
+    if constexpr (PK) kfn = gemv_chain_pk_kernel<RW, NCH, SA, NH, R, EPI, NORM, XC>; else kfn = gemv_chain_kernel<RW, NCH, SA, NH, R, EPI, NORM, XC>;
     if (!p) return raise_lds(kfn);
     size_t lds = 4 * (size_t)SA + xs_bytes(p->K, SA / (NCH * RW * 2));
     if (lds > 160 * 1024) return hipErrorInvalidValue;
@@ -3722,19 +3798,19 @@
     hipLaunchKernelGGL(kfn, dim3((unsigned)(p->S * p->n_wg)), dim3((1 + NH) * 64), lds, st, *p);
     return hipGetLastError();
 }
-template <int RW, int NCH, int SA, int NH, int R, int EPI, bool NORM>
+template <int RW, int NCH, int SA, int NH, int R, int EPI, bool NORM, bool PK = false>
 static hipError_t launch_chain_t(const GemvParams* p, hipStream_t st) {
     if constexpr (NORM) {
         if (!p) {
-            hipError_t e = launch_chain_x<RW, NCH, SA, NH, R, EPI, NORM, 2>(p, st);
-            if (e == hipSuccess) e = launch_chain_x<RW, NCH, SA, NH, R, EPI, NORM, 3>(p, st);
-            return e != hipSuccess ? e : launch_chain_x<RW, NCH, SA, NH, R, EPI, NORM, XCh<NORM>::value>(p, st);
+            hipError_t e = launch_chain_x<RW, NCH, SA, NH, R, EPI, NORM, 2, PK>(p, st);
+            if (e == hipSuccess) e = launch_chain_x<RW, NCH, SA, NH, R, EPI, NORM, 3, PK>(p, st);
+            return e != hipSuccess ? e : launch_chain_x<RW, NCH, SA, NH, R, EPI, NORM, XCh<NORM>::value, PK>(p, st);
         }
         const size_t need = xs_bytes(p->K, SA / (NCH * RW * 2)) / 4, per = (size_t)(1 + NH) * 512;
-        if (need <= 2 * per) return launch_chain_x<RW, NCH, SA, NH, R, EPI, NORM, 2>(p, st);
-        if (need <= 3 * per) return launch_chain_x<RW, NCH, SA, NH, R, EPI, NORM, 3>(p, st);
-    }
-    return launch_chain_x<RW, NCH, SA, NH, R, EPI, NORM, XCh<NORM>::value>(p, st);
+        if (need <= 2 * per) return launch_chain_x<RW, NCH, SA, NH, R, EPI, NORM, 2, PK>(p, st);
+        if (need <= 3 * per) return launch_chain_x<RW, NCH, SA, NH, R, EPI, NORM, 3, PK>(p, st);
+    }
+    return launch_chain_x<RW, NCH, SA, NH, R, EPI, NORM, XCh<NORM>::value, PK>(p, st);
 }
 
 template <int RW, int KS, int NH, int R, int EPI, bool NORM, int XC>
@@ -3784,6 +3860,31 @@
     if constexpr (NCH == 2) if (rw == 56) return either(p && p->sched && knob(Knob::TP_W13), launch_chain_t<56, 2, 14336, 7, 6, EPI, NORM>, launch_chain_t<56, 2, 14336, 7, 8, EPI, NORM>);
     if constexpr (NCH == 2) if (rw == 28) return launch_chain_t<28, 2, 14336, 7, 8, EPI, NORM>(p, st);
     return hipErrorInvalidValue;
+}
+
+#ifndef LNB_W13P_R
+#define LNB_W13P_R 5
+#endif
+#define WPACK_LANES_W13 (7 * 64)
+extern "C" int lnbk_w13p_supported(int rw, int K) {
+    return rw == 56 && K > 0 && K % 8 == 0 && 4 * (size_t)28672 + xs_bytes(K, 128) <= 160 * 1024 && xs_bytes(K, 128) / 4 <= (size_t)XCh<true>::value * 8 * 512 && seq_leaf_size(K, rms_nf(7) * 64) <= 256;
+}
+extern "C" hipError_t lnbk_gemv_w13p(const GemvParams* p, hipStream_t st) {
+    if (p && (!p->wp || !lnbk_w13p_supported(56, p->K))) return hipErrorInvalidValue;
+    return launch_chain_t<56, 2, 28672, 7, LNB_W13P_R, EPI_SILU_MUL, true, true>(p, st);
+}
+extern "C" size_t lnbk_wpack_w13_bytes(int n_blocks, int K) { return wpack_bytes(n_blocks, K, WPACK_LANES_W13, 56); }
+extern "C" hipError_t lnbk_wpack_stats(const uint16_t* w, size_t elems, unsigned* d_stats, hipStream_t st) {
+    static const unsigned init[4] = {0xFFu, 0, 0, 0};
+    hipError_t e = hipMemcpyAsync(d_stats, init, sizeof init, hipMemcpyHostToDevice, st);
+    if (e != hipSuccess) return e;
+    hipLaunchKernelGGL(wpack_stats_kernel, dim3(1024), dim3(256), 0, st, w, elems / 8, d_stats);
+    return hipGetLastError();
+}
+extern "C" hipError_t lnbk_wpack_w13(const uint16_t* w, void* out, int K, int n_blocks, unsigned base, hipStream_t st) {
+    const size_t n = (size_t)n_blocks * wpack_stages(K, WPACK_LANES_W13, 56) * WPACK_LANES_W13;
+    hipLaunchKernelGGL(wpack_pack_kernel, dim3((unsigned)((n + 255) / 256)), dim3(256), 0, st, w, (char*)out, K, 56, WPACK_LANES_W13, n_blocks, base);
+    return hipGetLastError();
 }
 
 template <int EPI> static hipError_t launch_rowcast(const GemvParams* p, hipStream_t st) {
@@ -3992,6 +4093,7 @@
         gemv(rw, 1, EPI_STORE, 1); gemv(rw, 1, EPI_STORE, 0); gemv(rw, 1, EPI_QKV_ROPE, 1); gemv(rw, 1, EPI_RESID, 0);
         if (rw != 24) gemv(rw, 2, EPI_SILU_MUL, 1);
     }
+    if (e == hipSuccess) e = lnbk_gemv_w13p(nullptr, nullptr);
     for (auto prepare : {launch_attn_long<true>, launch_attn_long<false>, launch_attn_one, launch_attn_short}) if (e == hipSuccess) e = prepare(nullptr, nullptr);
     if (e == hipSuccess) e = launch_attn_rows(nullptr, -1, nullptr);
     if (e != hipSuccess) return e;
diff --git a/llama-nuts-and-bolts_amd/csrc/lnb_knobs.h b/llama-nuts-and-bolts_amd/csrc/lnb_knobs.h
--- a/llama-nuts-and-bolts_amd/csrc/lnb_knobs.h
+++ b/llama-nuts-and-bolts_amd/csrc/lnb_knobs.h
@@ -9,6 +9,8 @@
     X(RW_W2, 0, LIVE, "rows per block of the resident w2 layout (16 with W2_QUAD: measurement; 0: by shape)") \
     X(RW_OUT, 0, LIVE, "rows per block of the resident LM-head layout (0: by shape)") \
     X(RW_OP, 0, LIVE, "rows per block of a stand-alone lnb_op_linear operand (0: by shape)") \
+     \
+    X(W13_PACKED, 1, LIVE, "0: lnb_model_finalize builds no 13-bit planar copy of the gate|up matrices; the one-token step streams the raw bf16 (lnb_model_wpack_info)") \
      \
     X(PREFILL_MFMA, 1, ONCE, "0: calls of 16+ rows stay on the one-row kernels (what the parity tests compare the matrix-core forms with)") \
     X(PREFILL_STREAM, 1, ONCE, "0: prefill products on the LDS-tiled gemm_mfma_kernel, never the streaming feed") \
diff --git a/llama-nuts-and-bolts_amd/csrc/lnb_wpack.h b/llama-nuts-and-bolts_amd/csrc/lnb_wpack.h
--- /dev/null
+++ b/llama-nuts-and-bolts_amd/csrc/lnb_wpack.h
@@ -0,0 +1,73 @@
+#pragma once
+#include <stdint.h>
+#include <stddef.h>
+
+#if defined(__HIPCC__)
+#define LNB_WP_HD __host__ __device__ __forceinline__
+#else
+#define LNB_WP_HD static inline
+#endif
+
+#define WPACK_GROUP 32
+#define WPACK_GROUP_BYTES 52
+enum { WPACK_OK = 0, WPACK_SUBNORMAL = 1, WPACK_INFNAN = 2, WPACK_WINDOW = 3, WPACK_NOMEM = 4 };
+
+struct WpackStats { uint32_t min_e2, max_e2, subnormal, infnan; };
+LNB_WP_HD void wpack_stats_init(WpackStats* s) { s->min_e2 = 0xFFu; s->max_e2 = 0; s->subnormal = 0; s->infnan = 0; }
+LNB_WP_HD void wpack_stats_add(WpackStats* s, uint16_t w) {
+    const uint32_t e = (w >> 7) & 0xFFu;
+    if (e == 0xFFu) { s->infnan = 1; return; }
+    if (e < 2) { if (w & 0x7FFFu) s->subnormal = 1; return; }
+    const uint32_t e2 = e >> 1;
+    if (e2 < s->min_e2) s->min_e2 = e2;
+    if (e2 > s->max_e2) s->max_e2 = e2;
+}
+LNB_WP_HD int wpack_window(const WpackStats* s, uint32_t* base) {
+    *base = 0;
+    if (s->subnormal) return WPACK_SUBNORMAL;
+    if (s->infnan) return WPACK_INFNAN;
+    if (s->max_e2 == 0) return WPACK_OK;
+    *base = s->min_e2 - 1;
+    return s->max_e2 - *base <= 15 ? WPACK_OK : WPACK_WINDOW;
+}
+
+LNB_WP_HD uint32_t wpack_code(uint16_t w, uint32_t base) { const uint32_t e2 = (w >> 8) & 0x7Fu; return e2 ? e2 - base : 0; }
+LNB_WP_HD uint16_t wpack_scalar(uint32_t code, uint32_t sign, uint32_t low, uint32_t base) {
+    return (uint16_t)((sign << 15) | ((code ? base + code : 0u) << 8) | low);
+}
+LNB_WP_HD void wpack_pack_group(const uint16_t* w, uint32_t base, uint32_t* low8, uint32_t* code4, uint32_t* sign1) {
+    for (int g = 0; g < 8; g++) low8[g] = 0;
+    for (int u = 0; u < 4; u++) code4[u] = 0;
+    uint32_t s = 0;
+    for (int g = 0; g < 8; g++)
+        for (int j = 0; j < 4; j++) {
+            const uint16_t v = w[4 * g + j];
+            low8[g] |= (uint32_t)(v & 0xFFu) << (8 * j);
+            code4[g >> 1] |= wpack_code(v, base) << (8 * j + 4 * (g & 1));
+            s |= (uint32_t)(v >> 15) << (8 * j + 7 - g);
+        }
+    *sign1 = s;
+}
+LNB_WP_HD void wpack_unpack_group(const uint32_t* low8, const uint32_t* code4, uint32_t sign1, uint32_t base, uint16_t* w) {
+    for (int g = 0; g < 8; g++)
+        for (int j = 0; j < 4; j++)
+            w[4 * g + j] = wpack_scalar((code4[g >> 1] >> (8 * j + 4 * (g & 1))) & 0xFu, (sign1 >> (8 * j + 7 - g)) & 1u, (low8[g] >> (8 * j)) & 0xFFu, base);
+}
+
+LNB_WP_HD uint32_t wpack_spread(uint32_t code_dword, int h) { return (h ? code_dword >> 4 : code_dword) & 0x0F0F0F0Fu; }
+LNB_WP_HD uint32_t wpack_hi4(uint32_t c, uint32_t signs, int g, uint32_t base4) {
+    const uint32_t nz = (c + 0x7F7F7F7Fu) & 0x80808080u;
+    const uint32_t keep = nz - (nz >> 7);
+    return ((c + base4) & keep) | ((signs << g) & 0x80808080u);
+}
+template <int J> LNB_WP_HD uint32_t wpack_wide(uint32_t hi4, uint32_t lo4) {
+#if defined(__HIP_DEVICE_COMPILE__)
+    return __builtin_amdgcn_perm(hi4, lo4, ((4u + J) << 24) | ((uint32_t)J << 16) | 0x0C0Cu);
+#else
+    return (((hi4 >> (8 * J)) & 0xFFu) << 24) | (((lo4 >> (8 * J)) & 0xFFu) << 16);
+#endif
+}
+
+LNB_WP_HD size_t wpack_stage_bytes(int lanes) { return (size_t)lanes * WPACK_GROUP_BYTES; }
+LNB_WP_HD int wpack_stages(int K, int lanes, int rw) { const int kcs = 2 * lanes / rw; return ((K >> 3) + kcs - 1) / kcs; }
+LNB_WP_HD size_t wpack_bytes(int n_blocks, int K, int lanes, int rw) { return (size_t)n_blocks * (size_t)wpack_stages(K, lanes, rw) * wpack_stage_bytes(lanes); }
diff --git a/llama-nuts-and-bolts_amd/lnb.py b/llama-nuts-and-bolts_amd/lnb.py
--- a/llama-nuts-and-bolts_amd/lnb.py
+++ b/llama-nuts-and-bolts_amd/lnb.py
@@ -53,6 +53,7 @@
     "lnb_model_enable_batch", "lnb_model_batch_bytes", "lnb_batch_create", "lnb_batch_destroy", "lnb_batch_decode", "lnb_batch_decode_until", "lnb_ctx_set_stop_ids", "lnb_decode_greedy_until", "lnb_batch_profile_kernel", "lnb_batch_set_state", "lnb_batch_check_error", "lnb_pipeline_tick_batch",
     "lnb_pipeline_init_host", "lnb_batch_boundary_ptr",
     "lnb_abi_version", "lnb_runtime_info", "lnb_profile_ffn_pair",
+    "lnb_model_wpack_bytes", "lnb_model_wpack_info", "lnb_op_rmsnorm_gate_up",
     "lnb_ctx_set_token_probs", "lnb_ctx_read_token_probs", "lnb_ctx_token_prob_walks", "lnb_forward_score", "lnb_op_token_probs",
     "lnb_forward_append", "lnb_forward_score_append",
     "lnb_ctx_set_draft", "lnb_decode_speculative_until", "lnb_op_ngram_draft",
@@ -165,6 +166,10 @@
     L.lnb_model_enable_batch.argtypes = [vp]
     L.lnb_model_batch_bytes.argtypes = [vp]
     L.lnb_model_batch_bytes.restype = C.c_int64
+    L.lnb_model_wpack_bytes.argtypes = [vp]
+    L.lnb_model_wpack_bytes.restype = C.c_int64
+    L.lnb_model_wpack_info.argtypes = [vp, i32p]
+    L.lnb_op_rmsnorm_gate_up.argtypes = [C.c_int, vp, vp, C.c_float, vp, vp, vp, C.c_int, C.c_int, C.c_int, C.POINTER(C.c_int)]
     L.lnb_batch_create.argtypes = [C.POINTER(vp), C.c_int, C.POINTER(vp)]
     L.lnb_batch_destroy.argtypes = [vp]
     L.lnb_batch_decode.argtypes = [vp, i32p, i32p, C.c_int, vp, f32p]
@@ -462,6 +467,14 @@
     def batch_bytes(self):
         return int(self.L.lnb_model_batch_bytes(self.h))
 
+    def wpack_bytes(self):
+        return int(self.L.lnb_model_wpack_bytes(self.h))
+
+    def wpack_info(self):
+        c = np.zeros(6, dtype=np.int32)
+        _chk(self.L.lnb_model_wpack_info(self.h, c.ctypes.data_as(C.POINTER(C.c_int32))))
+        return dict(zip(("packed", "subnormal", "infnan", "window", "no_memory", "not_tried"), (int(v) for v in c)))
+
     def append_many_info(self):
         p, w, g = C.c_int(0), C.c_int(0), C.c_int(0)
         _chk(self.L.lnb_model_append_many_info(self.h, C.byref(p), C.byref(w), C.byref(g)))
@@ -956,3 +969,16 @@
 
 def synth_tokens(seed, n, vocab):
     return np.array([_splitmix64(seed ^ ((i * 0x9E3779B97F4A7C15) & _M64)) % vocab for i in range(n)], dtype=np.int32)
+
+
+def op_rmsnorm_gate_up(x_u16, norm_w_u16, eps, w1_u16, w3_u16, packed=1, device=0):
+    x = np.ascontiguousarray(x_u16, dtype=np.uint16).reshape(-1)
+    nw = np.ascontiguousarray(norm_w_u16, dtype=np.uint16)
+    w1 = np.ascontiguousarray(w1_u16, dtype=np.uint16)
+    w3 = np.ascontiguousarray(w3_u16, dtype=np.uint16)
+    n, k = w1.shape
+    assert w3.shape == (n, k) and x.shape == (k,) and nw.shape == (k,)
+    y = np.empty(n, dtype=np.uint16)
+    st = C.c_int(0)
+    _chk(lib().lnb_op_rmsnorm_gate_up(device, _p(x), _p(nw), np.float32(eps), _p(w1), _p(w3), _p(y), n, k, int(packed), C.byref(st)))
+    return y, st.value
```

Measured after the change: 249.6 tokens/s (median of 6 runs). 1.05x the previous value.
